# Sohojoe/ppo-dash

Measured on AMD Instinct MI355X. Metric: env-steps/sec (rollout+GAE+PPO update) at 4096 envs×128 steps, 1/2/4/8 MI355X, higher is better.
Workload: dtype f32

## Files before the change

include/ppo_hip.h:

```cpp
#ifndef PPO_HIP_H
#define PPO_HIP_H

#include <stdint.h>

#ifdef __cplusplus
extern "C" {
#endif

#define PPO_EARG 1001
#define PPO_ESHAPE 1002

const char* ppo_last_error(void);
int ppo_abi_version(void);
int ppo_prof_enable(const char* names, int capacity);
int ppo_prof_collect(double* out3);
int ppo_prof_collect_one(int idx, double* out3);

int ppo_gae_partials_count(int N);
int ppo_compute_returns(const float* rewards, float* value_preds, const float* masks, const float* bad_masks,
                        const float* next_value, float* returns, float* adv, double* partials, int T, int N,
                        double gamma, double gae_lambda, int use_gae, int use_proper_time_limits, void* stream);
int ppo_gae_scan_partials_count(int N);
int ppo_compute_returns_scan(const float* rewards, float* value_preds, const float* masks, const float* bad_masks,
                             const float* next_value, float* returns, float* adv, double* partials, int T, int N,
                             double gamma, double gae_lambda, int use_gae, int use_proper_time_limits, void* stream);
int ppo_adv_diff_partials_count(long long n);
int ppo_adv_diff(const float* returns, const float* value_preds, float* adv, double* partials, long long n,
                 void* stream);
int ppo_adv_finalize(const double* partials, int nparts, double count, double* stats, void* stream);
int ppo_adv_normalize(float* adv, long long n, const double* stats, void* stream);

int ppo_copy(void* dst, const void* src, long long bytes, void* stream);
int ppo_fill_f32(float* p, long long n, float v, void* stream);
int ppo_storage_insert_scalars(int N, int step, const int64_t* action, const float* logp, const float* value,
                               const float* reward, const float* mask, const float* bad_mask, int64_t* actions,
                               float* action_log_probs, float* value_preds, float* rewards, float* masks,
                               float* bad_masks, void* stream);
int ppo_gather_rows(const void* src, const int64_t* idx, void* dst, long long nrows, long long row_bytes,
                    void* stream);
int ppo_gather_f16_to_f32(const void* src, const int64_t* idx, float* dst, long long nrows, long long row_elems,
                          void* stream);
int ppo_gather_env_columns(const void* src, const int64_t* envs, void* dst, int T, int N, int nsel,
                           long long row_bytes, void* stream);
int ppo_synth_env_step(uint8_t* obs, int N, long long obs_bytes, float* reward, float* mask, float* bad_mask,
                       unsigned long long seed, unsigned long long step, float p_done, void* stream);

int ppo_cartpole_step(float* state, int* steps, const int64_t* action, float* obs, float* reward, float* mask,
                      float* bad_mask, float* ep_len, int N, unsigned long long seed, unsigned long long counter,
                      int max_steps, void* stream);

long long ppo_packed_weights_size(int H);
int ppo_packed_offsets(int H, long long* off6);
int ppo_pack_weights(const float* w2, const float* w3, const float* w4, int H, float* packed, void* stream);
int ppo_conv1_fwd(const void* obs, int obs_is_u8, const int64_t* idx, long long row0, int C, int B, const float* w1,
                  const float* b1, float* out, void* stream);
int ppo_conv1_fwd_mask(const void* obs, int obs_is_u8, const int64_t* idx, long long row0, int C, int B,
                       const float* w1, const float* b1, float* out, uint32_t* mbits, void* stream);
int ppo_conv1_fwd_f32(const float* obs, const int64_t* idx, long long row0, int B, const float* w1, const float* b1,
                      float* out, uint32_t* mbits, void* stream);
int ppo_conv1_fwd_rgb(const uint8_t* frames, const int64_t* idx, long long row0, int B, const float* mean, double stdv,
                      const float* w1, const float* b1, float* out, uint32_t* mbits, void* stream);
int ppo_conv1_wgrad_f32(const float* dz1, const float* obs, const int64_t* idx, long long row0, int B, int Z,
                        float* slab, float* slab_bias, void* stream);
int ppo_conv1_wgrad_rgb(const float* dz1, const uint8_t* frames, const int64_t* idx, long long row0, int B,
                        const float* mean, double stdv, int Z, float* slab, float* slab_bias, void* stream);
int ppo_conv2_fwd(const float* a1, int B, const float* w2p, const float* b2, float* out, void* stream);
int ppo_conv2_fwd_mask(const float* a1, int B, const float* w2p, const float* b2, float* out, uint64_t* mbits,
                       void* stream);
int ppo_conv3_fwd(const float* a2, int B, const float* w3p, const float* b3, float* out, void* stream);
int ppo_trunk_fwd(const uint8_t* obs, const int64_t* idx, long long row0, int B, const float* w1, const float* b1,
                  float* a1, uint32_t* m1, const float* w2p, const float* b2, float* a2, uint64_t* m2,
                  const float* w3p, const float* b3, float* a3, void* stream);
int ppo_fc_fwd(const float* x, int M, const float* w4p, const float* b, int H, float* out, int ldo, void* stream);
long long ppo_fc_fwd_ws_bytes(int M, int H);
int ppo_fc_fwd_ws(const float* x, int M, const float* w4p, const float* b, int H, float* out, int ldo, float* ws,
                  long long ws_bytes, void* stream);
int ppo_linear_relu_fwd(const float* x, int M, int K, const float* w, const float* b, int N, float* out,
                        void* stream);
int ppo_linear_fwd_ex(const float* x, const int64_t* idx, int M, int K, int lda, const float* w, const float* b,
                      int N, float* out, int ldo, int act, void* stream);
int ppo_linear_dgrad_ex(const float* dy, int M, int K, const float* wt, int N, const float* act, int ldact, int mode,
                        float* dx, void* stream);
int ppo_linear_dgrad_pair(const float* dy0, const float* wt0, int K0, const float* dy1, const float* wt1, int K1,
                          int M, int N, float* dx, void* stream);
int ppo_transpose(const float* src, int rows, int cols, float* dst, void* stream);
int ppo_linear_dgrad_mask(const float* dy, int M, int K, const float* wt, int N, const float* act, float* dx,
                          void* stream);
int ppo_conv3_fwd_mask(const float* a2, int B, const float* w3p, const float* b3, float* out, uint16_t* mbits,
                       void* stream);
int ppo_fc_dgrad_bits(const float* dy, int M, int K, const float* wt, const uint16_t* mbits, float* dx,
                      void* stream);
int ppo_conv3_dgrad(const float* dz3, int B, const float* w3d, const float* a2, float* dz2, void* stream);
int ppo_conv3_dgrad_bits_ok(void);
int ppo_conv3_dgrad_bits(const float* dz3, int B, const float* w3d, const uint64_t* m2bits, float* dz2,
                         void* stream);
int ppo_conv2_dgrad(const float* dz2, int B, const float* w2d, const float* a1, float* dz1, void* stream);
int ppo_conv2_dgrad_bits_ok(void);
int ppo_conv2_dgrad_bits(const float* dz2, int B, const float* w2d, const uint32_t* m1bits, float* dz1,
                         void* stream);
int ppo_wgrad_splits(long long R, int tiles, int target_blocks, int min_ktiles);
int ppo_conv1_wgrad(const float* dz1, const void* obs, int obs_is_u8, const int64_t* idx, long long row0, int C,
                    int B, int Z, float* slab, float* slab_bias, void* stream);
int ppo_conv2_wgrad(const float* dz2, const float* a1, int B, int Z, float* slab, float* slab_bias, void* stream);
int ppo_conv3_wgrad(const float* dz3, const float* a2, int B, int Z, float* slab, float* slab_bias, void* stream);
int ppo_linear_wgrad(const float* dy, const float* x, int R, int N, int K, int Z, float* slab, float* slab_bias,
                     void* stream);
int ppo_probe_side_kernel(int blocks, int threads, long long ticks, long long* stamps, void* stream);
int ppo_probe_now(long long* out, void* stream);
int ppo_wgrad_reduce(const float* slab, const float* slab_bias, int Z, int M, int NW, int kind, int a, int b,
                     float* gw, float* gb, float scale, int accumulate, void* stream);
int ppo_colsum(const float* src, long long ld, int rows, long long cols, float* out, float scale, int accumulate,
               void* stream);
int ppo_tune_set(const char* key, int value);
int ppo_tune_get(const char* key);

int ppo_obs_preprocess(const uint8_t* src, long long src_stride, int N, int S, int mode, const double* mean,
                       double stdv, int mono, float* dst, long long dst_stride, void* stream);
int ppo_frame_stack(float* stacked, int N, int nstack, long long frame_elems, const float* obs,
                    const uint8_t* done, int reset, void* stream);

int ppo_gru_step_fwd(const float* hprev, const float* masks, const int64_t* mask_idx, const float* whh,
                     const float* bhh, const float* gi, int M, int H, float* hout, float* save_r, float* save_z,
                     float* save_n, float* save_ghn, float* save_hin, void* stream);
int ppo_gru_cell_bwd(const float* dout, const float* carry, const float* r, const float* z, const float* n,
                     const float* ghn, const float* hin, float* dgi, float* dgh, float* dhz, int M, int H,
                     int has_carry, void* stream);
int ppo_gru_step_bwd(const float* dgh, const float* whhT, const float* dhz, const float* masks,
                     const int64_t* mask_idx, float* carry, int M, int H, void* stream);
int ppo_gru_variant_set(int v);
int ppo_gru_variant_get(void);
int ppo_gru_seq_fwd(const float* h0, const float* masks, const int64_t* idx, const float* whh, const float* bhh,
                    const float* gi, int T, int n, int H, float* hout, float* save_r, float* save_z, float* save_n,
                    float* save_ghn, float* save_hin, void* stream);
int ppo_gru_persist_set(int v);
int ppo_gru_persist_get(void);
int ppo_gru_persist_spin_set(int polls);
int ppo_gru_persist_timeouts(void* stream);
int ppo_gru_seq_counters(int n);
int ppo_gru_seq_fwd_ws(const float* h0, const float* masks, const int64_t* idx, const float* whh, const float* bhh,
                       const float* gi, int T, int n, int H, float* hout, float* save_r, float* save_z,
                       float* save_n, float* save_ghn, float* save_hin, int* counters, int* err, void* stream);
int ppo_gru_seq_bwd(const float* dout, const float* save_r, const float* save_z, const float* save_n,
                    const float* save_ghn, const float* save_hin, const float* masks, const int64_t* idx,
                    const float* whhT, int T, int n, int H, float* dgi, float* dgh, float* dhz, float* carry,
                    void* stream);
int ppo_gru_seq_bwd_ws(const float* dout, const float* save_r, const float* save_z, const float* save_n,
                       const float* save_ghn, const float* save_hin, const float* masks, const int64_t* idx,
                       const float* whhT, int T, int n, int H, float* dgi, float* dgh, float* dhz, float* carry,
                       int* counters, int* err, void* stream);
int ppo_gru_step_bwd_cell(const float* dgh, const float* whhT, float* dhz, const float* masks,
                          const int64_t* mask_idx, float* carry, int M, int H, const float* dout_prev,
                          const float* r, const float* z, const float* n, const float* ghn, const float* hin,
                          float* dgi_prev, float* dgh_prev, void* stream);
int ppo_gru_pack(const float* wih, const float* whh, int H, int I, int Ip, float* wih_pad, float* wihT, float* whhT,
                 void* stream);
int ppo_concat_cols(const float* src, const int64_t* idx, long long rows, int ncols, float* dst, int ld, int col0,
                    int zero_to, void* stream);
int ppo_rec_indices(const int64_t* envs, int n, int T, int N, int64_t* idx, void* stream);

int ppo_heads_act(const float* feat, const float* feat_v, int N, int H, const float* wc, const float* bc,
                  const float* wa,
                  const float* ba, int A, const float* noise, unsigned long long seed, unsigned long long counter,
                  int deterministic, const int64_t* given, float* value, int64_t* action, float* logp,
                  float* entropy, void* stream);
int ppo_heads_train_blocks(int B);
int ppo_heads_train(const float* feat, const float* feat_v, int B, int H, const float* wc, const float* bc,
                    const float* wa,
                    const float* ba, int A, const int64_t* idx, long long row0, const int64_t* actions,
                    const float* old_logp, const float* adv, const float* vpred, const float* ret, float clip,
                    float value_coef, float entropy_coef, float inv_b, int use_clipped_value_loss, int feat_act,
                    float* dfeat, float* dfeat_v, float* part_w, float* part_b, float* part_loss, void* stream);
int ppo_heads_reduce(const float* part_w, const float* part_b, const float* part_loss, int nblk, int H, int A,
                     float* g_wc, float* g_bc, float* g_wa, float* g_ba, double* loss_acc, double inv_b, float scale,
                     int use_clipped_value_loss, void* stream);
int ppo_heads_gauss_act(const float* feat, const float* feat_v, int N, int H, const float* wc, const float* bc,
                        const float* wa, const float* ba, const float* logstd, int A, const float* noise,
                        unsigned long long seed, unsigned long long counter, int deterministic, const float* given,
                        float* value, float* action, float* logp, float* entropy, void* stream);
int ppo_heads_gauss_train(const float* feat, const float* feat_v, int B, int H, const float* wc, const float* bc,
                          const float* wa, const float* ba, const float* logstd, int A, const int64_t* idx,
                          long long row0, const float* actions, const float* old_logp, const float* adv,
                          const float* vpred, const float* ret, float clip, float value_coef, float entropy_coef,
                          float inv_b, int use_clipped_value_loss, int feat_act, float* dfeat, float* dfeat_v,
                          float* part_w, float* part_b, float* part_loss, void* stream);
int ppo_heads_gauss_reduce(const float* part_w, const float* part_b, const float* part_loss, int nblk, int H, int A,
                           float* g_wc, float* g_bc, float* g_wa, float* g_ba, float* g_logstd, double* loss_acc,
                           double inv_b, float scale, void* stream);
int ppo_heads_bern_act(const float* feat, const float* feat_v, int N, int H, const float* wc, const float* bc,
                       const float* wa, const float* ba, int A, const float* noise, unsigned long long seed,
                       unsigned long long counter, int deterministic, const float* given, float* value,
                       float* action, float* logp, float* entropy, void* stream);
int ppo_heads_bern_train(const float* feat, const float* feat_v, int B, int H, const float* wc, const float* bc,
                         const float* wa, const float* ba, int A, const int64_t* idx, long long row0,
                         const float* actions, const float* old_logp, const float* adv, const float* vpred,
                         const float* ret, float clip, float value_coef, float entropy_coef, float inv_b,
                         int use_clipped_value_loss, int feat_act, float* dfeat, float* dfeat_v, float* part_w,
                         float* part_b, float* part_loss, void* stream);
int ppo_heads_act_dc(const float* feat, const float* feat_v, int N, int H, const float* wc, const float* bc,
                     const float* wa, const float* ba, int A, const float* noise, unsigned long long seed,
                     const unsigned long long* counter, int deterministic, const int64_t* given, float* value,
                     int64_t* action, float* logp, float* entropy, void* stream);
int ppo_heads_gauss_act_dc(const float* feat, const float* feat_v, int N, int H, const float* wc, const float* bc,
                           const float* wa, const float* ba, const float* logstd, int A, const float* noise,
                           unsigned long long seed, const unsigned long long* counter, int deterministic,
                           const float* given, float* value, float* action, float* logp, float* entropy,
                           void* stream);
int ppo_heads_bern_act_dc(const float* feat, const float* feat_v, int N, int H, const float* wc, const float* bc,
                          const float* wa, const float* ba, int A, const float* noise, unsigned long long seed,
                          const unsigned long long* counter, int deterministic, const float* given, float* value,
                          float* action, float* logp, float* entropy, void* stream);
int ppo_rng_advance(unsigned long long* counter, unsigned long long by, void* stream);
int ppo_mean_f32(const float* x, long long n, float* out, void* stream);

int ppo_grad_partials_count(long long n);
int ppo_grad_sumsq(const float* g, long long n, float scale, double* partials, void* stream);
int ppo_clip_adam(float* params, float* grads, float* exp_avg, float* exp_avg_sq, long long n,
                  const double* partials, float scale, double max_norm, double lr, double beta1, double beta2,
                  double eps, long long step, double* norm_out, void* stream);
int ppo_clip_adam_guarded(float* params, float* grads, float* exp_avg, float* exp_avg_sq, long long n,
                          const double* partials, float scale, double max_norm, double lr, double beta1,
                          double beta2, double eps, long long step, double* norm_out, const int* guard_i,
                          const double* guard_d, int* skipped, void* stream);

#ifdef __cplusplus
}
#endif
#endif
```

ppo-dash_amd/a2c_ppo_acktr/_engine.py:

```python
import contextlib

import os

import torch

from . import _dist
from ._hip import call, ptr, stream
from .distributions import Bernoulli, DiagGaussian

FUSED_TRUNK = os.environ.get("PPO_FUSED_TRUNK", "1") != "0"
FEAT = 32 * 7 * 7


def _with_precision(fn):
    def wrapper(self, *args, **kwargs):
        if not getattr(self.policy, "_half_mode", False):
            return fn(self, *args, **kwargs)
        prev = call("ppo_tune_get", b"products")
        if prev != 1:
            call("ppo_tune_set", b"products", 1)
        try:
            return fn(self, *args, **kwargs)
        finally:
            if prev != 1:
                call("ppo_tune_set", b"products", prev)
    wrapper.__name__, wrapper.__doc__ = fn.__name__, fn.__doc__
    return wrapper


class _Workspace:
    def __init__(self):
        self.bufs = {}
        self.version = 0

    def get(self, name, numel, dtype=torch.float32, device=None):
        t = self.bufs.get(name)
        if t is None or t.numel() < numel or t.dtype != dtype or t.device != device:
            t = torch.empty(max(int(numel), 1), dtype=dtype, device=device)
            self.bufs[name] = t
            self.version += 1
        return t


class CNNEngine:

    W1, B1, W2, B2, W3, B3, W4, B4, WC, BC, WA, BA, LS = range(13)
    recurrent = False

    def _bind_dist(self, policy):
        self.dist_kind = ("gauss" if isinstance(policy.dist, DiagGaussian) else
                          "bern" if isinstance(policy.dist, Bernoulli) else "cat")
        self.gauss = self.dist_kind == "gauss"
        self.float_actions = self.dist_kind != "cat"
        self.A = (policy.dist.fc_mean if self.gauss else policy.dist.linear).weight.shape[0]

    def __init__(self, policy, device):
        self.policy = policy
        self.device = device
        base = policy.base
        self.C = base.main[0].weight.shape[1]
        self.H = base.main[7].weight.shape[0]
        self._bind_dist(policy)
        if self.H > 512 or self.H % 4 != 0:
            raise NotImplementedError(f"hidden_size {self.H}: the HIP engine supports multiples of 4 up to 512")
        if not self.recurrent and base.critic_linear.weight.shape[1] != self.H:
            raise NotImplementedError("vector observations with a non-recurrent CNNBase are not supported "
                                      "(the reference crashes there too: Categorical expects hidden_size inputs)")
        self.params = list(policy.parameters())
        self.ws = {"act": _Workspace(), "train": _Workspace()}
        self.act_ws = "act"
        self.obs_decode = None
        self.packed = None
        self._pack_key = None
        self.epoch = 0
        self._flatten()
        self.rng_seed = int(torch.initial_seed()) & 0xFFFFFFFFFFFFFFFF
        self.rng_counter = 0
        self._n_cu = None
        self._init_status()

    def _init_status(self):
        self.status = torch.zeros(4, dtype=torch.int32, device=self.device)
        self._rng_dev = None
        self._device_counter = False

    @property
    def rng_dev(self):
        if self._rng_dev is None:
            self._rng_dev = torch.zeros(1, dtype=torch.int64, device=self.device)
        return self._rng_dev

    def set_rng_dev(self, value):
        v = int(value) & 0xFFFFFFFFFFFFFFFF
        self.rng_dev.fill_(v - (1 << 64) if v >> 63 else v)

    @contextlib.contextmanager
    def using_device_counter(self):
        prev, self._device_counter = self._device_counter, True
        try:
            yield self.rng_dev
        finally:
            self._device_counter = prev

    def status_ptr(self, i):
        return self.status.data_ptr() + 4 * i

    def _flatten(self):
        n = sum(p.numel() for p in self.params)
        flat = torch.empty(n, device=self.device)
        grad = torch.zeros(n, device=self.device)
        off = 0
        self.offsets = []
        with torch.no_grad():
            for p in self.params:
                k = p.numel()
                flat[off:off + k].copy_(p.data.reshape(-1))
                p.data = flat[off:off + k].view_as(p)
                p.grad = grad[off:off + k].view_as(p)
                self.offsets.append(off)
                off += k
        self.flat, self.grad, self.numel = flat, grad, n
        self.epoch += 1

    @contextlib.contextmanager
    def using_workspace(self, name):
        self.ws.setdefault(name, _Workspace())
        prev, self.act_ws = self.act_ws, name
        try:
            yield self.ws[name]
        finally:
            self.act_ws = prev

    def is_bound(self):
        base = self.flat.data_ptr()
        for p, off in zip(self.params, self.offsets):
            if p.data.data_ptr() != base + 4 * off or not p.is_cuda:
                return False
        return True

    def ensure_bound(self):
        if not self.is_bound():
            self._flatten()

    def pv(self, i):
        return self.flat.data_ptr() + 4 * self.offsets[i]

    def gv(self, i):
        return self.grad.data_ptr() + 4 * self.offsets[i]

    def pack(self, force=False):
        key = (sum(p._version for p in self.params), self.epoch)
        if not force and self.packed is not None and key == self._pack_key:
            return
        if self.packed is None:
            self.packed = torch.empty(call("ppo_packed_weights_size", self.H), device=self.device)
            offs = torch.zeros(6, dtype=torch.int64)
            call("ppo_packed_offsets", self.H, offs.data_ptr())
            self.poff = [int(x) for x in offs]
        call("ppo_pack_weights", self.pv(self.W2), self.pv(self.W3), self.pv(self.W4), self.H,
             self.packed.data_ptr(), stream())
        self._pack_extra()
        self._pack_key = key

    def _pack_extra(self):
        pass

    def pk(self, seg):
        return self.packed.data_ptr() + 4 * self.poff[seg]

    @staticmethod
    def _obs_args(obs):
        if obs.dtype == torch.uint8:
            return 1
        if obs.dtype == torch.float32:
            return 0
        raise TypeError(f"observations must be uint8, float32 or float16, got {obs.dtype}")

    @staticmethod
    def _is_rgb(obs):
        return obs.dtype == torch.uint8 and tuple(obs.shape[-3:]) == (84, 84, 3)

    def set_obs_decode(self, mean, std):
        if self.C != 4:
            raise NotImplementedError("the fused RGB decode produces FrameStackMono(2)'s 4 channels (C = 4)")
        if mean is not None:
            m64 = torch.as_tensor(mean, dtype=torch.float64).reshape(84, 84, 3)
            m32 = m64.to(torch.float32)
            if not torch.equal(m32.to(torch.float64), m64):
                raise ValueError("the fused decode needs fp32-representable means (NormalizeWrapper's files hold "
                                 "fp32 values); use ObsPreprocess into fp32 storage otherwise")
            mean = m32.contiguous().to(self.device)
        if not float(std):
            raise ValueError("std must be non-zero")
        self.obs_decode = (mean, float(std))

    def _conv1(self, obs, idx, B, a1, m1, s):
        if self._is_rgb(obs):
            if self.obs_decode is None:
                raise TypeError("raw u8 RGB frames need the fused decode: Policy.set_obs_decode(ObsPreprocess)")
            mean, std = self.obs_decode
            call("ppo_conv1_fwd_rgb", obs.data_ptr(), ptr(idx, torch.int64, "idx"), 0, B, ptr(mean), std,
                 self.pv(self.W1), self.pv(self.B1), a1.data_ptr(), ptr(m1), s)
        elif m1 is not None:
            call("ppo_conv1_fwd_mask", obs.data_ptr(), self._obs_args(obs), ptr(idx, torch.int64, "idx"), 0, self.C,
                 B, self.pv(self.W1), self.pv(self.B1), a1.data_ptr(), m1.data_ptr(), s)
        else:
            call("ppo_conv1_fwd", obs.data_ptr(), self._obs_args(obs), ptr(idx, torch.int64, "idx"), 0, self.C, B,
                 self.pv(self.W1), self.pv(self.B1), a1.data_ptr(), s)

    def _obs_f32(self, obs, idx, B, ws):
        if obs.dtype != torch.float16:
            return obs, idx
        x = ws.get("obs32", B * self.C * 84 * 84, device=self.device)
        call("ppo_gather_f16_to_f32", obs.data_ptr(), ptr(idx, torch.int64, "idx"), x.data_ptr(), B,
             self.C * 84 * 84, stream())
        return x, None

    def trunk(self, obs, idx, B, ws, out=None, ldo=None):
        dev = self.device
        obs, idx = self._obs_f32(obs, idx, B, ws)
        a1 = ws.get("a1", B * 400 * 32, device=dev)
        a2 = ws.get("a2", B * 81 * 64, device=dev)
        a3 = ws.get("a3", B * FEAT, device=dev)
        if out is None:
            out, ldo = ws.get("h", B * self.H, device=dev), self.H
        s = stream()
        train = ws is self.ws["train"]
        m1 = ws.get("m1bits", B * 400, dtype=torch.int32, device=dev) if train else None
        m2 = ws.get("m2bits", B * 81, dtype=torch.int64, device=dev) if train else None
        m3 = ws.get("m3bits", B * 49, dtype=torch.int32, device=dev) if train else None
        if obs.dtype == torch.uint8 and self.C == 4 and not self._is_rgb(obs) and FUSED_TRUNK and not train:
            call("ppo_trunk_fwd", obs.data_ptr(), ptr(idx, torch.int64, "idx"), 0, B, self.pv(self.W1),
                 self.pv(self.B1), a1.data_ptr(), None, self.pk(0), self.pv(self.B2), a2.data_ptr(), None,
                 self.pk(1), self.pv(self.B3), a3.data_ptr(), s)
        else:
            self._conv1(obs, idx, B, a1, m1[:B * 400] if train else None, s)
            if train:
                call("ppo_conv2_fwd_mask", a1.data_ptr(), B, self.pk(0), self.pv(self.B2), a2.data_ptr(),
                     m2.data_ptr(), s)
                call("ppo_conv3_fwd_mask", a2.data_ptr(), B, self.pk(1), self.pv(self.B3), a3.data_ptr(),
                     m3.data_ptr(), s)
            else:
                call("ppo_conv2_fwd", a1.data_ptr(), B, self.pk(0), self.pv(self.B2), a2.data_ptr(), s)
                call("ppo_conv3_fwd", a2.data_ptr(), B, self.pk(1), self.pv(self.B3), a3.data_ptr(), s)
        if train:
            self._mask_rows = B
        nb = call("ppo_fc_fwd_ws_bytes", B, self.H)
        if nb:
            fws = ws.get("fc_ws", nb // 4, device=dev)
            call("ppo_fc_fwd_ws", a3.data_ptr(), B, self.pk(2), self.pv(self.B4), self.H, out.data_ptr(), ldo,
                 fws.data_ptr(), nb, s)
        else:
            call("ppo_fc_fwd", a3.data_ptr(), B, self.pk(2), self.pv(self.B4), self.H, out.data_ptr(), ldo, s)
        return out

    def _check_obs(self, obs):
        obs = obs if obs.is_cuda else obs.to(self.device)
        if self.obs_decode is not None and self._is_rgb(obs) and obs.dim() == 4:
            return obs.contiguous()
        if tuple(obs.shape[1:]) != (self.C, 84, 84):
            raise RuntimeError(f"CNNBase expects [N,{self.C},84,84] observations"
                               + (" or raw [N,84,84,3] u8 frames" if self.obs_decode is not None else "")
                               + f", got {tuple(obs.shape)}")
        return obs.contiguous()

    def _heads(self, h, B, deterministic=False, noise=None, given=None, want_entropy=False, value_only=False,
               hv=None):
        value = torch.empty(B, 1, device=self.device)
        if value_only:
            action = logp = ent = None
        elif self.float_actions:
            action = given if given is not None else torch.empty(B, self.A, device=self.device)
            logp = torch.empty(B, 1, device=self.device)
            ent = torch.empty(B, device=self.device) if want_entropy else None
        else:
            action = given if given is not None else torch.empty(B, 1, dtype=torch.int64, device=self.device)
            logp = torch.empty(B, 1, device=self.device)
            ent = torch.empty(B, device=self.device) if want_entropy else None
        if noise is not None:
            noise = noise.to(self.device, torch.float32).contiguous()
            if noise.shape != (B, self.A):
                raise RuntimeError(f"noise must be [{B},{self.A}]")
        if self._device_counter:
            counter, dc = self.rng_dev.data_ptr(), "_dc"
        else:
            self.rng_counter += 1
            counter, dc = self.rng_counter, ""
        if self.float_actions and given is not None and given.numel() != B * self.A:
            raise RuntimeError(f"actions must be [{B},{self.A}], got {tuple(given.shape)}")
        if self.dist_kind == "bern":
            call("ppo_heads_bern_act" + dc, h.data_ptr(), ptr(hv), B, self.H, self.pv(self.WC), self.pv(self.BC),
                 self.pv(self.WA), self.pv(self.BA), self.A, ptr(noise), self.rng_seed, counter,
                 int(bool(deterministic)),
                 ptr(given.reshape(-1).contiguous() if given is not None else None, torch.float32, "action"),
                 value.data_ptr(), None if given is not None or value_only else action.data_ptr(),
                 ptr(logp), ptr(ent), stream())
        elif self.gauss:
            call("ppo_heads_gauss_act" + dc, h.data_ptr(), ptr(hv), B, self.H, self.pv(self.WC), self.pv(self.BC),
                 self.pv(self.WA), self.pv(self.BA), self.pv(self.LS), self.A, ptr(noise), self.rng_seed,
                 counter, int(bool(deterministic)),
                 ptr(given.reshape(-1).contiguous() if given is not None else None, torch.float32, "action"),
                 value.data_ptr(), None if given is not None or value_only else action.data_ptr(),
                 ptr(logp), ptr(ent), stream())
        else:
            call("ppo_heads_act" + dc, h.data_ptr(), ptr(hv), B, self.H, self.pv(self.WC), self.pv(self.BC),
                 self.pv(self.WA), self.pv(self.BA), self.A, ptr(noise), self.rng_seed, counter,
                 int(bool(deterministic)),
                 ptr(given.reshape(-1).contiguous() if given is not None else None, torch.int64, "action"),
                 value.data_ptr(), None if given is not None or value_only else action.data_ptr(),
                 ptr(logp), ptr(ent), stream())
        if self._device_counter:
            call("ppo_rng_advance", self.rng_dev.data_ptr(), 1, stream())
        return value, action, logp, ent

    def mean(self, x):
        out = torch.empty((), device=self.device)
        call("ppo_mean_f32", x.data_ptr(), x.numel(), out.data_ptr(), stream())
        return out

    @_with_precision
    def act(self, obs, deterministic=False, noise=None, given=None, want_entropy=False, value_only=False):
        self.ensure_bound()
        self.pack()
        obs = self._check_obs(obs)
        B = obs.shape[0]
        h = self.trunk(obs, None, B, self.ws[self.act_ws])
        return self._heads(h, B, deterministic, noise, given, want_entropy, value_only)

    def _heads_train(self, storage, adv, idx, feat, B, hp, loss_acc, dfeat, feat_act, feat_v=None, dfeat_v=None):
        ws, dev, H, A, s = self.ws["train"], self.device, self.H, self.A, stream()
        nblk = call("ppo_heads_train_blocks", B)
        part_w = ws.get("part_w", nblk * (1 + A) * H, device=dev)
        part_b = ws.get("part_b", nblk * (1 + (2 * A if self.gauss else A)), device=dev)
        part_l = ws.get("part_l", nblk * 4, device=dev)
        inv_b = 1.0 / B
        if self.float_actions and storage.actions.shape[-1] != A:
            raise RuntimeError(f"storage holds {storage.actions.shape[-1]} action dimensions, the policy {A}")
        if self.dist_kind == "bern":
            call("ppo_heads_bern_train", feat.data_ptr(), ptr(feat_v), B, H, self.pv(self.WC), self.pv(self.BC),
                 self.pv(self.WA), self.pv(self.BA), A, idx.data_ptr(), 0,
                 ptr(storage.actions, torch.float32, "storage.actions"), storage.action_log_probs.data_ptr(),
                 adv.data_ptr(), storage.value_preds.data_ptr(), storage.returns.data_ptr(), hp["clip"],
                 hp["value_coef"], hp["entropy_coef"], inv_b, int(hp["use_clipped_value_loss"]), int(feat_act),
                 dfeat.data_ptr(), ptr(dfeat_v), part_w.data_ptr(), part_b.data_ptr(), part_l.data_ptr(), s)
            call("ppo_heads_reduce", part_w.data_ptr(), part_b.data_ptr(), part_l.data_ptr(), nblk, H, A,
                 self.gv(self.WC), self.gv(self.BC), self.gv(self.WA), self.gv(self.BA), loss_acc.data_ptr(), inv_b,
                 1.0, int(hp["use_clipped_value_loss"]), s)
            return
        if self.gauss:
            call("ppo_heads_gauss_train", feat.data_ptr(), ptr(feat_v), B, H, self.pv(self.WC), self.pv(self.BC),
                 self.pv(self.WA), self.pv(self.BA), self.pv(self.LS), A, idx.data_ptr(), 0,
                 ptr(storage.actions, torch.float32, "storage.actions"), storage.action_log_probs.data_ptr(),
                 adv.data_ptr(), storage.value_preds.data_ptr(), storage.returns.data_ptr(), hp["clip"],
                 hp["value_coef"], hp["entropy_coef"], inv_b, int(hp["use_clipped_value_loss"]), int(feat_act),
                 dfeat.data_ptr(), ptr(dfeat_v), part_w.data_ptr(), part_b.data_ptr(), part_l.data_ptr(), s)
            call("ppo_heads_gauss_reduce", part_w.data_ptr(), part_b.data_ptr(), part_l.data_ptr(), nblk, H, A,
                 self.gv(self.WC), self.gv(self.BC), self.gv(self.WA), self.gv(self.BA), self.gv(self.LS),
                 loss_acc.data_ptr(), inv_b, 1.0, s)
            return
        call("ppo_heads_train", feat.data_ptr(), ptr(feat_v), B, H, self.pv(self.WC), self.pv(self.BC), self.pv(self.WA),
             self.pv(self.BA), A, idx.data_ptr(), 0, storage.actions.data_ptr(), storage.action_log_probs.data_ptr(),
             adv.data_ptr(), storage.value_preds.data_ptr(), storage.returns.data_ptr(), hp["clip"], hp["value_coef"],
             hp["entropy_coef"], inv_b, int(hp["use_clipped_value_loss"]), int(feat_act), dfeat.data_ptr(),
             ptr(dfeat_v), part_w.data_ptr(), part_b.data_ptr(), part_l.data_ptr(), s)
        call("ppo_heads_reduce", part_w.data_ptr(), part_b.data_ptr(), part_l.data_ptr(), nblk, H, A,
             self.gv(self.WC), self.gv(self.BC), self.gv(self.WA), self.gv(self.BA), loss_acc.data_ptr(), inv_b, 1.0,
             int(hp["use_clipped_value_loss"]), s)

    def _trunk_backward(self, B, dh, obs, idx):
        ws, dev, s = self.ws["train"], self.device, stream()
        a1 = ws.bufs["a1"]
        a2, a3 = ws.bufs["a2"], ws.bufs["a3"]
        dz3 = ws.get("dz3", B * FEAT, device=dev)
        dz2 = ws.get("dz2", B * 81 * 64, device=dev)
        dz1 = ws.get("dz1", B * 400 * 32, device=dev)
        bits = getattr(self, "_mask_rows", None) == B
        if bits:
            call("ppo_fc_dgrad_bits", dh.data_ptr(), B, self.H, self.pk(3), ws.bufs["m3bits"].data_ptr(),
                 dz3.data_ptr(), s)
        else:
            call("ppo_linear_dgrad_mask", dh.data_ptr(), B, self.H, self.pk(3), FEAT, a3.data_ptr(), dz3.data_ptr(),
                 s)
        self._wgrad("fc", B, dh, a3, None, s)
        _dist.start_bucket(self.grad[self.offsets[self.W4]:])
        if bits:
            call("ppo_conv3_dgrad_bits", dz3.data_ptr(), B, self.pk(4), ws.bufs["m2bits"].data_ptr(), dz2.data_ptr(),
                 s)
        else:
            call("ppo_conv3_dgrad", dz3.data_ptr(), B, self.pk(4), a2.data_ptr(), dz2.data_ptr(), s)
        self._wgrad("conv3", B, dz3, a2, None, s)
        if bits:
            call("ppo_conv2_dgrad_bits", dz2.data_ptr(), B, self.pk(5), ws.bufs["m1bits"].data_ptr(), dz1.data_ptr(),
                 s)
        else:
            call("ppo_conv2_dgrad", dz2.data_ptr(), B, self.pk(5), a1.data_ptr(), dz1.data_ptr(), s)
        self._wgrad("conv2", B, dz2, a1, None, s)
        if obs.dtype == torch.float16:
            obs, idx = ws.bufs["obs32"], None
        self._wgrad("conv1", B, dz1, obs, idx, s)

    def _finish_step(self, optimizer):
        optimizer._step_flat(self)
        self.epoch += 1
        self.pack(force=True)

    @_with_precision
    def train_minibatch(self, storage, adv, idx, hp, loss_acc, optimizer):
        self.ensure_bound()
        self.pack()
        _dist.begin_minibatch()
        B = idx.numel()
        ws = self.ws["train"]
        h = self.trunk(storage.obs, idx, B, ws)
        dh = ws.get("dh", B * self.H, device=self.device)
        self._heads_train(storage, adv, idx, h, B, hp, loss_acc, dh, feat_act=1)
        self._trunk_backward(B, dh, storage.obs, idx)
        self._finish_step(optimizer)

    def _wgrad(self, layer, B, dz, x, idx, s):
        dev = self.device
        ws = self.ws["train"]
        if layer == "conv1":
            M, NW, kind, ka, kb, wi, bi, R, tiles = 32, self.C * 64, 0, 0, 0, self.W1, self.B1, B * 400, 1
        elif layer == "conv2":
            M, NW, kind, ka, kb, wi, bi, R, tiles = 64, 512, 1, 4, 32, self.W2, self.B2, B * 81, 4
        elif layer == "conv3":
            M, NW, kind, ka, kb, wi, bi, R, tiles = 32, 576, 1, 3, 64, self.W3, self.B3, B * 49, 5
        else:
            M, NW, kind, ka, kb, wi, bi, R, tiles = self.H, FEAT, 2, 32, 49, self.W4, self.B4, B, \
                ((self.H + 127) // 128) * 13
        if self._n_cu is None:
            self._n_cu = torch.cuda.get_device_properties(self.device).multi_processor_count
        target = max(self._n_cu, -(-B // 512)) * tiles if layer in ("conv1", "conv2", "conv3") else 2048
        Z = call("ppo_wgrad_splits", R, tiles, target, 16)
        slab = ws.get("slab", Z * M * NW, device=dev)
        slab_b = ws.get("slab_b", Z * M, device=dev)
        if layer == "conv1" and self._is_rgb(x):
            mean, std = self.obs_decode
            call("ppo_conv1_wgrad_rgb", dz.data_ptr(), x.data_ptr(), ptr(idx), 0, B, ptr(mean), std, Z,
                 slab.data_ptr(), slab_b.data_ptr(), s)
        elif layer == "conv1":
            call("ppo_conv1_wgrad", dz.data_ptr(), x.data_ptr(), self._obs_args(x), ptr(idx), 0, self.C, B, Z,
                 slab.data_ptr(), slab_b.data_ptr(), s)
        elif layer == "conv2":
            call("ppo_conv2_wgrad", dz.data_ptr(), x.data_ptr(), B, Z, slab.data_ptr(), slab_b.data_ptr(), s)
        elif layer == "conv3":
            call("ppo_conv3_wgrad", dz.data_ptr(), x.data_ptr(), B, Z, slab.data_ptr(), slab_b.data_ptr(), s)
        else:
            call("ppo_linear_wgrad", dz.data_ptr(), x.data_ptr(), B, self.H, FEAT, Z, slab.data_ptr(),
                 slab_b.data_ptr(), s)
        scale = 1.0 / 255.0 if layer == "conv1" and x.dtype == torch.uint8 and not self._is_rgb(x) else 1.0
        call("ppo_wgrad_reduce", slab.data_ptr(), slab_b.data_ptr(), Z, M, NW, kind, ka, kb, self.gv(wi), self.gv(bi),
             scale, 0, s)

    def _dense_wgrad(self, dy, x, R, N, K, kind, a, wi, bi):
        ws, dev, s = self.ws["train"], self.device, stream()
        tiles = ((N + 127) // 128) * ((K + 127) // 128)
        Z = call("ppo_wgrad_splits", R, tiles, 2048, 16)
        slab = ws.get("slab", Z * N * K, device=dev)
        slab_b = ws.get("slab_b", Z * N, device=dev)
        call("ppo_linear_wgrad", dy.data_ptr(), x.data_ptr(), R, N, K, Z, slab.data_ptr(), slab_b.data_ptr(), s)
        call("ppo_wgrad_reduce", slab.data_ptr(), slab_b.data_ptr(), Z, N, K, kind, a, 0, self.gv(wi), self.gv(bi),
             1.0, 0, s)


class RecurrentEngine(CNNEngine):

    GIH, GHH, GBI, GBH = range(4)
    W1, B1, W2, B2, W3, B3, W4, B4, WC, BC, WA, BA, LS = range(4, 17)
    recurrent = True

    def __init__(self, policy, device):
        gru = policy.base.gru
        self.V = policy.base.vector_obs_len
        H = policy.base.main[7].weight.shape[0]
        self.I = H + self.V
        self.Ip = (self.I + 3) // 4 * 4
        if gru.weight_ih_l0.shape != (3 * H, self.I) or H % 32 != 0:
            raise NotImplementedError("GRU engine needs hidden_size a multiple of 32 (<= 512)")
        self.gru_packed = None
        super().__init__(policy, device)

    def _pack_extra(self):
        H, Ip = self.H, self.Ip
        if self.gru_packed is None:
            self.gru_packed = torch.empty(3 * H * Ip + 6 * H * H, device=self.device)
        gp = self.gru_packed.data_ptr()
        self.wih_pad, self.wihT, self.whhT = gp, gp + 4 * 3 * H * Ip, gp + 4 * (3 * H * Ip + 3 * H * H)
        call("ppo_gru_pack", self.pv(self.GIH), self.pv(self.GHH), H, self.I, Ip, self.wih_pad, self.wihT, self.whhT,
             stream())

    def _input(self, obs, vec, idx, B, ws, rows_vec=None):
        dev, s, H, Ip = self.device, stream(), self.H, self.Ip
        x = ws.get("xpad", B * Ip, device=dev)
        self.trunk(obs, idx, B, ws, out=x, ldo=Ip)
        if Ip > H:
            src = vec if vec is not None else x
            call("ppo_concat_cols", src.data_ptr(), ptr(rows_vec), B, self.V if vec is not None else 0,
                 x.data_ptr(), Ip, H, Ip - H, s)
        gi = ws.get("gi", B * 3 * H, device=dev)
        call("ppo_linear_fwd_ex", x.data_ptr(), None, B, Ip, Ip, self.wih_pad, self.pv(self.GBI), 3 * H,
             gi.data_ptr(), 3 * H, 0, s)
        return x, gi

    def _vec(self, vec, B):
        if self.V == 0:
            return None
        return vec.to(self.device, torch.float32).reshape(B, self.V).contiguous()

    @_with_precision
    def act(self, obs, deterministic=False, noise=None, given=None, want_entropy=False, value_only=False,
            vec=None, hxs=None, masks=None):
        self.ensure_bound()
        self.pack()
        obs = self._check_obs(obs)
        B = obs.shape[0]
        ws = self.ws[self.act_ws]
        _, gi = self._input(obs, self._vec(vec, B), None, B, ws)
        hxs = hxs.to(self.device, torch.float32).reshape(B, self.H).contiguous()
        m = masks.to(self.device, torch.float32).reshape(B).contiguous() if masks is not None else None
        hout = torch.empty(B, self.H, device=self.device)
        call("ppo_gru_step_fwd", hxs.data_ptr(), ptr(m), None, self.pv(self.GHH), self.pv(self.GBH), gi.data_ptr(),
             B, self.H, hout.data_ptr(), None, None, None, None, None, stream())
        value, action, logp, ent = self._heads(hout, B, deterministic, noise, given, want_entropy, value_only)
        return value, action, logp, ent, hout

    @_with_precision
    def evaluate_sequence(self, obs, vec, hxs, masks, action):
        self.ensure_bound()
        self.pack()
        obs = self._check_obs(obs)
        R = obs.shape[0]
        N = hxs.shape[0]
        T = R // N
        ws = self.ws[self.act_ws]
        _, gi = self._input(obs, self._vec(vec, R), None, R, ws)
        hxs = hxs.to(self.device, torch.float32).reshape(N, self.H).contiguous()
        m = masks.to(self.device, torch.float32).reshape(R).contiguous()
        hout = torch.empty(R, self.H, device=self.device)
        H, s = self.H, stream()
        cnt = ws.get("gru_cnt", call("ppo_gru_seq_counters", N), torch.int32, self.device)
        call("ppo_gru_seq_fwd_ws", hxs.data_ptr(), m.data_ptr(), None, self.pv(self.GHH), self.pv(self.GBH),
             gi.data_ptr(), T, N, H, hout.data_ptr(), None, None, None, None, None, cnt.data_ptr(), self.status_ptr(2),
             s)
        if int(self.status[2].item()):
            self.status[2].zero_()
            raise RuntimeError("evaluate_actions: the persistent GRU kernel timed out (its outputs are invalid; "
                               "ppo_gru_persist_set(0) selects the per-step launches)")
        given = action.to(self.device, torch.float32 if self.float_actions else torch.int64)
        value, _, logp, ent = self._heads(hout, R, want_entropy=True, given=given)
        return value, logp, ent, hout[(T - 1) * N:]

    @_with_precision
    def train_minibatch_rec(self, storage, adv, envs, hp, loss_acc, optimizer):
        self.ensure_bound()
        self.pack()
        _dist.begin_minibatch()
        dev, H, s = self.device, self.H, stream()
        T, N, n = storage.num_steps, storage.rewards.shape[1], envs.numel()
        R = T * n
        ws = self.ws["train"]
        idx = ws.get("ridx", R, torch.int64, dev)[:R]
        call("ppo_rec_indices", envs.data_ptr(), n, T, N, idx.data_ptr(), s)
        h0 = ws.get("h0", n * H, device=dev)
        call("ppo_gather_rows", storage.recurrent_hidden_states.data_ptr(), envs.data_ptr(), h0.data_ptr(), n,
             4 * H, s)
        vec = storage.vector_obs if self.V else None
        x, gi = self._input(storage.obs, vec, idx, R, ws, rows_vec=idx if self.V else None)
        hout = ws.get("hout", R * H, device=dev)
        sv = {k: ws.get("s_" + k, R * H, device=dev) for k in ("r", "z", "n", "ghn", "hin")}
        masks = storage.masks
        cnt = ws.get("gru_cnt", call("ppo_gru_seq_counters", n), torch.int32, dev)
        _dist.assert_no_pending("train_minibatch_rec")
        call("ppo_gru_seq_fwd_ws", h0.data_ptr(), masks.data_ptr(), idx.data_ptr(), self.pv(self.GHH),
             self.pv(self.GBH), gi.data_ptr(), T, n, H, hout.data_ptr(), sv["r"].data_ptr(), sv["z"].data_ptr(),
             sv["n"].data_ptr(), sv["ghn"].data_ptr(), sv["hin"].data_ptr(), cnt.data_ptr(), self.status_ptr(0), s)
        dout = ws.get("dout", R * H, device=dev)
        self._heads_train(storage, adv, idx, hout, R, hp, loss_acc, dout, feat_act=0)
        dgi = ws.get("dgi", R * 3 * H, device=dev)
        dgh = ws.get("dgh", R * 3 * H, device=dev)
        dhz = ws.get("dhz", n * H, device=dev)
        carry = ws.get("carry", n * H, device=dev)
        _dist.assert_no_pending("train_minibatch_rec bptt")
        call("ppo_gru_seq_bwd_ws", dout.data_ptr(), sv["r"].data_ptr(), sv["z"].data_ptr(), sv["n"].data_ptr(),
             sv["ghn"].data_ptr(), sv["hin"].data_ptr(), masks.data_ptr(), idx.data_ptr(), self.whhT, T, n, H,
             dgi.data_ptr(), dgh.data_ptr(), dhz.data_ptr(), carry.data_ptr(), cnt.data_ptr(), self.status_ptr(0), s)
        self._dense_wgrad(dgh, sv["hin"], R, 3 * H, H, 0, 0, self.GHH, self.GBH)
        self._dense_wgrad(dgi, x, R, 3 * H, self.Ip, 3, self.I, self.GIH, self.GBI)
        dh = ws.get("dh", R * H, device=dev)
        call("ppo_linear_dgrad_ex", dgi.data_ptr(), R, 3 * H, self.wihT, H, x.data_ptr(), self.Ip, 1, dh.data_ptr(),
             s)
        self._trunk_backward(R, dh, storage.obs, idx)
        self._finish_step(optimizer)


class MLPEngine(CNNEngine):

    AW1, AB1, AW2, AB2, CW1, CB1, CW2, CB2, WC, BC, WA, BA, LS = range(13)

    def __init__(self, policy, device):
        base = policy.base
        if base.is_recurrent != self.recurrent:
            raise NotImplementedError("a recurrent MLPBase runs on RecurrentMLPEngine, a feed-forward one on "
                                      "MLPEngine (Policy.hip_engine() selects the engine)")
        self.policy, self.device = policy, device
        self.H = base._hidden_size
        self.I = (base.gru.weight_ih_l0 if self.recurrent else base.actor[0].weight).shape[1]
        self.V = base.vector_obs_len
        self.obs_dim = self.I - self.V
        self.Ip = (self.I + 3) // 4 * 4
        self._bind_dist(policy)
        if self.recurrent and (self.H % 32 != 0 or self.H > 512 or self.I < 1):
            raise NotImplementedError("GRU engine needs hidden_size a multiple of 32 (<= 512)")
        if self.H % 4 != 0 or self.H > 512:
            raise NotImplementedError(f"MLPBase hidden_size {self.H}: multiples of 4 up to 512")
        self.params = list(policy.parameters())
        self.ws = {"act": _Workspace(), "train": _Workspace()}
        self.act_ws = "act"
        self.packed = None
        self._pack_key = None
        self.epoch = 0
        self._flatten()
        self.rng_seed = int(torch.initial_seed()) & 0xFFFFFFFFFFFFFFFF
        self.rng_counter = 0
        self._init_status()

    def pack(self, force=False):
        key = (sum(p._version for p in self.params), self.epoch)
        if not force and self.packed is not None and key == self._pack_key:
            return
        H, Ip, s = self.H, self.Ip, stream()
        if self.packed is None:
            self.packed = torch.empty(2 * H * Ip + 2 * H * H, device=self.device)
        b = self.packed.data_ptr()
        self.aw1, self.cw1 = b, b + 4 * H * Ip
        self.aw2T, self.cw2T = b + 8 * H * Ip, b + 8 * H * Ip + 4 * H * H
        for w, dst in ((self.AW1, self.aw1), (self.CW1, self.cw1)):
            call("ppo_concat_cols", self.pv(w), None, H, self.I, dst, Ip, 0, Ip, s)
        call("ppo_transpose", self.pv(self.AW2), H, H, self.aw2T, s)
        call("ppo_transpose", self.pv(self.CW2), H, H, self.cw2T, s)
        self._pack_key = key

    def _x(self, obs, vec, idx, B, ws):
        dev, s = self.device, stream()
        x = ws.get("x", B * self.Ip, device=dev)
        call("ppo_concat_cols", obs.data_ptr(), ptr(idx), B, self.obs_dim, x.data_ptr(), self.Ip, 0,
             self.obs_dim if self.V else self.Ip, s)
        if self.V:
            call("ppo_concat_cols", vec.data_ptr(), ptr(idx), B, self.V, x.data_ptr(), self.Ip, self.obs_dim,
                 self.Ip - self.obs_dim, s)
        return x

    def _tower_in(self):
        return self.Ip, self.aw1, self.cw1

    def towers(self, x, B, ws):
        dev, H, s = self.device, self.H, stream()
        Ip, aw1, cw1 = self._tower_in()
        out = {}
        for name, w1, b1, w2, b2 in (("a", aw1, self.AB1, self.AW2, self.AB2),
                                     ("c", cw1, self.CB1, self.CW2, self.CB2)):
            h1 = ws.get(name + "1", B * H, device=dev)
            h2 = ws.get(name + "2", B * H, device=dev)
            call("ppo_linear_fwd_ex", x.data_ptr(), None, B, Ip, Ip, w1, self.pv(b1), H, h1.data_ptr(), H, 2, s)
            call("ppo_linear_fwd_ex", h1.data_ptr(), None, B, H, H, self.pv(w2), self.pv(b2), H, h2.data_ptr(), H, 2, s)
            out[name] = (h1, h2)
        return out

    @_with_precision
    def act(self, obs, deterministic=False, noise=None, given=None, want_entropy=False, value_only=False, vec=None):
        self.ensure_bound()
        self.pack()
        obs = (obs if obs.is_cuda else obs.to(self.device)).to(torch.float32).reshape(obs.shape[0], -1).contiguous()
        B = obs.shape[0]
        if obs.shape[1] != self.obs_dim:
            raise RuntimeError(f"MLPBase expects [N,{self.obs_dim}] observations, got {tuple(obs.shape)}")
        ws = self.ws[self.act_ws]
        v = vec.to(self.device, torch.float32).reshape(B, self.V).contiguous() if self.V else None
        x = self._x(obs, v, None, B, ws)
        t = self.towers(x, B, ws)
        return self._heads(t["a"][1], B, deterministic, noise, given, want_entropy, value_only, hv=t["c"][1])

    @_with_precision
    def train_minibatch(self, storage, adv, idx, hp, loss_acc, optimizer):
        self.ensure_bound()
        self.pack()
        _dist.begin_minibatch()
        dev, H, B = self.device, self.H, idx.numel()
        ws = self.ws["train"]
        x = self._x(storage.obs, storage.vector_obs if self.V else None, idx, B, ws)
        t = self.towers(x, B, ws)
        da2 = ws.get("da2", B * H, device=dev)
        dc2 = ws.get("dc2", B * H, device=dev)
        self._heads_train(storage, adv, idx, t["a"][1], B, hp, loss_acc, da2, feat_act=2, feat_v=t["c"][1],
                          dfeat_v=dc2)
        self._towers_backward(t, x, B, da2, dc2, self.Ip, 3, self.I)
        self._finish_step(optimizer)

    def _towers_backward(self, t, x, B, da2, dc2, K, kind, width):
        ws, dev, H = self.ws["train"], self.device, self.H
        d1s = []
        for name, d2, w1, b1, w2, b2, w2T in (("a", da2, self.AW1, self.AB1, self.AW2, self.AB2, self.aw2T),
                                               ("c", dc2, self.CW1, self.CB1, self.CW2, self.CB2, self.cw2T)):
            h1 = t[name][0]
            self._dense_wgrad(d2, h1, B, H, H, 0, 0, w2, b2)
            d1 = ws.get("d1" + name, B * H, device=dev)
            call("ppo_linear_dgrad_ex", d2.data_ptr(), B, H, w2T, H, h1.data_ptr(), H, 2, d1.data_ptr(), stream())
            self._dense_wgrad(d1, x, B, H, K, kind, width, w1, b1)
            d1s.append(d1)
        return d1s


class RecurrentMLPEngine(MLPEngine):

    GIH, GHH, GBI, GBH = range(4)
    AW1, AB1, AW2, AB2, CW1, CB1, CW2, CB2, WC, BC, WA, BA, LS = range(4, 17)
    recurrent = True

    def pack(self, force=False):
        key = (sum(p._version for p in self.params), self.epoch)
        if not force and self.packed is not None and key == self._pack_key:
            return
        H, Ip, s = self.H, self.Ip, stream()
        if self.packed is None:
            self.packed = torch.empty(3 * H * Ip + 3 * H * H + 4 * H * H, device=self.device)
        b = self.packed.data_ptr()
        self.wih_pad, self.whhT = b, b + 4 * 3 * H * Ip
        self.aw1T = self.whhT + 4 * 3 * H * H
        self.cw1T, self.aw2T, self.cw2T = (self.aw1T + 4 * H * H * i for i in (1, 2, 3))
        call("ppo_concat_cols", self.pv(self.GIH), None, 3 * H, self.I, self.wih_pad, Ip, 0, Ip, s)
        call("ppo_transpose", self.pv(self.GHH), 3 * H, H, self.whhT, s)
        for w, dst in ((self.AW1, self.aw1T), (self.CW1, self.cw1T), (self.AW2, self.aw2T), (self.CW2, self.cw2T)):
            call("ppo_transpose", self.pv(w), H, H, dst, s)
        self._pack_key = key

    def _tower_in(self):
        return self.H, self.pv(self.AW1), self.pv(self.CW1)

    def _rows(self, obs, vec, R):
        obs = (obs if obs.is_cuda else obs.to(self.device)).to(torch.float32).reshape(R, -1).contiguous()
        if obs.shape[1] != self.obs_dim:
            raise RuntimeError(f"MLPBase expects [N,{self.obs_dim}] observations, got {tuple(obs.shape)}")
        v = vec.to(self.device, torch.float32).reshape(R, self.V).contiguous() if self.V else None
        return obs, v

    def _gi(self, x, B, ws):
        gi = ws.get("gi", B * 3 * self.H, device=self.device)
        call("ppo_linear_fwd_ex", x.data_ptr(), None, B, self.Ip, self.Ip, self.wih_pad, self.pv(self.GBI),
             3 * self.H, gi.data_ptr(), 3 * self.H, 0, stream())
        return gi

    @_with_precision
    def act(self, obs, deterministic=False, noise=None, given=None, want_entropy=False, value_only=False,
            vec=None, hxs=None, masks=None):
        self.ensure_bound()
        self.pack()
        B = obs.shape[0]
        obs, v = self._rows(obs, vec, B)
        ws = self.ws[self.act_ws]
        gi = self._gi(self._x(obs, v, None, B, ws), B, ws)
        hxs = hxs.to(self.device, torch.float32).reshape(B, self.H).contiguous()
        m = masks.to(self.device, torch.float32).reshape(B).contiguous() if masks is not None else None
        hout = torch.empty(B, self.H, device=self.device)
        call("ppo_gru_step_fwd", hxs.data_ptr(), ptr(m), None, self.pv(self.GHH), self.pv(self.GBH), gi.data_ptr(),
             B, self.H, hout.data_ptr(), None, None, None, None, None, stream())
        t = self.towers(hout, B, ws)
        value, action, logp, ent = self._heads(t["a"][1], B, deterministic, noise, given, want_entropy, value_only,
                                               hv=t["c"][1])
        return value, action, logp, ent, hout

    @_with_precision
    def evaluate_sequence(self, obs, vec, hxs, masks, action):
        self.ensure_bound()
        self.pack()
        R, N = obs.shape[0], hxs.shape[0]
        T = R // N
        obs, v = self._rows(obs, vec, R)
        ws = self.ws[self.act_ws]
        gi = self._gi(self._x(obs, v, None, R, ws), R, ws)
        hxs = hxs.to(self.device, torch.float32).reshape(N, self.H).contiguous()
        m = masks.to(self.device, torch.float32).reshape(R).contiguous()
        hout = torch.empty(R, self.H, device=self.device)
        H, s = self.H, stream()
        cnt = ws.get("gru_cnt", call("ppo_gru_seq_counters", N), torch.int32, self.device)
        call("ppo_gru_seq_fwd_ws", hxs.data_ptr(), m.data_ptr(), None, self.pv(self.GHH), self.pv(self.GBH),
             gi.data_ptr(), T, N, H, hout.data_ptr(), None, None, None, None, None, cnt.data_ptr(), self.status_ptr(2),
             s)
        if int(self.status[2].item()):
            self.status[2].zero_()
            raise RuntimeError("evaluate_actions: the persistent GRU kernel timed out (its outputs are invalid; "
                               "ppo_gru_persist_set(0) selects the per-step launches)")
        given = action.to(self.device, torch.float32 if self.float_actions else torch.int64)
        t = self.towers(hout, R, ws)
        value, _, logp, ent = self._heads(t["a"][1], R, want_entropy=True, given=given, hv=t["c"][1])
        return value, logp, ent, hout[(T - 1) * N:]

    @_with_precision
    def train_minibatch_rec(self, storage, adv, envs, hp, loss_acc, optimizer):
        H = self.H
        if storage.recurrent_hidden_states.shape[-1] != H:
            raise RuntimeError(f"storage holds hidden states of width {storage.recurrent_hidden_states.shape[-1]}, "
                               f"the policy's GRU {H}")
        if storage.obs.dtype != torch.float32 or storage.obs[0, 0].numel() != self.obs_dim:
            raise RuntimeError(f"MLPBase expects float32 [{self.obs_dim}] observation rows in the storage, got "
                               f"{storage.obs.dtype} {tuple(storage.obs.shape[2:])}")
        self.ensure_bound()
        self.pack()
        _dist.begin_minibatch()
        dev, s = self.device, stream()
        T, N, n = storage.num_steps, storage.rewards.shape[1], envs.numel()
        R = T * n
        ws = self.ws["train"]
        idx = ws.get("ridx", R, torch.int64, dev)[:R]
        call("ppo_rec_indices", envs.data_ptr(), n, T, N, idx.data_ptr(), s)
        h0 = ws.get("h0", n * H, device=dev)
        call("ppo_gather_rows", storage.recurrent_hidden_states.data_ptr(), envs.data_ptr(), h0.data_ptr(), n,
             4 * H, s)
        x = self._x(storage.obs, storage.vector_obs if self.V else None, idx, R, ws)
        gi = self._gi(x, R, ws)
        hout = ws.get("hout", R * H, device=dev)
        sv = {k: ws.get("s_" + k, R * H, device=dev) for k in ("r", "z", "n", "ghn", "hin")}
        masks = storage.masks
        cnt = ws.get("gru_cnt", call("ppo_gru_seq_counters", n), torch.int32, dev)
        _dist.assert_no_pending("train_minibatch_rec")
        call("ppo_gru_seq_fwd_ws", h0.data_ptr(), masks.data_ptr(), idx.data_ptr(), self.pv(self.GHH),
             self.pv(self.GBH), gi.data_ptr(), T, n, H, hout.data_ptr(), sv["r"].data_ptr(), sv["z"].data_ptr(),
             sv["n"].data_ptr(), sv["ghn"].data_ptr(), sv["hin"].data_ptr(), cnt.data_ptr(), self.status_ptr(0), s)
        t = self.towers(hout, R, ws)
        da2 = ws.get("da2", R * H, device=dev)
        dc2 = ws.get("dc2", R * H, device=dev)
        self._heads_train(storage, adv, idx, t["a"][1], R, hp, loss_acc, da2, feat_act=2, feat_v=t["c"][1],
                          dfeat_v=dc2)
        d1a, d1c = self._towers_backward(t, hout, R, da2, dc2, H, 0, 0)
        dout = ws.get("dout", R * H, device=dev)
        call("ppo_linear_dgrad_pair", d1a.data_ptr(), self.aw1T, H, d1c.data_ptr(), self.cw1T, H, R, H,
             dout.data_ptr(), s)
        dgi = ws.get("dgi", R * 3 * H, device=dev)
        dgh = ws.get("dgh", R * 3 * H, device=dev)
        dhz = ws.get("dhz", n * H, device=dev)
        carry = ws.get("carry", n * H, device=dev)
        _dist.assert_no_pending("train_minibatch_rec bptt")
        call("ppo_gru_seq_bwd_ws", dout.data_ptr(), sv["r"].data_ptr(), sv["z"].data_ptr(), sv["n"].data_ptr(),
             sv["ghn"].data_ptr(), sv["hin"].data_ptr(), masks.data_ptr(), idx.data_ptr(), self.whhT, T, n, H,
             dgi.data_ptr(), dgh.data_ptr(), dhz.data_ptr(), carry.data_ptr(), cnt.data_ptr(), self.status_ptr(0), s)
        self._dense_wgrad(dgh, sv["hin"], R, 3 * H, H, 0, 0, self.GHH, self.GBH)
        self._dense_wgrad(dgi, x, R, 3 * H, self.Ip, 3, self.I, self.GIH, self.GBI)
        self._finish_step(optimizer)
```

ppo-dash_amd/a2c_ppo_acktr/_hip.py:

```python
import ctypes
import os

import torch

_HERE = os.path.dirname(os.path.abspath(__file__))
LIB_PATH = os.environ.get("PPO_HIP_LIB", os.path.join(os.path.dirname(_HERE), "lib", "libppo_hip.so"))

c_int, c_ll, c_ull, c_f, c_d, c_p = (ctypes.c_int, ctypes.c_longlong, ctypes.c_ulonglong, ctypes.c_float,
                                     ctypes.c_double, ctypes.c_void_p)

SIGNATURES = {
    "ppo_abi_version": [],
    "ppo_last_error": [],
    "ppo_prof_enable": [ctypes.c_char_p, c_int],
    "ppo_prof_collect": [c_p],
    "ppo_prof_collect_one": [c_int, c_p],
    "ppo_gae_partials_count": [c_int],
    "ppo_compute_returns": [c_p, c_p, c_p, c_p, c_p, c_p, c_p, c_p, c_int, c_int, c_d, c_d, c_int, c_int, c_p],
    "ppo_gae_scan_partials_count": [c_int],
    "ppo_compute_returns_scan": [c_p, c_p, c_p, c_p, c_p, c_p, c_p, c_p, c_int, c_int, c_d, c_d, c_int, c_int, c_p],
    "ppo_adv_diff_partials_count": [c_ll],
    "ppo_adv_diff": [c_p, c_p, c_p, c_p, c_ll, c_p],
    "ppo_adv_finalize": [c_p, c_int, c_d, c_p, c_p],
    "ppo_adv_normalize": [c_p, c_ll, c_p, c_p],
    "ppo_copy": [c_p, c_p, c_ll, c_p],
    "ppo_fill_f32": [c_p, c_ll, c_f, c_p],
    "ppo_storage_insert_scalars": [c_int, c_int, c_p, c_p, c_p, c_p, c_p, c_p, c_p, c_p, c_p, c_p, c_p, c_p, c_p],
    "ppo_gather_rows": [c_p, c_p, c_p, c_ll, c_ll, c_p],
    "ppo_gather_env_columns": [c_p, c_p, c_p, c_int, c_int, c_int, c_ll, c_p],
    "ppo_gather_f16_to_f32": [c_p, c_p, c_p, c_ll, c_ll, c_p],
    "ppo_synth_env_step": [c_p, c_int, c_ll, c_p, c_p, c_p, c_ull, c_ull, c_f, c_p],
    "ppo_cartpole_step": [c_p, c_p, c_p, c_p, c_p, c_p, c_p, c_p, c_int, c_ull, c_ull, c_int, c_p],
    "ppo_packed_weights_size": [c_int],
    "ppo_packed_offsets": [c_int, c_p],
    "ppo_pack_weights": [c_p, c_p, c_p, c_int, c_p, c_p],
    "ppo_conv1_fwd": [c_p, c_int, c_p, c_ll, c_int, c_int, c_p, c_p, c_p, c_p],
    "ppo_conv1_fwd_mask": [c_p, c_int, c_p, c_ll, c_int, c_int, c_p, c_p, c_p, c_p, c_p],
    "ppo_conv1_fwd_f32": [c_p, c_p, c_ll, c_int, c_p, c_p, c_p, c_p, c_p],
    "ppo_conv1_fwd_rgb": [c_p, c_p, c_ll, c_int, c_p, c_d, c_p, c_p, c_p, c_p, c_p],
    "ppo_conv1_wgrad_f32": [c_p, c_p, c_p, c_ll, c_int, c_int, c_p, c_p, c_p],
    "ppo_conv1_wgrad_rgb": [c_p, c_p, c_p, c_ll, c_int, c_p, c_d, c_int, c_p, c_p, c_p],
    "ppo_conv2_fwd": [c_p, c_int, c_p, c_p, c_p, c_p],
    "ppo_conv2_fwd_mask": [c_p, c_int, c_p, c_p, c_p, c_p, c_p],
    "ppo_conv3_fwd": [c_p, c_int, c_p, c_p, c_p, c_p],
    "ppo_trunk_fwd": [c_p, c_p, c_ll, c_int, c_p, c_p, c_p, c_p, c_p, c_p, c_p, c_p, c_p, c_p, c_p, c_p],
    "ppo_linear_relu_fwd": [c_p, c_int, c_int, c_p, c_p, c_int, c_p, c_p],
    "ppo_fc_fwd": [c_p, c_int, c_p, c_p, c_int, c_p, c_int, c_p],
    "ppo_fc_fwd_ws_bytes": [c_int, c_int],
    "ppo_fc_fwd_ws": [c_p, c_int, c_p, c_p, c_int, c_p, c_int, c_p, c_ll, c_p],
    "ppo_linear_dgrad_mask": [c_p, c_int, c_int, c_p, c_int, c_p, c_p, c_p],
    "ppo_conv3_fwd_mask": [c_p, c_int, c_p, c_p, c_p, c_p, c_p],
    "ppo_fc_dgrad_bits": [c_p, c_int, c_int, c_p, c_p, c_p, c_p],
    "ppo_conv3_dgrad": [c_p, c_int, c_p, c_p, c_p, c_p],
    "ppo_conv3_dgrad_bits_ok": [],
    "ppo_conv3_dgrad_bits": [c_p, c_int, c_p, c_p, c_p, c_p],
    "ppo_conv2_dgrad": [c_p, c_int, c_p, c_p, c_p, c_p],
    "ppo_conv2_dgrad_bits_ok": [],
    "ppo_conv2_dgrad_bits": [c_p, c_int, c_p, c_p, c_p, c_p],
    "ppo_wgrad_splits": [c_ll, c_int, c_int, c_int],
    "ppo_conv1_wgrad": [c_p, c_p, c_int, c_p, c_ll, c_int, c_int, c_int, c_p, c_p, c_p],
    "ppo_conv2_wgrad": [c_p, c_p, c_int, c_int, c_p, c_p, c_p],
    "ppo_probe_side_kernel": [c_int, c_int, c_ll, c_p, c_p],
    "ppo_probe_now": [c_p, c_p],
    "ppo_conv3_wgrad": [c_p, c_p, c_int, c_int, c_p, c_p, c_p],
    "ppo_linear_wgrad": [c_p, c_p, c_int, c_int, c_int, c_int, c_p, c_p, c_p],
    "ppo_wgrad_reduce": [c_p, c_p, c_int, c_int, c_int, c_int, c_int, c_int, c_p, c_p, c_f, c_int, c_p],
    "ppo_colsum": [c_p, c_ll, c_int, c_ll, c_p, c_f, c_int, c_p],
    "ppo_tune_set": [ctypes.c_char_p, c_int],
    "ppo_tune_get": [ctypes.c_char_p],
    "ppo_heads_act": [c_p, c_p, c_int, c_int, c_p, c_p, c_p, c_p, c_int, c_p, c_ull, c_ull, c_int, c_p, c_p, c_p,
                      c_p, c_p, c_p],
    "ppo_heads_train_blocks": [c_int],
    "ppo_heads_train": [c_p, c_p, c_int, c_int, c_p, c_p, c_p, c_p, c_int, c_p, c_ll, c_p, c_p, c_p, c_p, c_p, c_f,
                        c_f, c_f, c_f, c_int, c_int, c_p, c_p, c_p, c_p, c_p, c_p],
    "ppo_linear_fwd_ex": [c_p, c_p, c_int, c_int, c_int, c_p, c_p, c_int, c_p, c_int, c_int, c_p],
    "ppo_linear_dgrad_ex": [c_p, c_int, c_int, c_p, c_int, c_p, c_int, c_int, c_p, c_p],
    "ppo_linear_dgrad_pair": [c_p, c_p, c_int, c_p, c_p, c_int, c_int, c_int, c_p, c_p],
    "ppo_transpose": [c_p, c_int, c_int, c_p, c_p],
    "ppo_gru_step_fwd": [c_p, c_p, c_p, c_p, c_p, c_p, c_int, c_int, c_p, c_p, c_p, c_p, c_p, c_p, c_p],
    "ppo_gru_cell_bwd": [c_p, c_p, c_p, c_p, c_p, c_p, c_p, c_p, c_p, c_p, c_int, c_int, c_int, c_p],
    "ppo_gru_step_bwd": [c_p, c_p, c_p, c_p, c_p, c_p, c_int, c_int, c_p],
    "ppo_gru_variant_set": [c_int],
    "ppo_gru_variant_get": [],
    "ppo_gru_persist_set": [c_int],
    "ppo_gru_persist_get": [],
    "ppo_gru_persist_timeouts": [c_p],
    "ppo_gru_persist_spin_set": [c_int],
    "ppo_gru_seq_counters": [c_int],
    "ppo_gru_seq_fwd": [c_p, c_p, c_p, c_p, c_p, c_p, c_int, c_int, c_int, c_p, c_p, c_p, c_p, c_p, c_p, c_p],
    "ppo_gru_seq_fwd_ws": [c_p, c_p, c_p, c_p, c_p, c_p, c_int, c_int, c_int, c_p, c_p, c_p, c_p, c_p, c_p, c_p, c_p,
                           c_p],
    "ppo_gru_seq_bwd": [c_p, c_p, c_p, c_p, c_p, c_p, c_p, c_p, c_p, c_int, c_int, c_int, c_p, c_p, c_p, c_p, c_p],
    "ppo_gru_seq_bwd_ws": [c_p, c_p, c_p, c_p, c_p, c_p, c_p, c_p, c_p, c_int, c_int, c_int, c_p, c_p, c_p, c_p, c_p,
                           c_p, c_p],
    "ppo_gru_step_bwd_cell": [c_p, c_p, c_p, c_p, c_p, c_p, c_int, c_int, c_p, c_p, c_p, c_p, c_p, c_p, c_p, c_p, c_p],
    "ppo_gru_pack": [c_p, c_p, c_int, c_int, c_int, c_p, c_p, c_p, c_p],
    "ppo_concat_cols": [c_p, c_p, c_ll, c_int, c_p, c_int, c_int, c_int, c_p],
    "ppo_rec_indices": [c_p, c_int, c_int, c_int, c_p, c_p],
    "ppo_heads_reduce": [c_p, c_p, c_p, c_int, c_int, c_int, c_p, c_p, c_p, c_p, c_p, c_d, c_f, c_int, c_p],
    "ppo_mean_f32": [c_p, c_ll, c_p, c_p],
    "ppo_heads_gauss_act": [c_p, c_p, c_int, c_int, c_p, c_p, c_p, c_p, c_p, c_int, c_p, c_ull, c_ull, c_int, c_p,
                            c_p, c_p, c_p, c_p, c_p],
    "ppo_heads_gauss_train": [c_p, c_p, c_int, c_int, c_p, c_p, c_p, c_p, c_p, c_int, c_p, c_ll, c_p, c_p, c_p, c_p,
                              c_p, c_f, c_f, c_f, c_f, c_int, c_int, c_p, c_p, c_p, c_p, c_p, c_p],
    "ppo_heads_gauss_reduce": [c_p, c_p, c_p, c_int, c_int, c_int, c_p, c_p, c_p, c_p, c_p, c_p, c_d, c_f, c_p],
    "ppo_heads_bern_act": [c_p, c_p, c_int, c_int, c_p, c_p, c_p, c_p, c_int, c_p, c_ull, c_ull, c_int, c_p, c_p, c_p,
                           c_p, c_p, c_p],
    "ppo_heads_bern_train": [c_p, c_p, c_int, c_int, c_p, c_p, c_p, c_p, c_int, c_p, c_ll, c_p, c_p, c_p, c_p, c_p,
                             c_f, c_f, c_f, c_f, c_int, c_int, c_p, c_p, c_p, c_p, c_p, c_p],
    "ppo_heads_act_dc": [c_p, c_p, c_int, c_int, c_p, c_p, c_p, c_p, c_int, c_p, c_ull, c_p, c_int, c_p, c_p, c_p,
                         c_p, c_p, c_p],
    "ppo_heads_gauss_act_dc": [c_p, c_p, c_int, c_int, c_p, c_p, c_p, c_p, c_p, c_int, c_p, c_ull, c_p, c_int, c_p,
                               c_p, c_p, c_p, c_p, c_p],
    "ppo_heads_bern_act_dc": [c_p, c_p, c_int, c_int, c_p, c_p, c_p, c_p, c_int, c_p, c_ull, c_p, c_int, c_p, c_p,
                              c_p, c_p, c_p, c_p],
    "ppo_rng_advance": [c_p, c_ull, c_p],
    "ppo_obs_preprocess": [c_p, c_ll, c_int, c_int, c_int, c_p, c_d, c_int, c_p, c_ll, c_p],
    "ppo_frame_stack": [c_p, c_int, c_int, c_ll, c_p, c_p, c_int, c_p],
    "ppo_grad_partials_count": [c_ll],
    "ppo_grad_sumsq": [c_p, c_ll, c_f, c_p, c_p],
    "ppo_clip_adam": [c_p, c_p, c_p, c_p, c_ll, c_p, c_f, c_d, c_d, c_d, c_d, c_d, c_ll, c_p, c_p],
    "ppo_clip_adam_guarded": [c_p, c_p, c_p, c_p, c_ll, c_p, c_f, c_d, c_d, c_d, c_d, c_d, c_ll, c_p, c_p, c_p, c_p,
                              c_p],
}
_RESTYPES = {"ppo_last_error": ctypes.c_char_p, "ppo_packed_weights_size": c_ll, "ppo_fc_fwd_ws_bytes": c_ll}
_VALUE_FUNCS = {"ppo_abi_version", "ppo_gae_partials_count", "ppo_gae_scan_partials_count", "ppo_adv_diff_partials_count",
                "ppo_packed_weights_size", "ppo_fc_fwd_ws_bytes", "ppo_wgrad_splits", "ppo_heads_train_blocks", "ppo_grad_partials_count",
                "ppo_conv2_dgrad_bits_ok", "ppo_conv3_dgrad_bits_ok", "ppo_tune_get",
                "ppo_gru_persist_get", "ppo_gru_persist_timeouts", "ppo_gru_seq_counters"}

_LIB = None


def lib():
    global _LIB
    if _LIB is None:
        if not os.path.exists(LIB_PATH):
            raise RuntimeError(f"libppo_hip.so not found at {LIB_PATH}: build it with `make -C ppo-dash_amd` "
                               "(or __graft_entry__.build()); there is no CPU fallback")
        L = ctypes.CDLL(LIB_PATH)
        for name, args in SIGNATURES.items():
            if name.startswith("ppo_probe_") and not hasattr(L, name):
                continue
            fn = getattr(L, name)
            fn.argtypes = args
            fn.restype = _RESTYPES.get(name, c_int)
        _LIB = L
    return _LIB


class HipError(RuntimeError):
    pass


def call(name, *args):
    fn = getattr(lib(), name)
    rc = fn(*args)
    if name in _VALUE_FUNCS or name in _RESTYPES:
        return rc
    if rc != 0:
        msg = lib().ppo_last_error().decode(errors="replace")
        raise HipError(f"{name} failed ({rc}): {msg}")
    return rc


def stream():
    return torch.cuda.current_stream().cuda_stream


def ptr(t, dtype=None, name="tensor"):
    if t is None:
        return None
    if not t.is_cuda:
        raise RuntimeError(f"{name} must be on the MI355X (got {t.device}); the HIP engine has no CPU path")
    if dtype is not None and t.dtype != dtype:
        raise TypeError(f"{name} must be {dtype}, got {t.dtype}")
    if not t.is_contiguous():
        raise RuntimeError(f"{name} must be contiguous")
    return t.data_ptr()


def require_device():
    if not torch.cuda.is_available():
        raise RuntimeError("no MI355X visible: the a2c_ppo_acktr HIP engine needs a GPU (there is no CPU fallback)")
```

ppo-dash_amd/csrc/dense.hip:

```cpp
#include "conv_launch.h"

namespace {

__host__ __device__ inline void pack_segments(int H, long long* n) {
  n[0] = 64 * 512; n[1] = 32 * 576; n[2] = (long long)H * 1568; n[3] = n[2]; n[4] = 64 * 288; n[5] = 4 * 32 * 256;
}

__global__ __launch_bounds__(256) void pack_weights_kernel(const float* __restrict__ w2, const float* __restrict__ w3,
                                                           const float* __restrict__ w4, int H,
                                                           float* __restrict__ out) {
  long long n[6];
  pack_segments(H, n);
  const long long total = n[0] + n[1] + n[2] + n[3] + n[4] + n[5];
  for (long long i = (long long)blockIdx.x * 256 + threadIdx.x; i < total; i += (long long)gridDim.x * 256) {
    long long j = i, base = 0;
    int seg = 0;
    while (j >= n[seg]) {
      j -= n[seg];
      base += n[seg] * 5 / 2;
      ++seg;
    }
    float v;
    if (seg == 0) {
      const int co = (int)(j / 512), k = (int)(j % 512), ky = k / 128, kx = (k / 32) % 4, ci = k % 32;
      v = w2[co * 512 + ci * 16 + ky * 4 + kx];
    } else if (seg == 1) {
      const int co = (int)(j / 576), k = (int)(j % 576), ky = k / 192, kx = (k / 64) % 3, ci = k % 64;
      v = w3[co * 576 + ci * 9 + ky * 3 + kx];
    } else if (seg == 2) {
      const long long nn = j / 1568;
      const int k = (int)(j % 1568), pp = k / 32, c = k % 32;
      v = w4[nn * 1568 + c * 49 + pp];
    } else if (seg == 3) {
      const int k = (int)(j / H), nn = (int)(j % H), pp = k / 32, c = k % 32;
      v = w4[(long long)nn * 1568 + c * 49 + pp];
    } else if (seg == 4) {
      const int ci = (int)(j / 288), k = (int)(j % 288), ky = k / 96, kx = (k / 32) % 3, co = k % 32;
      v = w3[co * 576 + ci * 9 + ky * 3 + kx];
    } else {
      const int ph = (int)(j / 8192), rem = (int)(j % 8192), ci = rem / 256, k = rem % 256;
      const int ty = k >> 7, tx = (k >> 6) & 1, co = k & 63;
      const int ky = (ph >> 1) + 2 * ty, kx = (ph & 1) + 2 * tx;
      v = w2[co * 512 + ci * 16 + ky * 4 + kx];
    }
    out[base + j] = v;
    uint32_t h, m, l;
    split_bf16x3(v, h, m, l);
    uint16_t* pl = reinterpret_cast<uint16_t*>(out + base + n[seg]);
    pl[j] = (uint16_t)h;
    pl[n[seg] + j] = (uint16_t)m;
    pl[2 * n[seg] + j] = (uint16_t)l;
  }
}

}

PPO_API long long ppo_packed_weights_size(int H) {
  long long n[6];
  pack_segments(H, n);
  return (n[0] + n[1] + n[2] + n[3] + n[4] + n[5]) * 5 / 2;
}

PPO_API int ppo_packed_offsets(int H, long long* off6) {
  long long n[6];
  pack_segments(H, n);
  off6[0] = 0;
  for (int i = 1; i < 6; ++i) off6[i] = off6[i - 1] + n[i - 1] * 5 / 2;
  return 0;
}

PPO_API int ppo_pack_weights(const float* w2, const float* w3, const float* w4, int H, float* packed, void* stream) {
  ProfScope prof("pack_weights", as_stream(stream), 4.0 * 4.0 * ppo_packed_weights_size(H));
  PPO_REQUIRE(H > 0 && H % 4 == 0, "ppo_pack_weights: hidden size %d must be a positive multiple of 4", H);
  long long n[6];
  pack_segments(H, n);
  const long long total = n[0] + n[1] + n[2] + n[3] + n[4] + n[5];
  long long b = (total + 255) / 256;
  pack_weights_kernel<<<(unsigned)(b < 2048 ? b : 2048), 256, 0, as_stream(stream)>>>(w2, w3, w4, H, packed);
  PPO_LAUNCH_CHECK("pack_weights_kernel");
  return 0;
}

using CfgN64 = Cfg<128, 64, 2, 2, true, true>;
using CfgN128 = Cfg<128, 128, 2, 2, true, true>;
using CfgWfc = Cfg<128, 128, 2, 2, false, false, true>;
using X64 = CfgX<128, 64, 2, 2, true, true>;
using X128 = CfgX<128, 128, 2, 2, true, true>;
using X64s = CfgX<64, 64, 2, 2, true, true>;
using XW64 = CfgX<64, 128, 2, 2, false, false, true>;
using XP128 = CfgX<128, 128, 4, 1, true, true, false, false, false, true>;
using XP128w8 = CfgX<128, 128, 8, 1, true, true, false, false, false, true>;
using XP128x64w8 = CfgX<128, 64, 8, 1, true, true, false, false, false, true>;
using SW256x128 = CfgS<256, 128, 4, 2, false, false, true>;

static inline bool use_x9() { return tune_key(TK_X9) != 0; }
static inline bool use_x9_all() { return tune_key(TK_X9) == 2; }

PPO_API int ppo_fc_fwd(const float* x, int M, const float* w4p, const float* b, int H, float* out, int ldo,
                       void* stream) {
  PPO_REQUIRE(H > 0 && H % 8 == 0 && ldo >= H, "ppo_fc_fwd: H=%d ldo=%d", H, ldo);
  const int K = 1568;
  if (M > 0 && M <= tune_small_b()) return small_linear_fwd(x, nullptr, M, K, K, w4p, b, H, out, ldo, 1, as_stream(stream));
  if (use_x9()) {
    const bool wide = ((M + 127LL) / 128) * ((H + 127) / 128) >= 2LL * device_cus();
    const bool abuf = 4LL * M * K < 0x80000000LL;
#define PPO_FC(T, CFG)                                                                               \
  {                                                                                                  \
    T<CFG> p;                                                                                        \
    p.x = x; p.w = w4p; p.bias = b; p.out = out; p.M = M; p.N = H; p.K = K; p.ldo = ldo; p.relu = 1; \
    set_planes(p, w4p, (long long)H * K, H, K);                                                      \
    p.n_fast = 1;                                                                                    \
    p.vec = H % 4 == 0 && ldo % 4 == 0 && ((uintptr_t)out & 15) == 0 &&                              \
            (b == nullptr || ((uintptr_t)b & 15) == 0);                                              \
    return launch_x9(p, M, H, 1, as_stream(stream), "fc_fwd", 2.0 * M * H * K);                      \
  }
    if (wide && abuf) PPO_FC(DenseReluFwdB, XP128)
    if (wide) PPO_FC(DenseReluFwd, XP128)
    if (abuf) PPO_FC(DenseReluFwdB, XP128x64w8)
    PPO_FC(DenseReluFwd, XP128x64w8)
#undef PPO_FC
  }
  DenseReluFwd<CfgN128> p;
  p.x = x; p.w = w4p; p.bias = b; p.out = out; p.M = M; p.N = H; p.K = K; p.ldo = ldo; p.relu = 1;
  return launch(p, M, H, 1, as_stream(stream), "fc_fwd", 2.0 * M * H * K);
}

template <class C_>
struct DenseFwdSplitK : DenseReluFwdB<C_> {
  float* slab = nullptr;
  int chunk = 0;
  __device__ void k_range(int z, int& b, int& e) const {
    b = z * chunk < this->K ? z * chunk : this->K;
    e = b + chunk < this->K ? b + chunk : this->K;
  }
  __device__ void store(int m, int n, int z, float v) const {
    if (m < this->M && n < this->N) slab[((size_t)z * this->M + m) * this->N + n] = v;
  }
  __device__ void store4(int m, int n, int z, const f32x4& v) const {
    if (m < this->M && n < this->N) *reinterpret_cast<f32x4*>(slab + ((size_t)z * this->M + m) * this->N + n) = v;
  }
};

__global__ __launch_bounds__(256) void fc_splitk_reduce_kernel(const float* __restrict__ slab, int Z, int M, int N,
                                                               const float* __restrict__ bias, float* __restrict__ out,
                                                               int ldo) {
  const int n4 = N >> 2;
  const long long total = (long long)M * n4;
  for (long long i = (long long)blockIdx.x * 256 + threadIdx.x; i < total; i += (long long)gridDim.x * 256) {
    const int m = (int)(i / n4), q = (int)(i - (long long)m * n4);
    const f32x4* src = reinterpret_cast<const f32x4*>(slab + (size_t)m * N) + q;
    f32x4 v = src[0];
    for (int z = 1; z < Z; ++z) v += src[(size_t)z * M * n4];
    const f32x4 b = reinterpret_cast<const f32x4*>(bias)[q];
    f32x4 y;
#pragma unroll
    for (int r = 0; r < 4; ++r) y[r] = fmaxf(v[r] + b[r], 0.f);
    *reinterpret_cast<f32x4*>(out + (size_t)m * ldo + 4 * q) = y;
  }
}

PPO_API long long ppo_fc_fwd_ws_bytes(int M, int H) {
  const int Z = tune_key(TK_FC_SPLITK);
  if (Z <= 1 || M <= tune_small_b() || (long long)M * H > 4096LL * 1024) return 0;
  return 4LL * Z * M * H;
}

PPO_API int ppo_fc_fwd_ws(const float* x, int M, const float* w4p, const float* b, int H, float* out, int ldo,
                          float* ws, long long ws_bytes, void* stream) {
  const long long need = ppo_fc_fwd_ws_bytes(M, H);
  if (!use_x9() || need == 0 || ws == nullptr || ws_bytes < need || ldo % 4 != 0 || H % 4 != 0 || 4LL * M * 1568 >= 0x80000000LL ||
      ((uintptr_t)out & 15) != 0 || ((uintptr_t)ws & 15) != 0 || ((uintptr_t)b & 15) != 0)
    return ppo_fc_fwd(x, M, w4p, b, H, out, ldo, stream);
  const int K = 1568, Z = (int)(need / (4LL * M * H));
  hipStream_t st = as_stream(stream);
  int rc;
#define PPO_FCSK(CFG, VEC)                                                                   \
  {                                                                                          \
    DenseFwdSplitK<CFG> p;                                                                   \
    p.x = x; p.w = w4p; p.bias = b; p.out = out; p.M = M; p.N = H; p.K = K; p.ldo = ldo; p.relu = 1; \
    set_planes(p, w4p, (long long)H * K, H, K);                                              \
    p.n_fast = 1;                                                                            \
    p.slab = ws;                                                                             \
    p.vec = VEC;                                                                             \
    p.chunk = ((K + Z - 1) / Z + 31) / 32 * 32;                                              \
    rc = launch_x9(p, M, H, Z, st, "fc_fwd", 2.0 * M * H * K);                               \
  }
  if (tune_key(TK_FC_SPLITK_TILE)) PPO_FCSK(XP128, 1)
  else PPO_FCSK(XP128x64w8, 0)
#undef PPO_FCSK
  if (rc) return rc;
  const long long n = (long long)M * (H / 4);
  fc_splitk_reduce_kernel<<<(unsigned)std::min<long long>((n + 255) / 256, 4096), 256, 0, st>>>(ws, Z, M, H, b, out,
                                                                                               ldo);
  PPO_LAUNCH_CHECK("fc_splitk_reduce_kernel");
  return 0;
}

PPO_API int ppo_linear_relu_fwd(const float* x, int M, int K, const float* w, const float* b, int N, float* out,
                                void* stream) {
  PPO_REQUIRE(K % 4 == 0, "ppo_linear_relu_fwd: K=%d must be a multiple of 4", K);
  if (M > 0 && M <= tune_small_b()) return small_linear_fwd(x, nullptr, M, K, K, w, b, N, out, N, 1, as_stream(stream));
  if (use_x9()) {
    DenseReluFwd<X128> p;
    p.x = x; p.w = w; p.bias = b; p.out = out; p.M = M; p.N = N; p.K = K;
    return launch_x9(p, M, N, 1, as_stream(stream), "linear_relu_fwd", 2.0 * M * N * K);
  }
  if (N % 128 == 0) {
    DenseReluFwd<CfgN128> p;
    p.x = x; p.w = w; p.bias = b; p.out = out; p.M = M; p.N = N; p.K = K;
    return launch(p, M, N, 1, as_stream(stream), "linear_relu_fwd", 2.0 * M * N * K);
  }
  DenseReluFwd<CfgN64> p;
  p.x = x; p.w = w; p.bias = b; p.out = out; p.M = M; p.N = N; p.K = K;
  return launch(p, M, N, 1, as_stream(stream), "linear_relu_fwd", 2.0 * M * N * K);
}

PPO_API int ppo_linear_fwd_ex(const float* x, const int64_t* idx, int M, int K, int lda, const float* w, const float* b,
                              int N, float* out, int ldo, int act, void* stream) {
  PPO_REQUIRE(K % 4 == 0 && lda % 4 == 0, "ppo_linear_fwd_ex: K=%d lda=%d must be multiples of 4", K, lda);
  PPO_REQUIRE(act >= 0 && act <= 2, "ppo_linear_fwd_ex: act=%d", act);
  if (M > 0 && M <= tune_small_b()) return small_linear_fwd(x, idx, M, K, lda, w, b, N, out, ldo, act, as_stream(stream));
  if (use_x9()) {
    if (N <= 64) {
      DenseReluFwd<X64> p;
      p.x = x; p.w = w; p.bias = b; p.out = out; p.M = M; p.N = N; p.K = K; p.lda = lda; p.ldo = ldo; p.relu = act;
      p.idx = idx;
      return launch_x9(p, M, N, 1, as_stream(stream), "linear_fwd_ex", 2.0 * M * N * K);
    }
#define PPO_LEX(CFG)                                                                                       \
  {                                                                                                        \
    DenseReluFwd<CFG> p;                                                                                   \
    p.x = x; p.w = w; p.bias = b; p.out = out; p.M = M; p.N = N; p.K = K; p.lda = lda; p.ldo = ldo; p.relu = act; \
    p.idx = idx;                                                                                           \
    p.vec = N % 4 == 0 && (ldo ? ldo : N) % 4 == 0 && ((uintptr_t)out & 15) == 0 &&                        \
            (b == nullptr || ((uintptr_t)b & 15) == 0);                                                    \
    return launch_x9(p, M, N, 1, as_stream(stream), "linear_fwd_ex", 2.0 * M * N * K);                     \
  }
    if (((M + 127LL) / 128) * ((N + 127) / 128) < 2LL * device_cus()) PPO_LEX(X64s)
    PPO_LEX(X128)
#undef PPO_LEX
  }
  if (N % 128 == 0) {
    DenseReluFwd<CfgN128> p;
    p.x = x; p.w = w; p.bias = b; p.out = out; p.M = M; p.N = N; p.K = K; p.lda = lda; p.ldo = ldo; p.relu = act;
    p.idx = idx;
    return launch(p, M, N, 1, as_stream(stream), "linear_fwd_ex", 2.0 * M * N * K);
  }
  DenseReluFwd<CfgN64> p;
  p.x = x; p.w = w; p.bias = b; p.out = out; p.M = M; p.N = N; p.K = K; p.lda = lda; p.ldo = ldo; p.relu = act;
  p.idx = idx;
  return launch(p, M, N, 1, as_stream(stream), "linear_fwd_ex", 2.0 * M * N * K);
}

PPO_API int ppo_linear_dgrad_ex(const float* dy, int M, int K, const float* wt, int N, const float* act, int ldact,
                                int mode, float* dx, void* stream) {
  PPO_REQUIRE(K % 4 == 0, "ppo_linear_dgrad_ex: K=%d must be a multiple of 4", K);
  if (use_x9()) {
    DenseDgradMask<X128> p;
    p.dy = dy; p.wt = wt; p.act = act; p.dx = dx; p.M = M; p.N = N; p.K = K; p.ldact = ldact; p.mode = mode;
    p.vec = N % 4 == 0 && (ldact ? ldact : N) % 4 == 0 && ((uintptr_t)dx & 15) == 0 &&
            (act == nullptr || ((uintptr_t)act & 15) == 0);
    return launch_x9(p, M, N, 1, as_stream(stream), "linear_dgrad_ex", 2.0 * M * N * K);
  }
  DenseDgradMask<CfgN128> p;
  p.dy = dy; p.wt = wt; p.act = act; p.dx = dx; p.M = M; p.N = N; p.K = K; p.ldact = ldact; p.mode = mode;
  return launch(p, M, N, 1, as_stream(stream), "linear_dgrad_ex", 2.0 * M * N * K);
}

PPO_API int ppo_linear_dgrad_pair(const float* dy0, const float* wt0, int K0, const float* dy1, const float* wt1,
                                  int K1, int M, int N, float* dx, void* stream) {
  PPO_REQUIRE(K0 > 0 && K1 > 0 && K0 % 4 == 0 && K1 % 4 == 0,
              "ppo_linear_dgrad_pair: K0=%d K1=%d must be positive multiples of 4", K0, K1);
  PPO_REQUIRE(M >= 0 && N > 0, "ppo_linear_dgrad_pair: M=%d N=%d", M, N);
  const double flops = 2.0 * M * N * ((double)K0 + K1);
#define PPO_DGP(CFG, LAUNCH, VEC)                                                                  \
  {                                                                                                \
    DenseDgradPair<CFG> p;                                                                         \
    p.dy0 = dy0; p.wt0 = wt0; p.dy1 = dy1; p.wt1 = wt1; p.dx = dx; p.M = M; p.N = N; p.K0 = K0; p.K1 = K1; \
    p.vec = VEC;                                                                                   \
    return LAUNCH(p, M, N, 1, as_stream(stream), "linear_dgrad_pair", flops);                      \
  }
  if (use_x9()) {
    const int vec = N % 4 == 0 && ((uintptr_t)dx & 15) == 0;
    if (N <= 64) PPO_DGP(X64, launch_x9, vec)
    PPO_DGP(X128, launch_x9, vec)
  }
  PPO_DGP(CfgN128, launch, 0)
#undef PPO_DGP
}

__global__ __launch_bounds__(256) void transpose_kernel(const float* __restrict__ src, int rows, int cols,
                                                        float* __restrict__ dst) {
  const long long total = (long long)rows * cols;
  for (long long i = (long long)blockIdx.x * 256 + threadIdx.x; i < total; i += (long long)gridDim.x * 256) {
    const int c = (int)(i / rows), r = (int)(i - (long long)c * rows);
    dst[i] = src[(size_t)r * cols + c];
  }
}

PPO_API int ppo_transpose(const float* src, int rows, int cols, float* dst, void* stream) {
  PPO_REQUIRE(rows > 0 && cols > 0, "ppo_transpose: %d x %d", rows, cols);
  long long b = ((long long)rows * cols + 255) / 256;
  transpose_kernel<<<(unsigned)(b < 2048 ? b : 2048), 256, 0, as_stream(stream)>>>(src, rows, cols, dst);
  PPO_LAUNCH_CHECK("transpose_kernel");
  return 0;
}

PPO_API int ppo_linear_dgrad_mask(const float* dy, int M, int K, const float* wt, int N, const float* act, float* dx,
                                  void* stream) {
  PPO_REQUIRE(K % 4 == 0, "ppo_linear_dgrad_mask: K=%d must be a multiple of 4", K);
  if (use_x9()) {
    PPO_REQUIRE(K % 8 == 0, "ppo_linear_dgrad_mask: K=%d must be a multiple of 8", K);
#define PPO_DGM(T)                                                                                          \
  {                                                                                                         \
    T<XP128w8> p;                                                                                           \
    p.dy = dy; p.wt = wt; p.act = act; p.dx = dx; p.M = M; p.N = N; p.K = K;                                \
    set_planes(p, wt, (long long)N * K, N, K);                                                              \
    p.n_fast = 0;    \
    p.vec = N % 4 == 0 && ((uintptr_t)dx & 15) == 0 && (act == nullptr || ((uintptr_t)act & 15) == 0);     \
    return launch_x9(p, M, N, 1, as_stream(stream), "linear_dgrad_mask", 2.0 * M * N * K);                  \
  }
    if (4LL * M * K < 0x80000000LL) PPO_DGM(DenseDgradMaskB)
    PPO_DGM(DenseDgradMask)
#undef PPO_DGM
  }
  DenseDgradMask<CfgN128> p;
  p.dy = dy; p.wt = wt; p.act = act; p.dx = dx; p.M = M; p.N = N; p.K = K;
  return launch(p, M, N, 1, as_stream(stream), "linear_dgrad_mask", 2.0 * M * N * K);
}

template <class Base>
struct WithMask3Bits : Base {
  const uint16_t* mbits = nullptr;
  __device__ uint32_t bits(int m, int n) const { return (uint32_t)mbits[(size_t)m * 98 + (n >> 4)] >> (n & 15); }
  __device__ void store(int m, int n, int, float v) const {
    if (m < this->M && n < this->N) this->dx[(size_t)m * this->N + n] = (bits(m, n) & 1u) ? v : 0.f;
  }
  __device__ void store4(int m, int n, int, const f32x4& v) const {
    if (m >= this->M || n >= this->N) return;
    const uint32_t b = bits(m, n);
    f32x4 o;
#pragma unroll
    for (int r = 0; r < 4; ++r) o[r] = ((b >> r) & 1u) ? v[r] : 0.f;
    *reinterpret_cast<f32x4*>(this->dx + (size_t)m * this->N + n) = o;
  }
};

PPO_API int ppo_fc_dgrad_bits(const float* dy, int M, int K, const float* wt, const uint16_t* mbits, float* dx,
                              void* stream) {
  PPO_REQUIRE(M >= 0 && K > 0 && K % 8 == 0 && mbits != nullptr, "ppo_fc_dgrad_bits: M=%d K=%d", M, K);
  const int N = 1568;
  if (use_x9() && 4LL * M * K < 0x80000000LL) {
    WithMask3Bits<DenseDgradMaskB<XP128w8>> p;
    p.dy = dy; p.wt = wt; p.act = nullptr; p.dx = dx; p.M = M; p.N = N; p.K = K; p.mbits = mbits;
    set_planes(p, wt, (long long)N * K, N, K);
    p.n_fast = 0;
    p.vec = ((uintptr_t)dx & 15) == 0;
    return launch_x9(p, M, N, 1, as_stream(stream), "linear_dgrad_mask", 2.0 * M * N * K);
  }
  WithMask3Bits<DenseDgradMask<CfgN128>> p;
  p.dy = dy; p.wt = wt; p.act = nullptr; p.dx = dx; p.M = M; p.N = N; p.K = K; p.mbits = mbits;
  return launch(p, M, N, 1, as_stream(stream), "linear_dgrad_mask", 2.0 * M * N * K);
}

PPO_API int ppo_wgrad_splits(long long R, int tiles, int target_blocks, int min_ktiles) {
  long long kt = (R + BK16 - 1) / BK16;
  long long z = target_blocks / (tiles > 0 ? tiles : 1);
  if (z < 1) z = 1;
  if (kt / z < min_ktiles) z = kt / min_ktiles;
  if (z < 1) z = 1;
  if (z > 4096) z = 4096;
  return (int)z;
}

PPO_API int ppo_linear_wgrad(const float* dy, const float* x, int R, int N, int K, int Z, float* slab,
                             float* slab_bias, void* stream) {
  PPO_REQUIRE(N % 4 == 0 && K % 4 == 0, "ppo_linear_wgrad: N=%d K=%d must be multiples of 4", N, K);
  if (use_x9_all() || (use_x9() && N >= 128)) {
    if (N <= 64) {
      DenseWgrad<XW64> p;
      set_wgrad(p, dy, N, R, Z, slab, slab_bias, K);
      p.x = x; p.K = K;
      return launch_x9(p, N, K, Z, as_stream(stream), "linear_wgrad", 2.0 * R * N * K);
    }
    if ((long long)R * (N > K ? N : K) * 4 < 0x7fffffffLL) {
      DenseWgradB<SW256x128> p;
      set_wgrad(p, dy, N, R, Z, slab, slab_bias, K);
      p.x = x; p.K = K; p.n_fast = 0;
      p.vec = K % 4 == 0 && ((uintptr_t)slab & 15) == 0;
      return launch_x9(p, N, K, Z, as_stream(stream), "linear_wgrad", 2.0 * R * N * K);
    }
    DenseWgrad<SW256x128> p;
    set_wgrad(p, dy, N, R, Z, slab, slab_bias, K);
    p.x = x; p.K = K; p.n_fast = 0;
    p.vec = K % 4 == 0 && ((uintptr_t)slab & 15) == 0;
    return launch_x9(p, N, K, Z, as_stream(stream), "linear_wgrad", 2.0 * R * N * K);
  }
  DenseWgrad<CfgWfc> p;
  set_wgrad(p, dy, N, R, Z, slab, slab_bias, K);
  p.x = x; p.K = K;
  return launch(p, N, K, Z, as_stream(stream), "linear_wgrad", 2.0 * R * N * K);
}

PPO_API int ppo_wgrad_reduce(const float* slab, const float* slab_bias, int Z, int M, int NW, int kind, int a, int b,
                             float* gw, float* gb, float scale, int accumulate, void* stream) {
  PPO_REQUIRE(kind >= 0 && kind <= 3, "ppo_wgrad_reduce: kind=%d", kind);
  ProfScope prof("wgrad_reduce", as_stream(stream), 4.0 * (double)Z * M * (NW + 1) + 4.0 * M * (NW + 1));
  hipStream_t st = as_stream(stream);
  const long long cols = (long long)M * NW;
  int rc = colsum(slab, cols, Z, cols, ColMap{kind, a, b, NW}, gw, scale, accumulate, st);
  if (rc) return rc;
  return colsum(slab_bias, M, Z, M, ColMap{0, 0, 0, 1}, gb, 1.0f, accumulate, st);
}

PPO_API int ppo_colsum(const float* src, long long ld, int rows, long long cols, float* out, float scale,
                       int accumulate, void* stream) {
  return colsum(src, ld, rows, cols, ColMap{0, 0, 0, 1}, out, scale, accumulate, as_stream(stream));
}
```

ppo-dash_amd/csrc/heads.hip:

```cpp
#include "heads_common.h"
#include "tune.h"

namespace {

template <int AMAX>
__device__ __forceinline__ void categorical(const float (&z)[AMAX], int A, float (&nl)[AMAX], float (&p)[AMAX]) {
  float mx = z[0];
#pragma unroll
  for (int o = 1; o < AMAX; ++o)
    if (o < A) mx = fmaxf(mx, z[o]);
  float se = 0.f;
#pragma unroll
  for (int o = 0; o < AMAX; ++o)
    if (o < A) se += expf(z[o] - mx);
  const float lse = mx + logf(se);
  float m2 = -INFINITY;
#pragma unroll
  for (int o = 0; o < AMAX; ++o) {
    nl[o] = o < A ? z[o] - lse : -INFINITY;
    if (o < A) m2 = fmaxf(m2, nl[o]);
  }
  float s2 = 0.f;
#pragma unroll
  for (int o = 0; o < AMAX; ++o) {
    p[o] = o < A ? expf(nl[o] - m2) : 0.f;
    s2 += p[o];
  }
#pragma unroll
  for (int o = 0; o < AMAX; ++o) p[o] = p[o] / s2;
}

__device__ __forceinline__ int action_index(int64_t v, int A) {
  return (uint64_t)v < (uint64_t)A ? (int)v : -1;
}

__device__ __forceinline__ float exp_noise(uint64_t seed, uint64_t counter, long long row, int o, int A) {
  const uint64_t h = mix64(seed ^ mix64(counter * 0x2545F4914F6CDD1Dull + (uint64_t)(row * A + o)));
  return -logf(u01_open0(h));
}

template <int HC, int AMAX, bool FAST>
__global__ __launch_bounds__(64 * HW) void heads_act_kernel(
    const float* __restrict__ feat, const float* __restrict__ feat_v_, int N, int H_, const float* __restrict__ wc,
    const float* __restrict__ bc, const float* __restrict__ wa, const float* __restrict__ ba, int A_,
    const float* __restrict__ noise,
    unsigned long long seed, unsigned long long counter_v, const unsigned long long* __restrict__ counter_p,
    int deterministic, const int64_t* __restrict__ given,
    float* __restrict__ value_out, int64_t* __restrict__ action_out, float* __restrict__ logp_out,
    float* __restrict__ ent_out, int rows_per_wave) {
  const int lane = threadIdx.x & 63, wave = threadIdx.x >> 6;
  const int H = FAST ? 64 * HC : H_, A = FAST ? AMAX : A_;
  const float* const feat_v = FAST ? nullptr : feat_v_;
  const uint64_t counter = rng_counter_of(counter_p, counter_v);
  HeadW<HC, AMAX> w;
  load_head_w(w, wc, wa, A, H, lane);
  const float b0 = bc[0];
  const long long r0 = ((long long)blockIdx.x * HW + wave) * rows_per_wave;
  for (int rr = 0; rr < rows_per_wave; ++rr) {
    const long long row = r0 + rr;
    if (row >= N) break;
    float f[HC], fv[HC];
#pragma unroll
    for (int c = 0; c < HC; ++c) {
      const bool in = lane + 64 * c < H;
      f[c] = in ? feat[row * H + lane + 64 * c] : 0.f;
      fv[c] = feat_v ? (in ? feat_v[row * H + lane + 64 * c] : 0.f) : f[c];
    }
    float value, z[AMAX], nl[AMAX], p[AMAX];
    head_dots(w, f, fv, value, z, b0, ba, A);
    categorical(z, A, nl, p);
    int act;
    if (given) {
      act = action_index(given[row], A);
    } else {
      act = 0;
      float best = -INFINITY;
#pragma unroll
      for (int o = 0; o < AMAX; ++o) {
        if (o < A) {
          const float sc = deterministic ? p[o] : p[o] / (noise ? noise[row * A + o] : exp_noise(seed, counter, row, o, A));
          if (sc > best) { best = sc; act = o; }
        }
      }
    }
    float lp = (unsigned)act < (unsigned)A ? 0.f : __int_as_float(0x7fc00000), ent = 0.f;
#pragma unroll
    for (int o = 0; o < AMAX; ++o) {
      if (o == act && o < A) lp = nl[o];
      if (o < A) ent -= nl[o] * p[o];
    }
    if (lane == 0) {
      if (value_out) value_out[row] = value;
      if (action_out) action_out[row] = act;
      if (logp_out) logp_out[row] = lp;
      if (ent_out) ent_out[row] = ent;
    }
  }
}

struct TrainArgs {
  const float* feat;
  const float* feat_v;
  int B, H, A;
  const float *wc, *bc, *wa, *ba;
  const int64_t* idx;
  long long row0;
  const int64_t* actions;
  const float *old_logp, *adv, *vpred, *ret;
  float clip, value_coef, entropy_coef, inv_b;
  int use_clipped_value_loss;
  int feat_act;
  float* dfeat;
  float* dfeat_v;
  float* part_w;
  float* part_b;
  float* part_loss;
  int rows_per_wave;
};

template <int HC, int AMAX, bool FAST>
__global__ __launch_bounds__(64 * HW) void heads_train_kernel(const TrainArgs a) {
  const int lane = threadIdx.x & 63, wave = threadIdx.x >> 6;
  const int H = FAST ? 64 * HC : a.H, A = FAST ? AMAX : a.A;
  const float* const feat_v = FAST ? nullptr : a.feat_v;
  float* const dfeat_v = FAST ? nullptr : a.dfeat_v;
  HeadW<HC, AMAX> w;
  load_head_w(w, a.wc, a.wa, A, H, lane);
  const float b0 = a.bc[0];
  float gwc[HC], gwa[AMAX][HC], gbc = 0.f, gba[AMAX];
#pragma unroll
  for (int c = 0; c < HC; ++c) gwc[c] = 0.f;
#pragma unroll
  for (int o = 0; o < AMAX; ++o) {
    gba[o] = 0.f;
#pragma unroll
    for (int c = 0; c < HC; ++c) gwa[o][c] = 0.f;
  }
  float s_vl = 0.f, s_al = 0.f, s_ent = 0.f, s_bad = 0.f;
  const float clip = a.clip;
  const long long r0 = ((long long)blockIdx.x * HW + wave) * a.rows_per_wave;
  int q_act = 0;
  float q_adv = 0.f, q_olp = 0.f, q_vo = 0.f, q_ret = 0.f;
  if (lane < a.rows_per_wave && r0 + lane < a.B) {
    const long long sr = a.idx ? (long long)a.idx[r0 + lane] : a.row0 + r0 + lane;
    q_act = action_index(a.actions[sr], A);
    q_adv = a.adv[sr];
    q_olp = a.old_logp[sr];
    q_vo = a.vpred[sr];
    q_ret = a.ret[sr];
  }
  auto bcast = [](float x, int j) {
    return __int_as_float(__builtin_amdgcn_readlane(__float_as_int(x), j));
  };
  float fn[HC], fvn[HC];
  auto load_row = [&](long long row) {
#pragma unroll
    for (int c = 0; c < HC; ++c) {
      const bool in = row < a.B && lane + 64 * c < H;
      fn[c] = in ? a.feat[row * H + lane + 64 * c] : 0.f;
      fvn[c] = feat_v ? (in ? feat_v[row * H + lane + 64 * c] : 0.f) : fn[c];
    }
  };
  load_row(r0);
  for (int rr = 0; rr < a.rows_per_wave; ++rr) {
    const long long row = r0 + rr;
    if (row >= a.B) break;
    float f[HC], fv[HC];
#pragma unroll
    for (int c = 0; c < HC; ++c) {
      f[c] = fn[c];
      fv[c] = fvn[c];
    }
    if (rr + 1 < a.rows_per_wave) load_row(row + 1);
    float value, z[AMAX], nl[AMAX], p[AMAX];
    head_dots(w, f, fv, value, z, b0, a.ba, A);
    categorical(z, A, nl, p);
    const int act = __builtin_amdgcn_readlane(q_act, rr);
    s_bad += (unsigned)act < (unsigned)A ? 0.f : 1.f;
    float lp = 0.f, ent = 0.f;
#pragma unroll
    for (int o = 0; o < AMAX; ++o) {
      if (o == act) lp = nl[o];
      if (o < A) ent -= nl[o] * p[o];
    }
    const float adv = bcast(q_adv, rr);
    const float ratio = expf(lp - bcast(q_olp, rr));
    const float surr1 = ratio * adv;
    const float rc = fminf(fmaxf(ratio, 1.0f - clip), 1.0f + clip);
    const float surr2 = rc * adv;
    const float w1 = surr1 < surr2 ? 1.f : (surr1 == surr2 ? 0.5f : 0.f);
    const float inr = (ratio >= 1.0f - clip && ratio <= 1.0f + clip) ? 1.f : 0.f;
    const float g_logp = -a.inv_b * (w1 * adv + (1.f - w1) * adv * inr) * ratio;
    const float vo = bcast(q_vo, rr), R = bcast(q_ret, rr);
    float g_v, vl_row;
    if (a.use_clipped_value_loss) {
      const float dv = value - vo;
      const float vpc = vo + fminf(fmaxf(dv, -clip), clip);
      const float l1 = (value - R) * (value - R);
      const float l2 = (vpc - R) * (vpc - R);
      vl_row = fmaxf(l1, l2);
      const float u1 = l1 > l2 ? 1.f : (l1 == l2 ? 0.5f : 0.f);
      const float vin = (dv >= -clip && dv <= clip) ? 1.f : 0.f;
      g_v = a.value_coef * 0.5f * a.inv_b * (u1 * 2.f * (value - R) + (1.f - u1) * 2.f * (vpc - R) * vin);
    } else {
      vl_row = (R - value) * (R - value);
      g_v = a.value_coef * a.inv_b * (value - R);
    }
    s_vl += vl_row;
    s_al += fminf(surr1, surr2);
    s_ent += ent;
    float gz[AMAX];
    const float ce = a.entropy_coef * a.inv_b;
#pragma unroll
    for (int o = 0; o < AMAX; ++o)
      gz[o] = o < A ? g_logp * ((o == act ? 1.f : 0.f) - p[o]) + ce * p[o] * (nl[o] + ent) : 0.f;
#pragma unroll
    for (int c = 0; c < HC; ++c) {
      const float dv = g_v * w.wc[c];
      float d = dfeat_v ? 0.f : dv;
#pragma unroll
      for (int o = 0; o < AMAX; ++o) d += gz[o] * w.wa[o][c];
      if (lane + 64 * c < H) {
        const size_t q = (size_t)row * H + lane + 64 * c;
        a.dfeat[q] = act_grad(d, f[c], a.feat_act);
        if (dfeat_v) dfeat_v[q] = act_grad(dv, fv[c], a.feat_act);
      }
      gwc[c] += g_v * fv[c];
#pragma unroll
      for (int o = 0; o < AMAX; ++o) gwa[o][c] += gz[o] * f[c];
    }
    gbc += g_v;
#pragma unroll
    for (int o = 0; o < AMAX; ++o) gba[o] += gz[o];
  }
  __shared__ float red[HW][64 * HC];
  __shared__ float redb[HW][AMAX + 5];
  const int NO = 1 + A;
  for (int o = 0; o < NO; ++o) {
#pragma unroll
    for (int c = 0; c < HC; ++c) {
      float v = gwc[c];
#pragma unroll
      for (int q = 0; q < AMAX; ++q)
        if (o == q + 1) v = gwa[q][c];
      red[wave][lane + 64 * c] = v;
    }
    __syncthreads();
    if (wave == 0) {
#pragma unroll
      for (int c = 0; c < HC; ++c) {
        const int j = lane + 64 * c;
        float s = red[0][j];
        for (int q = 1; q < HW; ++q) s += red[q][j];
        if (j < H) a.part_w[((size_t)blockIdx.x * NO + o) * H + j] = s;
      }
    }
    __syncthreads();
  }
  if (lane == 0) {
    redb[wave][0] = gbc;
#pragma unroll
    for (int o = 0; o < AMAX; ++o) redb[wave][1 + o] = gba[o];
    redb[wave][AMAX + 1] = s_vl;
    redb[wave][AMAX + 2] = s_al;
    redb[wave][AMAX + 3] = s_ent;
    redb[wave][AMAX + 4] = s_bad;
  }
  __syncthreads();
  if (threadIdx.x < NO) {
    float s = 0.f;
    for (int q = 0; q < HW; ++q) s += redb[q][threadIdx.x];
    a.part_b[(size_t)blockIdx.x * NO + threadIdx.x] = s;
  }
  if (threadIdx.x < 4) {
    float s = 0.f;
    for (int q = 0; q < HW; ++q) s += redb[q][AMAX + 1 + threadIdx.x];
    a.part_loss[(size_t)blockIdx.x * 4 + threadIdx.x] = s;
  }
}

__global__ __launch_bounds__(64 * HW) void heads_train_lds_kernel(const TrainArgs a) {
  constexpr int A = 8, H = 512;
  const int lane = threadIdx.x & 63, wave = threadIdx.x >> 6;
  __shared__ f32x4 Wl[9][128];
  for (int i = threadIdx.x; i < 9 * H; i += 64 * HW) {
    const int o = i / H, k = i - H * o;
    reinterpret_cast<float*>(&Wl[o][0])[k] = o == 0 ? a.wc[k] : a.wa[(o - 1) * H + k];
  }
  const float b0 = a.bc[0];
  float ba[A];
#pragma unroll
  for (int o = 0; o < A; ++o) ba[o] = a.ba[o];
  __syncthreads();
  f32x4 gw[9][2];
#pragma unroll
  for (int o = 0; o < 9; ++o) gw[o][0] = gw[o][1] = f32x4{0.f, 0.f, 0.f, 0.f};
  float gbc = 0.f, gba[A];
#pragma unroll
  for (int o = 0; o < A; ++o) gba[o] = 0.f;
  float s_vl = 0.f, s_al = 0.f, s_ent = 0.f, s_bad = 0.f;
  const float clip = a.clip;
  const long long r0 = ((long long)blockIdx.x * HW + wave) * a.rows_per_wave;
  int q_act = 0;
  float q_adv = 0.f, q_olp = 0.f, q_vo = 0.f, q_ret = 0.f;
  if (lane < a.rows_per_wave && r0 + lane < a.B) {
    const long long sr = a.idx ? (long long)a.idx[r0 + lane] : a.row0 + r0 + lane;
    q_act = action_index(a.actions[sr], A);
    q_adv = a.adv[sr];
    q_olp = a.old_logp[sr];
    q_vo = a.vpred[sr];
    q_ret = a.ret[sr];
  }
  auto bcast = [](float x, int j) { return __int_as_float(__builtin_amdgcn_readlane(__float_as_int(x), j)); };
  f32x4 fn[2];
  auto load_row = [&](long long row) {
#pragma unroll
    for (int c2 = 0; c2 < 2; ++c2)
      fn[c2] = row < a.B ? reinterpret_cast<const f32x4*>(a.feat + row * H)[lane + 64 * c2] : f32x4{0.f, 0.f, 0.f, 0.f};
  };
  load_row(r0);
  for (int rr = 0; rr < a.rows_per_wave; ++rr) {
    const long long row = r0 + rr;
    if (row >= a.B) break;
    const f32x4 f[2] = {fn[0], fn[1]};
    if (rr + 1 < a.rows_per_wave) load_row(row + 1);
    float dots[9];
#pragma unroll
    for (int o = 0; o < 9; ++o) {
      float t = 0.f;
#pragma unroll
      for (int c2 = 0; c2 < 2; ++c2) {
        const f32x4 w = Wl[o][lane + 64 * c2];
#pragma unroll
        for (int q = 0; q < 4; ++q) t += f[c2][q] * w[q];
      }
      dots[o] = wave_sum(t);
    }
    const float value = dots[0] + b0;
    float z[A], nl[A], p[A];
#pragma unroll
    for (int o = 0; o < A; ++o) z[o] = dots[1 + o] + ba[o];
    categorical(z, A, nl, p);
    const int act = __builtin_amdgcn_readlane(q_act, rr);
    s_bad += (unsigned)act < (unsigned)A ? 0.f : 1.f;
    float lp = 0.f, ent = 0.f;
#pragma unroll
    for (int o = 0; o < A; ++o) {
      if (o == act) lp = nl[o];
      ent -= nl[o] * p[o];
    }
    const float adv = bcast(q_adv, rr);
    const float ratio = expf(lp - bcast(q_olp, rr));
    const float surr1 = ratio * adv;
    const float rc = fminf(fmaxf(ratio, 1.0f - clip), 1.0f + clip);
    const float surr2 = rc * adv;
    const float w1 = surr1 < surr2 ? 1.f : (surr1 == surr2 ? 0.5f : 0.f);
    const float inr = (ratio >= 1.0f - clip && ratio <= 1.0f + clip) ? 1.f : 0.f;
    const float g_logp = -a.inv_b * (w1 * adv + (1.f - w1) * adv * inr) * ratio;
    const float vo = bcast(q_vo, rr), R = bcast(q_ret, rr);
    float g_v, vl_row;
    if (a.use_clipped_value_loss) {
      const float dv = value - vo;
      const float vpc = vo + fminf(fmaxf(dv, -clip), clip);
      const float l1 = (value - R) * (value - R);
      const float l2 = (vpc - R) * (vpc - R);
      vl_row = fmaxf(l1, l2);
      const float u1 = l1 > l2 ? 1.f : (l1 == l2 ? 0.5f : 0.f);
      const float vin = (dv >= -clip && dv <= clip) ? 1.f : 0.f;
      g_v = a.value_coef * 0.5f * a.inv_b * (u1 * 2.f * (value - R) + (1.f - u1) * 2.f * (vpc - R) * vin);
    } else {
      vl_row = (R - value) * (R - value);
      g_v = a.value_coef * a.inv_b * (value - R);
    }
    s_vl += vl_row;
    s_al += fminf(surr1, surr2);
    s_ent += ent;
    float g[9];
    g[0] = g_v;
    const float ce = a.entropy_coef * a.inv_b;
#pragma unroll
    for (int o = 0; o < A; ++o) g[1 + o] = g_logp * ((o == act ? 1.f : 0.f) - p[o]) + ce * p[o] * (nl[o] + ent);
#pragma unroll
    for (int c2 = 0; c2 < 2; ++c2) {
      f32x4 d = Wl[0][lane + 64 * c2] * g[0];
#pragma unroll
      for (int o = 1; o < 9; ++o) {
        const f32x4 w = Wl[o][lane + 64 * c2];
#pragma unroll
        for (int q = 0; q < 4; ++q) d[q] += g[o] * w[q];
      }
      f32x4 y;
#pragma unroll
      for (int q = 0; q < 4; ++q) y[q] = act_grad(d[q], f[c2][q], a.feat_act);
      reinterpret_cast<f32x4*>(a.dfeat + row * H)[lane + 64 * c2] = y;
#pragma unroll
      for (int o = 0; o < 9; ++o)
#pragma unroll
        for (int q = 0; q < 4; ++q) gw[o][c2][q] += g[o] * f[c2][q];
    }
    gbc += g_v;
#pragma unroll
    for (int o = 0; o < A; ++o) gba[o] += g[1 + o];
  }
  __shared__ f32x4 red[HW][128];
  __shared__ float redb[HW][A + 5];
  for (int o = 0; o < 9; ++o) {
#pragma unroll
    for (int c2 = 0; c2 < 2; ++c2) red[wave][lane + 64 * c2] = gw[o][c2];
    __syncthreads();
    if (wave == 0) {
#pragma unroll
      for (int c2 = 0; c2 < 2; ++c2) {
        f32x4 t = red[0][lane + 64 * c2];
        for (int q = 1; q < HW; ++q) t += red[q][lane + 64 * c2];
        reinterpret_cast<f32x4*>(a.part_w + ((size_t)blockIdx.x * 9 + o) * H)[lane + 64 * c2] = t;
      }
    }
    __syncthreads();
  }
  if (lane == 0) {
    redb[wave][0] = gbc;
#pragma unroll
    for (int o = 0; o < A; ++o) redb[wave][1 + o] = gba[o];
    redb[wave][A + 1] = s_vl;
    redb[wave][A + 2] = s_al;
    redb[wave][A + 3] = s_ent;
    redb[wave][A + 4] = s_bad;
  }
  __syncthreads();
  if (threadIdx.x < 9) {
    float t = 0.f;
    for (int q = 0; q < HW; ++q) t += redb[q][threadIdx.x];
    a.part_b[(size_t)blockIdx.x * 9 + threadIdx.x] = t;
  }
  if (threadIdx.x < 4) {
    float t = 0.f;
    for (int q = 0; q < HW; ++q) t += redb[q][A + 1 + threadIdx.x];
    a.part_loss[(size_t)blockIdx.x * 4 + threadIdx.x] = t;
  }
}

__global__ __launch_bounds__(256) void mean_kernel(const float* __restrict__ x, long long n, float* __restrict__ out) {
  double s = 0.0;
  for (long long i = threadIdx.x; i < n; i += 256) s += (double)x[i];
  __shared__ double r[256];
  r[threadIdx.x] = s;
  __syncthreads();
  for (int o = 128; o > 0; o >>= 1) {
    if (threadIdx.x < o) r[threadIdx.x] += r[threadIdx.x + o];
    __syncthreads();
  }
  if (threadIdx.x == 0) out[0] = (float)(r[0] / (double)n);
}

struct ActCall {
  const float *feat, *feat_v;
  int N, H;
  const float *wc, *bc, *wa, *ba;
  int A;
  const float* noise;
  unsigned long long seed, counter;
  const unsigned long long* counter_p;
  int det;
  const int64_t* given;
  float* v;
  int64_t* act;
  float *lp, *ent;
};

template <int HC, int AMAX>
int launch_act(const ActCall& c, hipStream_t st) {
  const int rpw = (int)std::min<long long>(8, std::max<long long>(1, ceil_div(c.N, 4096)));
  const unsigned blocks = ceil_div(c.N, HW * rpw);
  if (c.A == AMAX && c.H == 64 * HC && !c.feat_v)
    heads_act_kernel<HC, AMAX, true><<<blocks, 64 * HW, 0, st>>>(c.feat, c.feat_v, c.N, c.H, c.wc, c.bc, c.wa, c.ba, c.A,
                                                        c.noise, c.seed, c.counter, c.counter_p, c.det, c.given, c.v,
                                                        c.act, c.lp, c.ent, rpw);
  else
    heads_act_kernel<HC, AMAX, false><<<blocks, 64 * HW, 0, st>>>(c.feat, c.feat_v, c.N, c.H, c.wc, c.bc, c.wa, c.ba, c.A,
                                                         c.noise, c.seed, c.counter, c.counter_p, c.det, c.given, c.v,
                                                         c.act, c.lp, c.ent, rpw);
  PPO_LAUNCH_CHECK("heads_act_kernel");
  return 0;
}

template <int AMAX>
int dispatch_act(int HC, const ActCall& c, hipStream_t st) {
  switch (HC) {
    case 1: return launch_act<1, AMAX>(c, st);
    case 2: return launch_act<2, AMAX>(c, st);
    case 4: return launch_act<4, AMAX>(c, st);
    case 8: return launch_act<8, AMAX>(c, st);
  }
  ppo_set_error("heads: hidden size %d not supported (<= 512)", c.H);
  return PPO_EARG;
}

int heads_act(const char* name, const ActCall& c, void* stream) {
  PPO_REQUIRE(c.N >= 0 && c.A >= 1 && c.A <= 16, "%s: N=%d A=%d (1..16 actions)", name, c.N, c.A);
  PPO_REQUIRE(c.H > 0 && c.H <= 512, "%s: hidden size %d (1..512)", name, c.H);
  ProfScope prof("heads_act", as_stream(stream), (double)c.N * (4.0 * c.H * (c.feat_v ? 2 : 1) + 16.0));
  if (c.N == 0) return 0;
  if (c.A <= 8) return dispatch_act<8>(hc_of(c.H), c, as_stream(stream));
  return dispatch_act<16>(hc_of(c.H), c, as_stream(stream));
}

__global__ void rng_advance_kernel(unsigned long long* counter, unsigned long long by) { *counter += by; }

template <int HC, int AMAX>
int launch_train(const TrainArgs& a, int blocks, hipStream_t st) {
  if (tune_heads_lds() && HC == 8 && AMAX == 8 && a.A == 8 && a.H == 512 && !a.feat_v && !a.dfeat_v &&
      ((uintptr_t)a.feat & 15) == 0 && ((uintptr_t)a.dfeat & 15) == 0 && ((uintptr_t)a.part_w & 15) == 0) {
    heads_train_lds_kernel<<<blocks, 64 * HW, 0, st>>>(a);
    PPO_LAUNCH_CHECK("heads_train_lds_kernel");
    return 0;
  }
  if (a.A == AMAX && a.H == 64 * HC && !a.feat_v && !a.dfeat_v)
    heads_train_kernel<HC, AMAX, true><<<blocks, 64 * HW, 0, st>>>(a);
  else
    heads_train_kernel<HC, AMAX, false><<<blocks, 64 * HW, 0, st>>>(a);
  PPO_LAUNCH_CHECK("heads_train_kernel");
  return 0;
}

template <int AMAX>
int dispatch_train(int HC, const TrainArgs& a, int blocks, hipStream_t st) {
  switch (HC) {
    case 1: return launch_train<1, AMAX>(a, blocks, st);
    case 2: return launch_train<2, AMAX>(a, blocks, st);
    case 4: return launch_train<4, AMAX>(a, blocks, st);
    case 8: return launch_train<8, AMAX>(a, blocks, st);
  }
  ppo_set_error("heads: hidden size %d not supported (<= 512)", a.H);
  return PPO_EARG;
}

}

PPO_API int ppo_heads_act(const float* feat, const float* feat_v, int N, int H, const float* wc, const float* bc,
                          const float* wa,
                          const float* ba, int A, const float* noise, unsigned long long seed,
                          unsigned long long counter, int deterministic, const int64_t* given, float* value,
                          int64_t* action, float* logp, float* entropy, void* stream) {
  const ActCall c = {feat, feat_v, N, H, wc, bc, wa, ba, A, noise, seed, counter, nullptr, deterministic, given,
                     value, action, logp, entropy};
  return heads_act("ppo_heads_act", c, stream);
}

PPO_API int ppo_heads_act_dc(const float* feat, const float* feat_v, int N, int H, const float* wc, const float* bc,
                             const float* wa, const float* ba, int A, const float* noise, unsigned long long seed,
                             const unsigned long long* counter, int deterministic, const int64_t* given,
                             float* value, int64_t* action, float* logp, float* entropy, void* stream) {
  PPO_REQUIRE(counter != nullptr, "ppo_heads_act_dc: counter is NULL (a device pointer to one 8-byte word)");
  const ActCall c = {feat, feat_v, N, H, wc, bc, wa, ba, A, noise, seed, 0ull, counter, deterministic, given,
                     value, action, logp, entropy};
  return heads_act("ppo_heads_act_dc", c, stream);
}

PPO_API int ppo_rng_advance(unsigned long long* counter, unsigned long long by, void* stream) {
  PPO_REQUIRE(counter != nullptr, "ppo_rng_advance: counter is NULL (a device pointer to one 8-byte word)");
  rng_advance_kernel<<<1, 1, 0, as_stream(stream)>>>(counter, by);
  PPO_LAUNCH_CHECK("rng_advance_kernel");
  return 0;
}

PPO_API int ppo_heads_train_blocks(int B) {
  const int rpw = 32;
  return (int)ceil_div(B, HW * rpw);
}

PPO_API int ppo_heads_train(const float* feat, const float* feat_v, int B, int H, const float* wc, const float* bc,
                            const float* wa,
                            const float* ba, int A, const int64_t* idx, long long row0, const int64_t* actions,
                            const float* old_logp, const float* adv, const float* vpred, const float* ret, float clip,
                            float value_coef, float entropy_coef, float inv_b, int use_clipped_value_loss,
                            int feat_act, float* dfeat, float* dfeat_v, float* part_w, float* part_b,
                            float* part_loss, void* stream) {
  PPO_REQUIRE(B > 0 && A >= 1 && A <= 16, "ppo_heads_train: B=%d A=%d", B, A);
  PPO_REQUIRE(H > 0 && H <= 512, "ppo_heads_train: hidden size %d (1..512)", H);
  ProfScope prof("heads_train", as_stream(stream),
                 (double)B * (8.0 * H * (feat_v ? 2 : 1) + (idx ? 8.0 : 0.0) + 32.0));
  TrainArgs a;
  a.feat = feat; a.feat_v = feat_v; a.B = B; a.H = H; a.A = A; a.wc = wc; a.bc = bc; a.wa = wa; a.ba = ba;
  a.idx = idx; a.row0 = row0; a.actions = actions; a.old_logp = old_logp; a.adv = adv; a.vpred = vpred; a.ret = ret;
  a.clip = clip; a.value_coef = value_coef; a.entropy_coef = entropy_coef; a.inv_b = inv_b;
  a.use_clipped_value_loss = use_clipped_value_loss;
  a.feat_act = feat_act;
  a.dfeat_v = dfeat_v;
  a.dfeat = dfeat; a.part_w = part_w; a.part_b = part_b; a.part_loss = part_loss;
  a.rows_per_wave = 32;
  const int blocks = ppo_heads_train_blocks(B);
  hipStream_t st = as_stream(stream);
  if (A <= 8) return dispatch_train<8>(hc_of(H), a, blocks, st);
  return dispatch_train<16>(hc_of(H), a, blocks, st);
}

PPO_API int ppo_heads_reduce(const float* part_w, const float* part_b, const float* part_loss, int nblk, int H, int A,
                             float* g_wc, float* g_bc, float* g_wa, float* g_ba, double* loss_acc, double inv_b,
                             float scale, int use_clipped_value_loss, void* stream) {
  (void)use_clipped_value_loss;
  ProfScope prof("heads_reduce", as_stream(stream), 4.0 * nblk * (1.0 + A) * (H + 1));
  const long long NO = 1 + A;
  int rc;
  if ((rc = ppo_colsum(part_w, NO * H, nblk, H, g_wc, scale, 0, stream))) return rc;
  if ((rc = ppo_colsum(part_w + H, NO * H, nblk, (long long)A * H, g_wa, scale, 0, stream))) return rc;
  if ((rc = ppo_colsum(part_b, NO, nblk, 1, g_bc, scale, 0, stream))) return rc;
  if ((rc = ppo_colsum(part_b + 1, NO, nblk, A, g_ba, scale, 0, stream))) return rc;
  if (loss_acc) {
    loss_reduce_kernel<<<1, 256, 0, as_stream(stream)>>>(part_loss, nblk, loss_acc, inv_b);
    PPO_LAUNCH_CHECK("loss_reduce_kernel");
  }
  return 0;
}

PPO_API int ppo_mean_f32(const float* x, long long n, float* out, void* stream) {
  PPO_REQUIRE(n > 0, "ppo_mean_f32: n=%lld", n);
  mean_kernel<<<1, 256, 0, as_stream(stream)>>>(x, n, out);
  PPO_LAUNCH_CHECK("mean_kernel");
  return 0;
}
```

ppo-dash_amd/csrc/igemm.h:

```cpp
#pragma once
#include <string.h>

#include "common.h"

namespace {

constexpr int BK16 = 16;

template <int ROWS, bool KC, int BK>
struct Tile {
  static constexpr int LD = BK;
  static constexpr int SIZE = KC ? ROWS * LD : BK * ROWS;
  static constexpr int NV4 = ROWS * BK / 4;
};

template <int BK>
__device__ __forceinline__ int kc_off(int row, int k) {
  constexpr int CPR = BK / 4;
  const int q = (k >> 2) ^ ((row / (16 / CPR)) & (CPR - 1));
  return row * BK + 4 * q;
}

template <int ROWS, bool KC, int BK>
__device__ __forceinline__ f32x4 frag(const float* S, int row, int kb) {
  if constexpr (KC) {
    return *reinterpret_cast<const f32x4*>(S + kc_off<BK>(row, kb));
  } else {
    f32x4 r;
    r[0] = S[(kb + 0) * ROWS + row];
    r[1] = S[(kb + 1) * ROWS + row];
    r[2] = S[(kb + 2) * ROWS + row];
    r[3] = S[(kb + 3) * ROWS + row];
    return r;
  }
}

__device__ __forceinline__ int xcd_remap(int bid, int nb) {
  const int xcd = bid & 7, q = nb >> 3, r = nb & 7;
  const int base = xcd < r ? xcd * (q + 1) : r * (q + 1) + (xcd - r) * q;
  return base + (bid >> 3);
}

__device__ __forceinline__ f32x4 zero4() { return f32x4{0.f, 0.f, 0.f, 0.f}; }

__device__ __forceinline__ f32x4 to_f32x4(const f32x4& v) { return v; }
__device__ __forceinline__ f32x4 to_f32x4(uint32_t u) {
  return f32x4{(float)(u & 255u), (float)((u >> 8) & 255u), (float)((u >> 16) & 255u), (float)(u >> 24)};
}

template <class P>
__global__ __launch_bounds__(P::NT) void igemm_kernel(const P p) {
  constexpr int BM = P::BM, BN = P::BN, NT = P::NT, WM = P::WM, WN = P::WN, BK = P::BK;
  constexpr int TM = BM / (32 * WM), TN = BN / (32 * WN);
  static_assert(TM * 32 * WM == BM && TN * 32 * WN == BN && WM * WN * 64 == NT, "tile config");
  static_assert(BK == 16 || BK == 32, "k-tile");
  using TA = Tile<BM, P::A_KC, BK>;
  using TB = Tile<BN, P::B_KC, BK>;
  constexpr int NVA = (TA::NV4 + NT - 1) / NT, NVB = (TB::NV4 + NT - 1) / NT;
  constexpr int STAGE = TA::SIZE + TB::SIZE;
#ifndef PPO_GEMM_STAGES
#define PPO_GEMM_STAGES 2
#endif
  constexpr int NS = PPO_GEMM_STAGES;
  static_assert(NS == 2 || NS == 3, "stages");
  __shared__ __attribute__((aligned(16))) float smem[NS * STAGE];

  const int tid = threadIdx.x, lane = tid & 63, wave = tid >> 6;
  const int wm = wave / WN, wn = wave % WN;
  const int m0 = xcd_remap(blockIdx.x, gridDim.x) * BM;
  const int n0 = blockIdx.y * BN;
  const int z = blockIdx.z;
  int kbeg, kend;
  p.k_range(z, kbeg, kend);
  const int nk = kend > kbeg ? (kend - kbeg + BK - 1) / BK : 0;

  typename P::ACtx actx[NVA];
  typename P::BCtx bctx[NVB];
  int ak[NVA], aoff[NVA], bk[NVB], boff[NVB];
  bool aon[NVA], bon[NVB];
#pragma unroll
  for (int i = 0; i < NVA; ++i) {
    const int f = tid + i * NT;
    aon[i] = f < TA::NV4;
    if constexpr (P::A_KC) {
      const int row = f / (BK / 4), kq = f % (BK / 4);
      actx[i] = p.a_ctx(m0 + row, z);
      ak[i] = 4 * kq;
      aoff[i] = kc_off<BK>(row, 4 * kq);
    } else {
      const int k = f / (BM / 4), rq = f % (BM / 4);
      actx[i] = p.a_ctx(m0 + 4 * rq, z);
      ak[i] = k;
      aoff[i] = k * BM + 4 * rq;
    }
  }
#pragma unroll
  for (int i = 0; i < NVB; ++i) {
    const int f = tid + i * NT;
    bon[i] = f < TB::NV4;
    if constexpr (P::B_KC) {
      const int row = f / (BK / 4), kq = f % (BK / 4);
      bctx[i] = p.b_ctx(n0 + row, z);
      bk[i] = 4 * kq;
      boff[i] = kc_off<BK>(row, 4 * kq);
    } else {
      const int k = f / (BN / 4), rq = f % (BN / 4);
      bctx[i] = p.b_ctx(n0 + 4 * rq, z);
      bk[i] = k;
      boff[i] = k * BN + 4 * rq;
    }
  }

  using ARaw = decltype(p.a_load(actx[0], 0));
  ARaw ra[NVA];
  auto bload = [&](int i, int k0) {
    if constexpr (P::B_TILE) return p.b_load_t(bctx[i], p.tile(k0), k0 + bk[i]);
    else return p.b_load(bctx[i], k0 + bk[i]);
  };
  using BRaw = decltype(bload(0, 0));
  BRaw rb[NVB];
  auto gload = [&](int k0) {
#pragma unroll
    for (int i = 0; i < NVA; ++i) ra[i] = aon[i] ? p.a_load(actx[i], k0 + ak[i]) : ARaw{};
#pragma unroll
    for (int i = 0; i < NVB; ++i) rb[i] = bon[i] ? bload(i, k0) : BRaw{};
  };
  auto sstore = [&](int buf) {
    float* As = smem + buf * STAGE;
    float* Bs = As + TA::SIZE;
#pragma unroll
    for (int i = 0; i < NVA; ++i)
      if (aon[i]) *reinterpret_cast<f32x4*>(As + aoff[i]) = to_f32x4(ra[i]);
#pragma unroll
    for (int i = 0; i < NVB; ++i)
      if (bon[i]) *reinterpret_cast<f32x4*>(Bs + boff[i]) = to_f32x4(rb[i]);
  };

  f32x16 acc[TM][TN];
#pragma unroll
  for (int i = 0; i < TM; ++i)
#pragma unroll
    for (int j = 0; j < TN; ++j)
#pragma unroll
      for (int r = 0; r < 16; ++r) acc[i][j][r] = 0.f;
  float bias_acc = 0.f;

  const int frow = lane & 31, fk = 4 * (lane >> 5);
  auto bias_part = [&](const float* As) {
    if constexpr (P::BIAS_FROM_A) {
      static_assert(!P::A_KC && NT % BM == 0 && BK % (NT / BM) == 0, "bias partials");
      constexpr int G = NT / BM;
      if (blockIdx.y == 0) {
#pragma unroll
        for (int k = tid / BM; k < BK; k += G) bias_acc += As[k * BM + tid % BM];
      }
    }
  };
  auto read_frags = [&](const float* As, int kb, f32x4 (&af)[TM], f32x4 (&bf)[TN]) {
    const float* Bs = As + TA::SIZE;
#pragma unroll
    for (int i = 0; i < TM; ++i) af[i] = frag<BM, P::A_KC, BK>(As, (wm * TM + i) * 32 + frow, kb + fk);
#pragma unroll
    for (int j = 0; j < TN; ++j) bf[j] = frag<BN, P::B_KC, BK>(Bs, (wn * TN + j) * 32 + frow, kb + fk);
  };
  auto mfma_group = [&](const f32x4 (&af)[TM], const f32x4 (&bf)[TN]) {
#pragma unroll
    for (int s = 0; s < 4; ++s)
#pragma unroll
      for (int i = 0; i < TM; ++i)
#pragma unroll
        for (int j = 0; j < TN; ++j)
          acc[i][j] = __builtin_amdgcn_mfma_f32_32x32x2f32(af[i][s], bf[j][s], acc[i][j], 0, 0, 0);
  };

  if constexpr (NS == 2) {
    if (nk > 0) {
      gload(kbeg);
      sstore(0);
    }
    __syncthreads();
    for (int kt = 0; kt < nk; ++kt) {
      const int buf = kt & 1;
      if (kt + 1 < nk) gload(kbeg + (kt + 1) * BK);
      const float* As = smem + buf * STAGE;
      bias_part(As);
#pragma unroll
      for (int kk = 0; kk < BK; kk += 8) {
        f32x4 af[TM], bf[TN];
        read_frags(As, kk, af, bf);
        mfma_group(af, bf);
      }
      if (kt + 1 < nk) sstore(buf ^ 1);
      __syncthreads();
    }
  } else {
    if (nk > 0) {
      gload(kbeg);
      sstore(0);
    }
    if (nk > 1) {
      gload(kbeg + BK);
      sstore(1);
    }
    __syncthreads();
    f32x4 fa[TM], fb[TN];
    if (nk > 0) read_frags(smem, 0, fa, fb);
    int cur = 0;
    for (int kt = 0; kt < nk; ++kt) {
      const int nxt = cur == 2 ? 0 : cur + 1, stg = nxt == 2 ? 0 : nxt + 1;
      if (kt + 2 < nk) gload(kbeg + (kt + 2) * BK);
      const float* As = smem + cur * STAGE;
      bias_part(As);
#pragma unroll
      for (int kk = 0; kk < BK; kk += 8) {
        f32x4 ga[TM], gb[TN];
        if (kk + 8 < BK) read_frags(As, kk + 8, ga, gb);
        else if (kt + 1 < nk) read_frags(smem + nxt * STAGE, 0, ga, gb);
        mfma_group(fa, fb);
#pragma unroll
        for (int i = 0; i < TM; ++i) fa[i] = ga[i];
#pragma unroll
        for (int j = 0; j < TN; ++j) fb[j] = gb[j];
      }
      if (kt + 2 < nk) sstore(stg);
      __syncthreads();
      cur = nxt;
    }
  }

  const int hi = lane >> 5;
  if constexpr (P::TILE_EPI) {
    static_assert(WN == 1, "tile epilogue: one wave column");
#pragma unroll
    for (int i = 0; i < TM; ++i)
#pragma unroll
      for (int r = 0; r < 16; ++r) {
        const int row = (wm * TM + i) * 32 + (r & 3) + 8 * (r >> 2) + 4 * hi;
        float v[TN];
#pragma unroll
        for (int j = 0; j < TN; ++j) v[j] = acc[i][j][r];
        p.store_tile(m0 + row, blockIdx.y * 32 + frow, z, v);
      }
  } else {
#pragma unroll
    for (int i = 0; i < TM; ++i)
#pragma unroll
      for (int j = 0; j < TN; ++j)
#pragma unroll
        for (int r = 0; r < 16; ++r) {
          const int row = (wm * TM + i) * 32 + (r & 3) + 8 * (r >> 2) + 4 * hi;
          const int col = (wn * TN + j) * 32 + frow;
          p.store(m0 + row, n0 + col, z, acc[i][j][r]);
        }
  }
  if constexpr (P::BIAS_FROM_A) {
    if (blockIdx.y == 0) {
      constexpr int G = NT / BM;
      smem[tid] = bias_acc;
      __syncthreads();
      if (tid < BM) {
        float t = smem[tid];
#pragma unroll
        for (int g = 1; g < G; ++g) t += smem[g * BM + tid];
        p.store_bias(m0 + tid, z, t);
      }
    }
  }
}

template <int BM_, int BN_, int WM_, int WN_, bool AKC, bool BKC, bool BIASA = false, int BK_ = BK16>
struct Cfg {
  static constexpr int BM = BM_, BN = BN_, WM = WM_, WN = WN_, NT = 64 * WM_ * WN_, BK = BK_;
  static constexpr bool A_KC = AKC, B_KC = BKC, BIAS_FROM_A = BIASA, TILE_EPI = false, B_TILE = false;
  struct ACtx { const float* p; int a; int b; bool ok; };
  struct BCtx { const float* p; int a; bool ok; };
};


__device__ __forceinline__ long long obs_row(const int64_t* idx, long long row0, int b) {
  return idx ? (long long)idx[b] : row0 + b;
}

template <class C_>
struct DenseReluFwd : C_ {
  const float* x; const float* w; const float* bias; float* out; int M, N, K;
  int lda = 0, ldo = 0, relu = 1;
  const int64_t* idx = nullptr;
  using ACtx = typename C_::ACtx;
  using BCtx = typename C_::BCtx;
  __device__ ACtx a_ctx(int m, int) const {
    if (m >= M) return {x, 0, 0, false};
    return {x + (size_t)(idx ? idx[m] : m) * (lda ? lda : K), 0, 0, true};
  }
  __device__ f32x4 a_load(const ACtx& c, int k) const {
    return (c.ok && k < K) ? *reinterpret_cast<const f32x4*>(c.p + k) : zero4();
  }
  __device__ BCtx b_ctx(int n, int) const { return {w + (size_t)n * K, 0, n < N}; }
  __device__ f32x4 b_load(const BCtx& c, int k) const {
    return (c.ok && k < K) ? *reinterpret_cast<const f32x4*>(c.p + k) : zero4();
  }
  __device__ void k_range(int, int& b, int& e) const { b = 0; e = K; }
  __device__ void store(int m, int n, int, float v) const {
    if (m < M && n < N) {
      float y = bias ? v + bias[n] : v;
      out[(size_t)m * (ldo ? ldo : N) + n] = relu == 1 ? fmaxf(y, 0.f) : (relu == 2 ? tanhf(y) : y);
    }
  }
  static constexpr bool VEC_STORE = true;
  int vec = 0;
  __device__ void store4(int m, int n, int, const f32x4& v) const {
    if (m >= M || n >= N) return;
    f32x4 y = v;
    if (bias) y += *reinterpret_cast<const f32x4*>(bias + n);
#pragma unroll
    for (int r = 0; r < 4; ++r) y[r] = relu == 1 ? fmaxf(y[r], 0.f) : (relu == 2 ? tanhf(y[r]) : y[r]);
    *reinterpret_cast<f32x4*>(out + (size_t)m * (ldo ? ldo : N) + n) = y;
  }
};

template <class C_>
struct DenseDgradMask : C_ {
  const float* dy; const float* wt; const float* act; float* dx; int M, N, K;
  int ldact = 0;
  int mode = 1;
  using ACtx = typename C_::ACtx;
  using BCtx = typename C_::BCtx;
  __device__ ACtx a_ctx(int m, int) const { return {dy + (size_t)m * K, 0, 0, m < M}; }
  __device__ f32x4 a_load(const ACtx& c, int k) const {
    return (c.ok && k < K) ? *reinterpret_cast<const f32x4*>(c.p + k) : zero4();
  }
  __device__ BCtx b_ctx(int n, int) const { return {wt + (size_t)n * K, 0, n < N}; }
  __device__ f32x4 b_load(const BCtx& c, int k) const {
    return (c.ok && k < K) ? *reinterpret_cast<const f32x4*>(c.p + k) : zero4();
  }
  __device__ void k_range(int, int& b, int& e) const { b = 0; e = K; }
  __device__ void store(int m, int n, int, float v) const {
    if (m < M && n < N) {
      const size_t i = (size_t)m * N + n;
      if (!act) {
        dx[i] = v;
      } else {
        const float y = act[(size_t)m * (ldact ? ldact : N) + n];
        dx[i] = mode == 2 ? v * (1.0f - y * y) : (y > 0.f ? v : 0.f);
      }
    }
  }
  static constexpr bool VEC_STORE = true;
  int vec = 0;
  __device__ void store4(int m, int n, int, const f32x4& v) const {
    if (m >= M || n >= N) return;
    f32x4 o = v;
    if (act) {
      const f32x4 y = *reinterpret_cast<const f32x4*>(act + (size_t)m * (ldact ? ldact : N) + n);
#pragma unroll
      for (int r = 0; r < 4; ++r) o[r] = mode == 2 ? v[r] * (1.0f - y[r] * y[r]) : (y[r] > 0.f ? v[r] : 0.f);
    }
    *reinterpret_cast<f32x4*>(dx + (size_t)m * N + n) = o;
  }
};

template <class C_>
struct DenseDgradPair : C_ {
  const float* dy0; const float* wt0; const float* dy1; const float* wt1; float* dx; int M, N, K0, K1;
  struct ACtx { const float* p0; const float* p1; bool ok; };
  struct BCtx { const float* p0; const float* p1; bool ok; };
  __device__ f32x4 load(const float* p0, const float* p1, bool ok, int k) const {
    if (!ok || k >= K0 + K1) return zero4();
    return *reinterpret_cast<const f32x4*>(k < K0 ? p0 + k : p1 + (k - K0));
  }
  __device__ ACtx a_ctx(int m, int) const { return {dy0 + (size_t)m * K0, dy1 + (size_t)m * K1, m < M}; }
  __device__ f32x4 a_load(const ACtx& c, int k) const { return load(c.p0, c.p1, c.ok, k); }
  __device__ BCtx b_ctx(int n, int) const { return {wt0 + (size_t)n * K0, wt1 + (size_t)n * K1, n < N}; }
  __device__ f32x4 b_load(const BCtx& c, int k) const { return load(c.p0, c.p1, c.ok, k); }
  __device__ void k_range(int, int& b, int& e) const { b = 0; e = K0 + K1; }
  __device__ void store(int m, int n, int, float v) const {
    if (m < M && n < N) dx[(size_t)m * N + n] = v;
  }
  static constexpr bool VEC_STORE = true;
  int vec = 0;
  __device__ void store4(int m, int n, int, const f32x4& v) const {
    if (m >= M || n >= N) return;
    *reinterpret_cast<f32x4*>(dx + (size_t)m * N + n) = v;
  }
};

struct ABufCtx { uint32_t off; };
__device__ __forceinline__ f32x4 abuf_load(const float* base, uint32_t bytes, const ABufCtx& c, int k, int K) {
  const uint32_t off = k < K ? c.off + 4u * (uint32_t)k : 0x80000000u;
  return __builtin_bit_cast(f32x4, __builtin_amdgcn_raw_buffer_load_b128(make_rsrc(base, bytes), off, 0, 0));
}

template <class C_>
struct DenseReluFwdB : DenseReluFwd<C_> {
  using ACtx = ABufCtx;
  __device__ uint32_t ld() const { return (uint32_t)(this->lda ? this->lda : this->K); }
  __device__ ACtx a_ctx(int m, int) const { return {m < this->M ? 4u * (uint32_t)m * ld() : 0x80000000u}; }
  __device__ f32x4 a_load(const ACtx& c, int k) const {
    return abuf_load(this->x, 4u * (uint32_t)this->M * ld(), c, k, this->K);
  }
};

template <class C_>
struct DenseDgradMaskB : DenseDgradMask<C_> {
  using ACtx = ABufCtx;
  __device__ ACtx a_ctx(int m, int) const { return {m < this->M ? 4u * (uint32_t)m * (uint32_t)this->K : 0x80000000u}; }
  __device__ f32x4 a_load(const ACtx& c, int k) const {
    return abuf_load(this->dy, 4u * (uint32_t)this->M * (uint32_t)this->K, c, k, this->K);
  }
};

template <class C_>
struct WgradBase : C_ {
  const float* dz; int COUT; long long R; int chunk;
  float* slab; float* slab_bias; int NW;
  using ACtx = typename C_::ACtx;
  __device__ ACtx a_ctx(int co, int) const { return {dz + co, 0, 0, co < COUT}; }
  __device__ f32x4 a_load(const ACtx& c, int r) const {
    return (c.ok && r < R) ? *reinterpret_cast<const f32x4*>(c.p + (size_t)r * COUT) : zero4();
  }
  __device__ void k_range(int z, int& b, int& e) const {
    const long long bb = (long long)z * chunk;
    b = (int)(bb < R ? bb : R);
    const long long ee = bb + chunk;
    e = (int)(ee < R ? ee : R);
  }
  __device__ void store(int m, int n, int z, float v) const {
    if (m < COUT && n < NW) slab[((size_t)z * COUT + m) * NW + n] = v;
  }
  static constexpr bool VEC_STORE = true;
  int vec = 0;
  __device__ void store4(int m, int n, int z, const f32x4& v) const {
    if (m < COUT && n < NW) *reinterpret_cast<f32x4*>(slab + ((size_t)z * COUT + m) * NW + n) = v;
  }
  __device__ void store_bias(int m, int z, float v) const {
    if (m < COUT) slab_bias[(size_t)z * COUT + m] = v;
  }
};

template <class C_>
struct DenseWgrad : WgradBase<C_> {
  const float* x; int K;
  struct BCtx { const float* p; bool ok; };
  __device__ BCtx b_ctx(int n, int) const { return {x + n, n < K}; }
  __device__ f32x4 b_load(const BCtx& c, int r) const {
    return (c.ok && r < this->R) ? *reinterpret_cast<const f32x4*>(c.p + (size_t)r * K) : zero4();
  }
};

template <class C_>
struct DenseWgradB : WgradBase<C_> {
  const float* x; int K;
  struct ACtx { uint32_t off; };
  struct BCtx { uint32_t off; };
  __device__ ACtx a_ctx(int co, int) const { return {co < this->COUT ? 4u * (uint32_t)co : 0x80000000u}; }
  __device__ f32x4 a_load(const ACtx& c, int r) const {
    const auto rs = make_rsrc(this->dz, (uint32_t)(this->R * this->COUT) * 4u);
    return __builtin_bit_cast(f32x4, __builtin_amdgcn_raw_buffer_load_b128(
                                         rs, c.off + __umul24((uint32_t)r, 4u * (uint32_t)this->COUT), 0, 0));
  }
  __device__ BCtx b_ctx(int n, int) const { return {n < K ? 4u * (uint32_t)n : 0x80000000u}; }
  __device__ f32x4 b_load(const BCtx& c, int r) const {
    const auto rs = make_rsrc(x, (uint32_t)(this->R * K) * 4u);
    return __builtin_bit_cast(f32x4, __builtin_amdgcn_raw_buffer_load_b128(
                                         rs, c.off + __umul24((uint32_t)r, 4u * (uint32_t)K), 0, 0));
  }
};

struct ColMap {
  int kind, a, b, nw;
  __device__ __forceinline__ size_t operator()(long long c) const {
    if (kind == 0) return (size_t)c;
    const int m = (int)(c / nw), n = (int)(c - (long long)m * nw);
    if (kind == 3) return n < a ? (size_t)m * a + n : (size_t)-1;
    if (kind == 1) {
      const int ky = n / (a * b), rem = n - ky * (a * b), kx = rem / b, ci = rem - kx * b;
      return (size_t)m * nw + (size_t)ci * a * a + ky * a + kx;
    }
    const int pp = n / a, ch = n - pp * a;
    return (size_t)m * nw + (size_t)ch * b + pp;
  }
};

__global__ __launch_bounds__(256) void colsum_kernel(const float* __restrict__ src, long long ld, int Z,
                                                     long long cols, ColMap map, float* __restrict__ out, float scale,
                                                     int accumulate) {
  const int cl = threadIdx.x & 31, zg = threadIdx.x >> 5;
  const long long c = (long long)blockIdx.x * 32 + cl;
  float s0 = 0.f, s1 = 0.f, s2 = 0.f, s3 = 0.f;
  if (c < cols) {
    const float* p = src + c;
    int z = zg;
    for (; z + 24 < Z; z += 32) {
      s0 += p[(size_t)z * ld];
      s1 += p[(size_t)(z + 8) * ld];
      s2 += p[(size_t)(z + 16) * ld];
      s3 += p[(size_t)(z + 24) * ld];
    }
    for (; z < Z; z += 8) s0 += p[(size_t)z * ld];
  }
  __shared__ float red[8][33];
  red[zg][cl] = (s0 + s1) + (s2 + s3);
  __syncthreads();
  if (zg == 0 && c < cols) {
    float t = red[0][cl];
#pragma unroll
    for (int g = 1; g < 8; ++g) t += red[g][cl];
    t *= scale;
    const size_t o = map(c);
    if (o != (size_t)-1) out[o] = accumulate ? out[o] + t : t;
  }
}

template <class P>
int launch(const P& p, long long M, int N, int Z, hipStream_t st, const char* name, double flops) {
  if (M <= 0 || N <= 0 || Z <= 0) return 0;
  const long long gx = (M + P::BM - 1) / P::BM;
  if (gx > 0x7fffffffLL) {
    ppo_set_error("%s: grid too large (M=%lld)", name, M);
    return PPO_ESHAPE;
  }
  dim3 grid((unsigned)gx, (unsigned)((N + P::BN - 1) / P::BN), (unsigned)Z);
  int slot;
  const bool prof = ppo_prof_begin(name, st, &slot);
  igemm_kernel<P><<<grid, P::NT, 0, st>>>(p);
  if (prof) ppo_prof_end(slot, st, flops);
  PPO_LAUNCH_CHECK(name);
  return 0;
}


static inline int colsum(const float* src, long long ld, int Z, long long cols, ColMap map, float* out, float scale,
                         int accumulate, hipStream_t st) {
  if (cols <= 0) return 0;
  colsum_kernel<<<ceil_div(cols, 32), 256, 0, st>>>(src, ld, Z, cols, map, out, scale, accumulate);
  PPO_LAUNCH_CHECK("colsum_kernel");
  return 0;
}

}
```

Baseline: 1.622 million.

## Fuse FC split-K reduce into heads act kernel and batch colsum launches

During rollout with categorical actions, the FC split-K partial slab is no longer reduced by a separate kernel. The heads act kernel reads the slab slices directly, then sums them, adds the bias and applies ReLU per row. This removes one kernel launch and the round trip of the reduced FC output through memory. Separately, the wgrad and heads-reduce column sums are merged into one multi-job colsum launch instead of two to four launches. The heads kernel now reads Z slices per row instead of one feature vector, which may raise its memory traffic and register use.

```diff
diff --git a/include/ppo_hip.h b/include/ppo_hip.h
--- a/include/ppo_hip.h
+++ b/include/ppo_hip.h
@@ -75,6 +75,8 @@
 long long ppo_fc_fwd_ws_bytes(int M, int H);
 int ppo_fc_fwd_ws(const float* x, int M, const float* w4p, const float* b, int H, float* out, int ldo, float* ws,
                   long long ws_bytes, void* stream);
+int ppo_fc_fwd_slab_slices(int M, int H);
+int ppo_fc_fwd_slab(const float* x, int M, const float* w4p, int H, float* ws, long long ws_bytes, void* stream);
 int ppo_linear_relu_fwd(const float* x, int M, int K, const float* w, const float* b, int N, float* out,
                         void* stream);
 int ppo_linear_fwd_ex(const float* x, const int64_t* idx, int M, int K, int lda, const float* w, const float* b,
@@ -164,6 +166,7 @@
                   int deterministic, const int64_t* given, float* value, int64_t* action, float* logp,
                   float* entropy, void* stream);
 int ppo_heads_train_blocks(int B);
+int ppo_heads_train_rows(int which);
 int ppo_heads_train(const float* feat, const float* feat_v, int B, int H, const float* wc, const float* bc,
                     const float* wa,
                     const float* ba, int A, const int64_t* idx, long long row0, const int64_t* actions,
@@ -200,6 +203,15 @@
                      const float* wa, const float* ba, int A, const float* noise, unsigned long long seed,
                      const unsigned long long* counter, int deterministic, const int64_t* given, float* value,
                      int64_t* action, float* logp, float* entropy, void* stream);
+int ppo_heads_act_ws(const float* slab, int slices, const float* fc_bias, int N, int H, const float* wc,
+                     const float* bc, const float* wa, const float* ba, int A, const float* noise,
+                     unsigned long long seed, unsigned long long counter, int deterministic, const int64_t* given,
+                     float* value, int64_t* action, float* logp, float* entropy, void* stream);
+int ppo_heads_act_ws_dc(const float* slab, int slices, const float* fc_bias, int N, int H, const float* wc,
+                        const float* bc, const float* wa, const float* ba, int A, const float* noise,
+                        unsigned long long seed, const unsigned long long* counter, int deterministic,
+                        const int64_t* given, float* value, int64_t* action, float* logp, float* entropy,
+                        void* stream);
 int ppo_heads_gauss_act_dc(const float* feat, const float* feat_v, int N, int H, const float* wc, const float* bc,
                            const float* wa, const float* ba, const float* logstd, int A, const float* noise,
                            unsigned long long seed, const unsigned long long* counter, int deterministic,
diff --git a/ppo-dash_amd/a2c_ppo_acktr/_engine.py b/ppo-dash_amd/a2c_ppo_acktr/_engine.py
--- a/ppo-dash_amd/a2c_ppo_acktr/_engine.py
+++ b/ppo-dash_amd/a2c_ppo_acktr/_engine.py
@@ -40,6 +40,12 @@
             self.bufs[name] = t
             self.version += 1
         return t
+
+
+class FcSlab:
+
+    def __init__(self, ws, slices):
+        self.ws, self.slices = ws, slices
 
 
 class CNNEngine:
@@ -216,7 +222,7 @@
              self.C * 84 * 84, stream())
         return x, None
 
-    def trunk(self, obs, idx, B, ws, out=None, ldo=None):
+    def trunk(self, obs, idx, B, ws, out=None, ldo=None, slab_ok=False):
         dev = self.device
         obs, idx = self._obs_f32(obs, idx, B, ws)
         a1 = ws.get("a1", B * 400 * 32, device=dev)
@@ -248,6 +254,10 @@
         nb = call("ppo_fc_fwd_ws_bytes", B, self.H)
         if nb:
             fws = ws.get("fc_ws", nb // 4, device=dev)
+            slices = call("ppo_fc_fwd_slab_slices", B, self.H) if slab_ok else 0
+            if slices:
+                call("ppo_fc_fwd_slab", a3.data_ptr(), B, self.pk(2), self.H, fws.data_ptr(), nb, s)
+                return FcSlab(fws, slices)
             call("ppo_fc_fwd_ws", a3.data_ptr(), B, self.pk(2), self.pv(self.B4), self.H, out.data_ptr(), ldo,
                  fws.data_ptr(), nb, s)
         else:
@@ -302,6 +312,11 @@
                  ptr(given.reshape(-1).contiguous() if given is not None else None, torch.float32, "action"),
                  value.data_ptr(), None if given is not None or value_only else action.data_ptr(),
                  ptr(logp), ptr(ent), stream())
+        elif isinstance(h, FcSlab):
+            call("ppo_heads_act_ws" + dc, h.ws.data_ptr(), h.slices, self.pv(self.B4), B, self.H, self.pv(self.WC),
+                 self.pv(self.BC), self.pv(self.WA), self.pv(self.BA), self.A, ptr(noise), self.rng_seed, counter,
+                 int(bool(deterministic)), None, value.data_ptr(), None if value_only else action.data_ptr(),
+                 ptr(logp), ptr(ent), stream())
         else:
             call("ppo_heads_act" + dc, h.data_ptr(), ptr(hv), B, self.H, self.pv(self.WC), self.pv(self.BC),
                  self.pv(self.WA), self.pv(self.BA), self.A, ptr(noise), self.rng_seed, counter,
@@ -324,7 +339,8 @@
         self.pack()
         obs = self._check_obs(obs)
         B = obs.shape[0]
-        h = self.trunk(obs, None, B, self.ws[self.act_ws])
+        slab_ok = self.dist_kind == "cat" and given is None
+        h = self.trunk(obs, None, B, self.ws[self.act_ws], slab_ok=slab_ok)
         return self._heads(h, B, deterministic, noise, given, want_entropy, value_only)
 
     def _heads_train(self, storage, adv, idx, feat, B, hp, loss_acc, dfeat, feat_act, feat_v=None, dfeat_v=None):
diff --git a/ppo-dash_amd/a2c_ppo_acktr/_hip.py b/ppo-dash_amd/a2c_ppo_acktr/_hip.py
--- a/ppo-dash_amd/a2c_ppo_acktr/_hip.py
+++ b/ppo-dash_amd/a2c_ppo_acktr/_hip.py
@@ -48,6 +48,8 @@
     "ppo_fc_fwd": [c_p, c_int, c_p, c_p, c_int, c_p, c_int, c_p],
     "ppo_fc_fwd_ws_bytes": [c_int, c_int],
     "ppo_fc_fwd_ws": [c_p, c_int, c_p, c_p, c_int, c_p, c_int, c_p, c_ll, c_p],
+    "ppo_fc_fwd_slab_slices": [c_int, c_int],
+    "ppo_fc_fwd_slab": [c_p, c_int, c_p, c_int, c_p, c_ll, c_p],
     "ppo_linear_dgrad_mask": [c_p, c_int, c_int, c_p, c_int, c_p, c_p, c_p],
     "ppo_conv3_fwd_mask": [c_p, c_int, c_p, c_p, c_p, c_p, c_p],
     "ppo_fc_dgrad_bits": [c_p, c_int, c_int, c_p, c_p, c_p, c_p],
@@ -71,6 +73,7 @@
     "ppo_heads_act": [c_p, c_p, c_int, c_int, c_p, c_p, c_p, c_p, c_int, c_p, c_ull, c_ull, c_int, c_p, c_p, c_p,
                       c_p, c_p, c_p],
     "ppo_heads_train_blocks": [c_int],
+    "ppo_heads_train_rows": [c_int],
     "ppo_heads_train": [c_p, c_p, c_int, c_int, c_p, c_p, c_p, c_p, c_int, c_p, c_ll, c_p, c_p, c_p, c_p, c_p, c_f,
                         c_f, c_f, c_f, c_int, c_int, c_p, c_p, c_p, c_p, c_p, c_p],
     "ppo_linear_fwd_ex": [c_p, c_p, c_int, c_int, c_int, c_p, c_p, c_int, c_p, c_int, c_int, c_p],
@@ -114,6 +117,10 @@
                                c_p, c_p, c_p, c_p, c_p],
     "ppo_heads_bern_act_dc": [c_p, c_p, c_int, c_int, c_p, c_p, c_p, c_p, c_int, c_p, c_ull, c_p, c_int, c_p, c_p,
                               c_p, c_p, c_p, c_p],
+    "ppo_heads_act_ws": [c_p, c_int, c_p, c_int, c_int, c_p, c_p, c_p, c_p, c_int, c_p, c_ull, c_ull, c_int, c_p,
+                         c_p, c_p, c_p, c_p, c_p],
+    "ppo_heads_act_ws_dc": [c_p, c_int, c_p, c_int, c_int, c_p, c_p, c_p, c_p, c_int, c_p, c_ull, c_p, c_int, c_p,
+                            c_p, c_p, c_p, c_p, c_p],
     "ppo_rng_advance": [c_p, c_ull, c_p],
     "ppo_obs_preprocess": [c_p, c_ll, c_int, c_int, c_int, c_p, c_d, c_int, c_p, c_ll, c_p],
     "ppo_frame_stack": [c_p, c_int, c_int, c_ll, c_p, c_p, c_int, c_p],
@@ -125,7 +132,7 @@
 }
 _RESTYPES = {"ppo_last_error": ctypes.c_char_p, "ppo_packed_weights_size": c_ll, "ppo_fc_fwd_ws_bytes": c_ll}
 _VALUE_FUNCS = {"ppo_abi_version", "ppo_gae_partials_count", "ppo_gae_scan_partials_count", "ppo_adv_diff_partials_count",
-                "ppo_packed_weights_size", "ppo_fc_fwd_ws_bytes", "ppo_wgrad_splits", "ppo_heads_train_blocks", "ppo_grad_partials_count",
+                "ppo_packed_weights_size", "ppo_fc_fwd_ws_bytes", "ppo_fc_fwd_slab_slices", "ppo_wgrad_splits", "ppo_heads_train_blocks", "ppo_heads_train_rows", "ppo_grad_partials_count",
                 "ppo_conv2_dgrad_bits_ok", "ppo_conv3_dgrad_bits_ok", "ppo_tune_get",
                 "ppo_gru_persist_get", "ppo_gru_persist_timeouts", "ppo_gru_seq_counters"}
 
diff --git a/ppo-dash_amd/csrc/colsum.h b/ppo-dash_amd/csrc/colsum.h
--- /dev/null
+++ b/ppo-dash_amd/csrc/colsum.h
@@ -0,0 +1,13 @@
+#pragma once
+
+struct ColsumCall {
+  const float* src;
+  long long ld;
+  int rows;
+  long long cols;
+  float* out;
+  float scale;
+  int accumulate;
+};
+
+int colsum_calls(const ColsumCall* calls, int n, void* stream);
diff --git a/ppo-dash_amd/csrc/dense.hip b/ppo-dash_amd/csrc/dense.hip
--- a/ppo-dash_amd/csrc/dense.hip
+++ b/ppo-dash_amd/csrc/dense.hip
@@ -1,4 +1,5 @@
 #include "conv_launch.h"
+#include "colsum.h"
 
 namespace {
 
@@ -165,14 +166,9 @@
   return 4LL * Z * M * H;
 }
 
-PPO_API int ppo_fc_fwd_ws(const float* x, int M, const float* w4p, const float* b, int H, float* out, int ldo,
-                          float* ws, long long ws_bytes, void* stream) {
-  const long long need = ppo_fc_fwd_ws_bytes(M, H);
-  if (!use_x9() || need == 0 || ws == nullptr || ws_bytes < need || ldo % 4 != 0 || H % 4 != 0 || 4LL * M * 1568 >= 0x80000000LL ||
-      ((uintptr_t)out & 15) != 0 || ((uintptr_t)ws & 15) != 0 || ((uintptr_t)b & 15) != 0)
-    return ppo_fc_fwd(x, M, w4p, b, H, out, ldo, stream);
-  const int K = 1568, Z = (int)(need / (4LL * M * H));
-  hipStream_t st = as_stream(stream);
+static int fc_fwd_splitk(const float* x, int M, const float* w4p, const float* b, int H, float* out, int ldo,
+                         float* ws, int Z, hipStream_t st) {
+  const int K = 1568;
   int rc;
 #define PPO_FCSK(CFG, VEC)                                                                   \
   {                                                                                          \
@@ -188,12 +184,40 @@
   if (tune_key(TK_FC_SPLITK_TILE)) PPO_FCSK(XP128, 1)
   else PPO_FCSK(XP128x64w8, 0)
 #undef PPO_FCSK
+  return rc;
+}
+
+PPO_API int ppo_fc_fwd_ws(const float* x, int M, const float* w4p, const float* b, int H, float* out, int ldo,
+                          float* ws, long long ws_bytes, void* stream) {
+  const long long need = ppo_fc_fwd_ws_bytes(M, H);
+  if (!use_x9() || need == 0 || ws == nullptr || ws_bytes < need || ldo % 4 != 0 || H % 4 != 0 || 4LL * M * 1568 >= 0x80000000LL ||
+      ((uintptr_t)out & 15) != 0 || ((uintptr_t)ws & 15) != 0 || ((uintptr_t)b & 15) != 0)
+    return ppo_fc_fwd(x, M, w4p, b, H, out, ldo, stream);
+  const int Z = (int)(need / (4LL * M * H));
+  hipStream_t st = as_stream(stream);
+  const int rc = fc_fwd_splitk(x, M, w4p, b, H, out, ldo, ws, Z, st);
   if (rc) return rc;
   const long long n = (long long)M * (H / 4);
   fc_splitk_reduce_kernel<<<(unsigned)std::min<long long>((n + 255) / 256, 4096), 256, 0, st>>>(ws, Z, M, H, b, out,
                                                                                                ldo);
   PPO_LAUNCH_CHECK("fc_splitk_reduce_kernel");
   return 0;
+}
+
+PPO_API int ppo_fc_fwd_slab_slices(int M, int H) {
+  const long long need = ppo_fc_fwd_ws_bytes(M, H);
+  if (!use_x9() || need == 0 || H % 4 != 0 || 4LL * M * 1568 >= 0x80000000LL) return 0;
+  return (int)(need / (4LL * M * H));
+}
+
+PPO_API int ppo_fc_fwd_slab(const float* x, int M, const float* w4p, int H, float* ws, long long ws_bytes,
+                            void* stream) {
+  const int Z = ppo_fc_fwd_slab_slices(M, H);
+  PPO_REQUIRE(Z > 0, "ppo_fc_fwd_slab: no split-K form at M=%d H=%d (ppo_fc_fwd_slab_slices is 0)", M, H);
+  PPO_REQUIRE(ws != nullptr && ((uintptr_t)ws & 15) == 0 && ws_bytes >= 4LL * Z * M * H,
+              "ppo_fc_fwd_slab: workspace %p (16-byte aligned) of %lld bytes, %lld needed", (void*)ws, ws_bytes,
+              4LL * Z * M * H);
+  return fc_fwd_splitk(x, M, w4p, nullptr, H, nullptr, H, ws, Z, as_stream(stream));
 }
 
 PPO_API int ppo_linear_relu_fwd(const float* x, int M, int K, const float* w, const float* b, int N, float* out,
@@ -406,14 +430,22 @@
                              float* gw, float* gb, float scale, int accumulate, void* stream) {
   PPO_REQUIRE(kind >= 0 && kind <= 3, "ppo_wgrad_reduce: kind=%d", kind);
   ProfScope prof("wgrad_reduce", as_stream(stream), 4.0 * (double)Z * M * (NW + 1) + 4.0 * M * (NW + 1));
-  hipStream_t st = as_stream(stream);
   const long long cols = (long long)M * NW;
-  int rc = colsum(slab, cols, Z, cols, ColMap{kind, a, b, NW}, gw, scale, accumulate, st);
-  if (rc) return rc;
-  return colsum(slab_bias, M, Z, M, ColMap{0, 0, 0, 1}, gb, 1.0f, accumulate, st);
+  const ColJob jobs[2] = {{slab, cols, Z, cols, ColMap{kind, a, b, NW}, gw, scale, accumulate},
+                          {slab_bias, M, Z, M, ColMap{0, 0, 0, 1}, gb, 1.0f, accumulate}};
+  return colsum_jobs(jobs, 2, as_stream(stream));
 }
 
 PPO_API int ppo_colsum(const float* src, long long ld, int rows, long long cols, float* out, float scale,
                        int accumulate, void* stream) {
   return colsum(src, ld, rows, cols, ColMap{0, 0, 0, 1}, out, scale, accumulate, as_stream(stream));
 }
+
+int colsum_calls(const ColsumCall* calls, int n, void* stream) {
+  ColJob jobs[COLJOBS_MAX];
+  PPO_REQUIRE(n >= 0 && n <= COLJOBS_MAX, "colsum_calls: %d calls (at most %d)", n, COLJOBS_MAX);
+  for (int i = 0; i < n; ++i)
+    jobs[i] = ColJob{calls[i].src, calls[i].ld, calls[i].rows, calls[i].cols, ColMap{0, 0, 0, 1}, calls[i].out,
+                     calls[i].scale, calls[i].accumulate};
+  return colsum_jobs(jobs, n, as_stream(stream));
+}
diff --git a/ppo-dash_amd/csrc/heads.hip b/ppo-dash_amd/csrc/heads.hip
--- a/ppo-dash_amd/csrc/heads.hip
+++ b/ppo-dash_amd/csrc/heads.hip
@@ -1,5 +1,6 @@
 #include "heads_common.h"
 #include "tune.h"
+#include "colsum.h"
 
 namespace {
 
@@ -39,9 +40,36 @@
   return -logf(u01_open0(h));
 }
 
-template <int HC, int AMAX, bool FAST>
-__global__ __launch_bounds__(64 * HW) void heads_act_kernel(
-    const float* __restrict__ feat, const float* __restrict__ feat_v_, int N, int H_, const float* __restrict__ wc,
+struct SlabFeat {
+  int Z;
+  const float* bias;
+};
+
+template <int HC>
+__device__ __forceinline__ void slab_features(const float* __restrict__ slab, const SlabFeat& sf, long long N,
+                                              long long row, int H, int lane, float (&f)[HC]) {
+  const float* const p = slab + row * H + lane;
+  const size_t zs = (size_t)N * H;
+#pragma unroll
+  for (int c = 0; c < HC; ++c) f[c] = lane + 64 * c < H ? p[64 * c] : 0.f;
+  if (sf.Z == 4) {
+#pragma unroll
+    for (int z = 1; z < 4; ++z)
+#pragma unroll
+      for (int c = 0; c < HC; ++c) f[c] += lane + 64 * c < H ? p[z * zs + 64 * c] : 0.f;
+  } else {
+    for (int z = 1; z < sf.Z; ++z)
+#pragma unroll
+      for (int c = 0; c < HC; ++c) f[c] += lane + 64 * c < H ? p[z * zs + 64 * c] : 0.f;
+  }
+#pragma unroll
+  for (int c = 0; c < HC; ++c) f[c] = lane + 64 * c < H ? fmaxf(f[c] + sf.bias[lane + 64 * c], 0.f) : 0.f;
+}
+
+template <int HC, int AMAX, bool FAST, bool WS>
+__device__ __forceinline__ void heads_act_rows(
+    const float* __restrict__ feat, const float* __restrict__ feat_v_, const SlabFeat sf, int N, int H_,
+    const float* __restrict__ wc,
     const float* __restrict__ bc, const float* __restrict__ wa, const float* __restrict__ ba, int A_,
     const float* __restrict__ noise,
     unsigned long long seed, unsigned long long counter_v, const unsigned long long* __restrict__ counter_p,
@@ -60,11 +88,17 @@
     const long long row = r0 + rr;
     if (row >= N) break;
     float f[HC], fv[HC];
-#pragma unroll
-    for (int c = 0; c < HC; ++c) {
-      const bool in = lane + 64 * c < H;
-      f[c] = in ? feat[row * H + lane + 64 * c] : 0.f;
-      fv[c] = feat_v ? (in ? feat_v[row * H + lane + 64 * c] : 0.f) : f[c];
+    if constexpr (WS) {
+      slab_features<HC>(feat, sf, N, row, H, lane, f);
+#pragma unroll
+      for (int c = 0; c < HC; ++c) fv[c] = f[c];
+    } else {
+#pragma unroll
+      for (int c = 0; c < HC; ++c) {
+        const bool in = lane + 64 * c < H;
+        f[c] = in ? feat[row * H + lane + 64 * c] : 0.f;
+        fv[c] = feat_v ? (in ? feat_v[row * H + lane + 64 * c] : 0.f) : f[c];
+      }
     }
     float value, z[AMAX], nl[AMAX], p[AMAX];
     head_dots(w, f, fv, value, z, b0, ba, A);
@@ -96,6 +130,33 @@
       if (ent_out) ent_out[row] = ent;
     }
   }
+}
+
+template <int HC, int AMAX, bool FAST>
+__global__ __launch_bounds__(64 * HW) void heads_act_kernel(
+    const float* __restrict__ feat, const float* __restrict__ feat_v_, int N, int H_, const float* __restrict__ wc,
+    const float* __restrict__ bc, const float* __restrict__ wa, const float* __restrict__ ba, int A_,
+    const float* __restrict__ noise,
+    unsigned long long seed, unsigned long long counter_v, const unsigned long long* __restrict__ counter_p,
+    int deterministic, const int64_t* __restrict__ given,
+    float* __restrict__ value_out, int64_t* __restrict__ action_out, float* __restrict__ logp_out,
+    float* __restrict__ ent_out, int rows_per_wave) {
+  heads_act_rows<HC, AMAX, FAST, false>(feat, feat_v_, SlabFeat{0, nullptr}, N, H_, wc, bc, wa, ba, A_, noise, seed,
+                                        counter_v, counter_p, deterministic, given, value_out, action_out, logp_out,
+                                        ent_out, rows_per_wave);
+}
+
+template <int HC, int AMAX, bool FAST>
+__global__ __launch_bounds__(64 * HW) void heads_act_ws_kernel(
+    const float* __restrict__ slab, const SlabFeat sf, int N, int H_, const float* __restrict__ wc,
+    const float* __restrict__ bc, const float* __restrict__ wa, const float* __restrict__ ba, int A_,
+    const float* __restrict__ noise,
+    unsigned long long seed, unsigned long long counter_v, const unsigned long long* __restrict__ counter_p,
+    int deterministic, const int64_t* __restrict__ given,
+    float* __restrict__ value_out, int64_t* __restrict__ action_out, float* __restrict__ logp_out,
+    float* __restrict__ ent_out, int rows_per_wave) {
+  heads_act_rows<HC, AMAX, FAST, true>(slab, nullptr, sf, N, H_, wc, bc, wa, ba, A_, noise, seed, counter_v, counter_p,
+                                       deterministic, given, value_out, action_out, logp_out, ent_out, rows_per_wave);
 }
 
 struct TrainArgs {
@@ -279,9 +340,24 @@
   }
 }
 
-__global__ __launch_bounds__(64 * HW) void heads_train_lds_kernel(const TrainArgs a) {
-  constexpr int A = 8, H = 512;
+__device__ __forceinline__ float fold32(float x, float y) {
+  const auto r = __builtin_amdgcn_permlane32_swap(__float_as_uint(x), __float_as_uint(y), false, false);
+  return __uint_as_float(r[0]) + __uint_as_float(r[1]);
+}
+__device__ __forceinline__ float fold16(float x, float y) {
+  const auto r = __builtin_amdgcn_permlane16_swap(__float_as_uint(x), __float_as_uint(y), false, false);
+  return __uint_as_float(r[0]) + __uint_as_float(r[1]);
+}
+
+constexpr int HEADS_TRAIN_ROWS = 2;
+
+template <int R>
+__global__ __launch_bounds__(64 * HW, 2) void heads_train_lds_kernel(const TrainArgs a) {
+#pragma clang fp contract(off)
+  static_assert(R == 2 || R == 4, "row group: 2 or 4 rows");
+  constexpr int A = 8, H = 512, GL = 64 / R;
   const int lane = threadIdx.x & 63, wave = threadIdx.x >> 6;
+  const int grp = lane / GL;
   __shared__ f32x4 Wl[9][128];
   for (int i = threadIdx.x; i < 9 * H; i += 64 * HW) {
     const int o = i / H, k = i - H * o;
@@ -312,95 +388,142 @@
     q_ret = a.ret[sr];
   }
   auto bcast = [](float x, int j) { return __int_as_float(__builtin_amdgcn_readlane(__float_as_int(x), j)); };
-  f32x4 fn[2];
-  auto load_row = [&](long long row) {
-#pragma unroll
-    for (int c2 = 0; c2 < 2; ++c2)
-      fn[c2] = row < a.B ? reinterpret_cast<const f32x4*>(a.feat + row * H)[lane + 64 * c2] : f32x4{0.f, 0.f, 0.f, 0.f};
+  f32x4 fn[R][2];
+  auto load_rows = [&](long long row) {
+#pragma unroll
+    for (int j = 0; j < R; ++j)
+#pragma unroll
+      for (int c2 = 0; c2 < 2; ++c2)
+        fn[j][c2] = row + j < a.B ? reinterpret_cast<const f32x4*>(a.feat + (row + j) * H)[lane + 64 * c2]
+                                  : f32x4{0.f, 0.f, 0.f, 0.f};
   };
-  load_row(r0);
-  for (int rr = 0; rr < a.rows_per_wave; ++rr) {
+  load_rows(r0);
+  for (int rr = 0; rr < a.rows_per_wave; rr += R) {
     const long long row = r0 + rr;
     if (row >= a.B) break;
-    const f32x4 f[2] = {fn[0], fn[1]};
-    if (rr + 1 < a.rows_per_wave) load_row(row + 1);
+    int nr = a.rows_per_wave - rr < R ? a.rows_per_wave - rr : R;
+    if (a.B - row < nr) nr = (int)(a.B - row);
+    f32x4 f[R][2];
+#pragma unroll
+    for (int j = 0; j < R; ++j) {
+      f[j][0] = fn[j][0];
+      f[j][1] = fn[j][1];
+    }
+    if (rr + R < a.rows_per_wave) load_rows(row + R);
+    float t[R][9];
+#pragma unroll
+    for (int j = 0; j < R; ++j)
+#pragma unroll
+      for (int o = 0; o < 9; ++o) t[j][o] = 0.f;
+#pragma unroll
+    for (int c2 = 0; c2 < 2; ++c2) {
+#pragma unroll
+      for (int o = 0; o < 9; ++o) {
+        const f32x4 w = Wl[o][lane + 64 * c2];
+#pragma unroll
+        for (int j = 0; j < R; ++j)
+#pragma unroll
+          for (int q = 0; q < 4; ++q) t[j][o] = __builtin_fmaf(f[j][c2][q], w[q], t[j][o]);
+      }
+    }
     float dots[9];
 #pragma unroll
     for (int o = 0; o < 9; ++o) {
-      float t = 0.f;
-#pragma unroll
-      for (int c2 = 0; c2 < 2; ++c2) {
-        const f32x4 w = Wl[o][lane + 64 * c2];
-#pragma unroll
-        for (int q = 0; q < 4; ++q) t += f[c2][q] * w[q];
-      }
-      dots[o] = wave_sum(t);
+      float s;
+      if constexpr (R == 4) {
+        s = fold16(fold32(t[0][o], t[2][o]), fold32(t[1][o], t[3][o]));
+      } else {
+        s = fold32(t[0][o], t[1][o]);
+        s += __shfl_xor(s, 16, 64);
+      }
+#pragma unroll
+      for (int x = 8; x > 0; x >>= 1) s += __shfl_xor(s, x, 64);
+      dots[o] = s;
     }
     const float value = dots[0] + b0;
     float z[A], nl[A], p[A];
 #pragma unroll
     for (int o = 0; o < A; ++o) z[o] = dots[1 + o] + ba[o];
     categorical(z, A, nl, p);
-    const int act = __builtin_amdgcn_readlane(q_act, rr);
-    s_bad += (unsigned)act < (unsigned)A ? 0.f : 1.f;
+    const int act = __shfl(q_act, rr + grp, 64);
+    const float bad = (unsigned)act < (unsigned)A ? 0.f : 1.f;
     float lp = 0.f, ent = 0.f;
 #pragma unroll
     for (int o = 0; o < A; ++o) {
       if (o == act) lp = nl[o];
       ent -= nl[o] * p[o];
     }
-    const float adv = bcast(q_adv, rr);
-    const float ratio = expf(lp - bcast(q_olp, rr));
+    const float adv = __shfl(q_adv, rr + grp, 64);
+    const float ratio = expf(lp - __shfl(q_olp, rr + grp, 64));
     const float surr1 = ratio * adv;
     const float rc = fminf(fmaxf(ratio, 1.0f - clip), 1.0f + clip);
     const float surr2 = rc * adv;
     const float w1 = surr1 < surr2 ? 1.f : (surr1 == surr2 ? 0.5f : 0.f);
     const float inr = (ratio >= 1.0f - clip && ratio <= 1.0f + clip) ? 1.f : 0.f;
-    const float g_logp = -a.inv_b * (w1 * adv + (1.f - w1) * adv * inr) * ratio;
-    const float vo = bcast(q_vo, rr), R = bcast(q_ret, rr);
+    const float g_logp = -a.inv_b * __builtin_fmaf(w1, adv, (1.f - w1) * adv * inr) * ratio;
+    const float vo = __shfl(q_vo, rr + grp, 64), Rt = __shfl(q_ret, rr + grp, 64);
     float g_v, vl_row;
     if (a.use_clipped_value_loss) {
       const float dv = value - vo;
       const float vpc = vo + fminf(fmaxf(dv, -clip), clip);
-      const float l1 = (value - R) * (value - R);
-      const float l2 = (vpc - R) * (vpc - R);
+      const float l1 = (value - Rt) * (value - Rt);
+      const float l2 = (vpc - Rt) * (vpc - Rt);
       vl_row = fmaxf(l1, l2);
       const float u1 = l1 > l2 ? 1.f : (l1 == l2 ? 0.5f : 0.f);
       const float vin = (dv >= -clip && dv <= clip) ? 1.f : 0.f;
-      g_v = a.value_coef * 0.5f * a.inv_b * (u1 * 2.f * (value - R) + (1.f - u1) * 2.f * (vpc - R) * vin);
+      g_v = a.value_coef * 0.5f * a.inv_b * __builtin_fmaf(vin, (1.f - u1) * 2.f * (vpc - Rt), u1 * 2.f * (value - Rt));
     } else {
-      vl_row = (R - value) * (R - value);
-      g_v = a.value_coef * a.inv_b * (value - R);
-    }
-    s_vl += vl_row;
-    s_al += fminf(surr1, surr2);
-    s_ent += ent;
+      vl_row = (Rt - value) * (Rt - value);
+      g_v = a.value_coef * a.inv_b * (value - Rt);
+    }
+    const float al_row = fminf(surr1, surr2);
     float g[9];
     g[0] = g_v;
     const float ce = a.entropy_coef * a.inv_b;
 #pragma unroll
-    for (int o = 0; o < A; ++o) g[1 + o] = g_logp * ((o == act ? 1.f : 0.f) - p[o]) + ce * p[o] * (nl[o] + ent);
+    for (int o = 0; o < A; ++o)
+      g[1 + o] = __builtin_fmaf(g_logp, (o == act ? 1.f : 0.f) - p[o], ce * p[o] * (nl[o] + ent));
+    float gs[R][9];
+#pragma unroll
+    for (int j = 0; j < R; ++j) {
+      if (j < nr) {
+#pragma unroll
+        for (int o = 0; o < 9; ++o) gs[j][o] = bcast(g[o], j * GL);
+        s_bad += bcast(bad, j * GL);
+        s_vl += bcast(vl_row, j * GL);
+        s_al += bcast(al_row, j * GL);
+        s_ent += bcast(ent, j * GL);
+        gbc += gs[j][0];
+#pragma unroll
+        for (int o = 0; o < A; ++o) gba[o] += gs[j][1 + o];
+      }
+    }
 #pragma unroll
     for (int c2 = 0; c2 < 2; ++c2) {
-      f32x4 d = Wl[0][lane + 64 * c2] * g[0];
-#pragma unroll
-      for (int o = 1; o < 9; ++o) {
-        const f32x4 w = Wl[o][lane + 64 * c2];
-#pragma unroll
-        for (int q = 0; q < 4; ++q) d[q] += g[o] * w[q];
-      }
-      f32x4 y;
-#pragma unroll
-      for (int q = 0; q < 4; ++q) y[q] = act_grad(d[q], f[c2][q], a.feat_act);
-      reinterpret_cast<f32x4*>(a.dfeat + row * H)[lane + 64 * c2] = y;
-#pragma unroll
-      for (int o = 0; o < 9; ++o)
-#pragma unroll
-        for (int q = 0; q < 4; ++q) gw[o][c2][q] += g[o] * f[c2][q];
-    }
-    gbc += g_v;
-#pragma unroll
-    for (int o = 0; o < A; ++o) gba[o] += g[1 + o];
+      f32x4 w[9];
+#pragma unroll
+      for (int o = 0; o < 9; ++o) w[o] = Wl[o][lane + 64 * c2];
+#pragma unroll
+      for (int j = 0; j < R; ++j) {
+        if (j < nr) {
+          f32x4 d = w[0] * gs[j][0];
+#pragma unroll
+          for (int o = 1; o < 9; ++o) {
+            d[0] += gs[j][o] * w[o][0];
+#pragma unroll
+            for (int q = 1; q < 4; ++q) d[q] = __builtin_fmaf(gs[j][o], w[o][q], d[q]);
+          }
+          f32x4 y;
+#pragma unroll
+          for (int q = 0; q < 4; ++q) y[q] = act_grad(d[q], f[j][c2][q], a.feat_act);
+          reinterpret_cast<f32x4*>(a.dfeat + (row + j) * H)[lane + 64 * c2] = y;
+#pragma unroll
+          for (int o = 0; o < 9; ++o)
+#pragma unroll
+            for (int q = 0; q < 4; ++q) gw[o][c2][q] = __builtin_fmaf(gs[j][o], f[j][c2][q], gw[o][c2][q]);
+        }
+      }
+    }
   }
   __shared__ f32x4 red[HW][128];
   __shared__ float redb[HW][A + 5];
@@ -466,12 +589,25 @@
   float* v;
   int64_t* act;
   float *lp, *ent;
+  SlabFeat slab = {0, nullptr};
 };
 
 template <int HC, int AMAX>
 int launch_act(const ActCall& c, hipStream_t st) {
   const int rpw = (int)std::min<long long>(8, std::max<long long>(1, ceil_div(c.N, 4096)));
   const unsigned blocks = ceil_div(c.N, HW * rpw);
+  if (c.slab.Z > 0) {
+    if (c.A == AMAX && c.H == 64 * HC)
+      heads_act_ws_kernel<HC, AMAX, true><<<blocks, 64 * HW, 0, st>>>(c.feat, c.slab, c.N, c.H, c.wc, c.bc, c.wa, c.ba,
+                                                             c.A, c.noise, c.seed, c.counter, c.counter_p, c.det,
+                                                             c.given, c.v, c.act, c.lp, c.ent, rpw);
+    else
+      heads_act_ws_kernel<HC, AMAX, false><<<blocks, 64 * HW, 0, st>>>(c.feat, c.slab, c.N, c.H, c.wc, c.bc, c.wa, c.ba,
+                                                              c.A, c.noise, c.seed, c.counter, c.counter_p, c.det,
+                                                              c.given, c.v, c.act, c.lp, c.ent, rpw);
+    PPO_LAUNCH_CHECK("heads_act_ws_kernel");
+    return 0;
+  }
   if (c.A == AMAX && c.H == 64 * HC && !c.feat_v)
     heads_act_kernel<HC, AMAX, true><<<blocks, 64 * HW, 0, st>>>(c.feat, c.feat_v, c.N, c.H, c.wc, c.bc, c.wa, c.ba, c.A,
                                                         c.noise, c.seed, c.counter, c.counter_p, c.det, c.given, c.v,
@@ -499,7 +635,8 @@
 int heads_act(const char* name, const ActCall& c, void* stream) {
   PPO_REQUIRE(c.N >= 0 && c.A >= 1 && c.A <= 16, "%s: N=%d A=%d (1..16 actions)", name, c.N, c.A);
   PPO_REQUIRE(c.H > 0 && c.H <= 512, "%s: hidden size %d (1..512)", name, c.H);
-  ProfScope prof("heads_act", as_stream(stream), (double)c.N * (4.0 * c.H * (c.feat_v ? 2 : 1) + 16.0));
+  ProfScope prof("heads_act", as_stream(stream),
+                 (double)c.N * (4.0 * c.H * (c.slab.Z > 0 ? c.slab.Z : c.feat_v ? 2 : 1) + 16.0));
   if (c.N == 0) return 0;
   if (c.A <= 8) return dispatch_act<8>(hc_of(c.H), c, as_stream(stream));
   return dispatch_act<16>(hc_of(c.H), c, as_stream(stream));
@@ -511,7 +648,7 @@
 int launch_train(const TrainArgs& a, int blocks, hipStream_t st) {
   if (tune_heads_lds() && HC == 8 && AMAX == 8 && a.A == 8 && a.H == 512 && !a.feat_v && !a.dfeat_v &&
       ((uintptr_t)a.feat & 15) == 0 && ((uintptr_t)a.dfeat & 15) == 0 && ((uintptr_t)a.part_w & 15) == 0) {
-    heads_train_lds_kernel<<<blocks, 64 * HW, 0, st>>>(a);
+    heads_train_lds_kernel<HEADS_TRAIN_ROWS><<<blocks, 64 * HW, 0, st>>>(a);
     PPO_LAUNCH_CHECK("heads_train_lds_kernel");
     return 0;
   }
@@ -557,6 +694,34 @@
   return heads_act("ppo_heads_act_dc", c, stream);
 }
 
+static int heads_act_ws(const char* name, ActCall c, int slices, const float* fc_bias, void* stream) {
+  PPO_REQUIRE(c.feat != nullptr && fc_bias != nullptr && slices >= 1 && slices <= 64,
+              "%s: slab %p, fc bias %p, %d slices (1..64)", name, (const void*)c.feat, (const void*)fc_bias, slices);
+  c.slab = SlabFeat{slices, fc_bias};
+  return heads_act(name, c, stream);
+}
+
+PPO_API int ppo_heads_act_ws(const float* slab, int slices, const float* fc_bias, int N, int H, const float* wc,
+                             const float* bc, const float* wa, const float* ba, int A, const float* noise,
+                             unsigned long long seed, unsigned long long counter, int deterministic,
+                             const int64_t* given, float* value, int64_t* action, float* logp, float* entropy,
+                             void* stream) {
+  const ActCall c = {slab, nullptr, N, H, wc, bc, wa, ba, A, noise, seed, counter, nullptr, deterministic, given,
+                     value, action, logp, entropy};
+  return heads_act_ws("ppo_heads_act_ws", c, slices, fc_bias, stream);
+}
+
+PPO_API int ppo_heads_act_ws_dc(const float* slab, int slices, const float* fc_bias, int N, int H, const float* wc,
+                                const float* bc, const float* wa, const float* ba, int A, const float* noise,
+                                unsigned long long seed, const unsigned long long* counter, int deterministic,
+                                const int64_t* given, float* value, int64_t* action, float* logp, float* entropy,
+                                void* stream) {
+  PPO_REQUIRE(counter != nullptr, "ppo_heads_act_ws_dc: counter is NULL (a device pointer to one 8-byte word)");
+  const ActCall c = {slab, nullptr, N, H, wc, bc, wa, ba, A, noise, seed, 0ull, counter, deterministic, given,
+                     value, action, logp, entropy};
+  return heads_act_ws("ppo_heads_act_ws_dc", c, slices, fc_bias, stream);
+}
+
 PPO_API int ppo_rng_advance(unsigned long long* counter, unsigned long long by, void* stream) {
   PPO_REQUIRE(counter != nullptr, "ppo_rng_advance: counter is NULL (a device pointer to one 8-byte word)");
   rng_advance_kernel<<<1, 1, 0, as_stream(stream)>>>(counter, by);
@@ -564,9 +729,12 @@
   return 0;
 }
 
-PPO_API int ppo_heads_train_blocks(int B) {
-  const int rpw = 32;
-  return (int)ceil_div(B, HW * rpw);
+constexpr int HEADS_TRAIN_RPW = 32;
+
+PPO_API int ppo_heads_train_blocks(int B) { return (int)ceil_div(B, HW * HEADS_TRAIN_RPW); }
+
+PPO_API int ppo_heads_train_rows(int which) {
+  return which == 0 ? HW : which == 1 ? HEADS_TRAIN_RPW : which == 2 ? HEADS_TRAIN_ROWS : 0;
 }
 
 PPO_API int ppo_heads_train(const float* feat, const float* feat_v, int B, int H, const float* wc, const float* bc,
@@ -588,7 +756,7 @@
   a.feat_act = feat_act;
   a.dfeat_v = dfeat_v;
   a.dfeat = dfeat; a.part_w = part_w; a.part_b = part_b; a.part_loss = part_loss;
-  a.rows_per_wave = 32;
+  a.rows_per_wave = HEADS_TRAIN_RPW;
   const int blocks = ppo_heads_train_blocks(B);
   hipStream_t st = as_stream(stream);
   if (A <= 8) return dispatch_train<8>(hc_of(H), a, blocks, st);
@@ -601,11 +769,12 @@
   (void)use_clipped_value_loss;
   ProfScope prof("heads_reduce", as_stream(stream), 4.0 * nblk * (1.0 + A) * (H + 1));
   const long long NO = 1 + A;
-  int rc;
-  if ((rc = ppo_colsum(part_w, NO * H, nblk, H, g_wc, scale, 0, stream))) return rc;
-  if ((rc = ppo_colsum(part_w + H, NO * H, nblk, (long long)A * H, g_wa, scale, 0, stream))) return rc;
-  if ((rc = ppo_colsum(part_b, NO, nblk, 1, g_bc, scale, 0, stream))) return rc;
-  if ((rc = ppo_colsum(part_b + 1, NO, nblk, A, g_ba, scale, 0, stream))) return rc;
+  const ColsumCall sums[4] = {{part_w, NO * H, nblk, H, g_wc, scale, 0},
+                              {part_w + H, NO * H, nblk, (long long)A * H, g_wa, scale, 0},
+                              {part_b, NO, nblk, 1, g_bc, scale, 0},
+                              {part_b + 1, NO, nblk, A, g_ba, scale, 0}};
+  const int rc = colsum_calls(sums, 4, stream);
+  if (rc) return rc;
   if (loss_acc) {
     loss_reduce_kernel<<<1, 256, 0, as_stream(stream)>>>(part_loss, nblk, loss_acc, inv_b);
     PPO_LAUNCH_CHECK("loss_reduce_kernel");
diff --git a/ppo-dash_amd/csrc/igemm.h b/ppo-dash_amd/csrc/igemm.h
--- a/ppo-dash_amd/csrc/igemm.h
+++ b/ppo-dash_amd/csrc/igemm.h
@@ -481,11 +481,11 @@
   }
 };
 
-__global__ __launch_bounds__(256) void colsum_kernel(const float* __restrict__ src, long long ld, int Z,
-                                                     long long cols, ColMap map, float* __restrict__ out, float scale,
-                                                     int accumulate) {
+__device__ __forceinline__ void colsum_block(const float* __restrict__ src, long long ld, int Z, long long cols,
+                                             const ColMap& map, float* __restrict__ out, float scale, int accumulate,
+                                             long long block) {
   const int cl = threadIdx.x & 31, zg = threadIdx.x >> 5;
-  const long long c = (long long)blockIdx.x * 32 + cl;
+  const long long c = block * 32 + cl;
   float s0 = 0.f, s1 = 0.f, s2 = 0.f, s3 = 0.f;
   if (c < cols) {
     const float* p = src + c;
@@ -511,6 +511,37 @@
   }
 }
 
+__global__ __launch_bounds__(256) void colsum_kernel(const float* __restrict__ src, long long ld, int Z,
+                                                     long long cols, ColMap map, float* __restrict__ out, float scale,
+                                                     int accumulate) {
+  colsum_block(src, ld, Z, cols, map, out, scale, accumulate, blockIdx.x);
+}
+
+struct ColJob {
+  const float* src;
+  long long ld;
+  int Z;
+  long long cols;
+  ColMap map;
+  float* out;
+  float scale;
+  int accumulate;
+};
+constexpr int COLJOBS_MAX = 4;
+struct ColJobs {
+  ColJob job[COLJOBS_MAX];
+  unsigned first[COLJOBS_MAX + 1];
+};
+
+__global__ __launch_bounds__(256) void colsum_jobs_kernel(const ColJobs js) {
+  int i = 0;
+#pragma unroll
+  for (int k = 1; k < COLJOBS_MAX; ++k)
+    if (blockIdx.x >= js.first[k]) i = k;
+  const ColJob& j = js.job[i];
+  colsum_block(j.src, j.ld, j.Z, j.cols, j.map, j.out, j.scale, j.accumulate, blockIdx.x - js.first[i]);
+}
+
 template <class P>
 int launch(const P& p, long long M, int N, int Z, hipStream_t st, const char* name, double flops) {
   if (M <= 0 || N <= 0 || Z <= 0) return 0;
@@ -537,4 +568,21 @@
   return 0;
 }
 
-}
+static inline int colsum_jobs(const ColJob* jobs, int n, hipStream_t st) {
+  ColJobs js = {};
+  unsigned blocks = 0;
+  int k = 0;
+  for (int i = 0; i < n && k < COLJOBS_MAX; ++i) {
+    if (jobs[i].cols <= 0) continue;
+    js.job[k] = jobs[i];
+    js.first[k++] = blocks;
+    blocks += (unsigned)ceil_div(jobs[i].cols, 32);
+  }
+  for (int i = k; i <= COLJOBS_MAX; ++i) js.first[i] = blocks;
+  if (blocks == 0) return 0;
+  colsum_jobs_kernel<<<blocks, 256, 0, st>>>(js);
+  PPO_LAUNCH_CHECK("colsum_jobs_kernel");
+  return 0;
+}
+
+}
```

Measured after the change: 1.634 million, median of 6. Within noise of the previous version (+0.7%).
